# freewym/espresso

Hardware: AMD Instinct MI355X
Metric: audio-hours/sec training (LibriSpeech Conformer-12 + CTC) (higher is better)
Workload: dtype bf16; 1 GPU; LibriSpeech 960h Conformer-12 + CTC update step, <=26000 frames & <=24 utts per GPU, V=5004, on-GPU fbank+CMVN+SpecAugment, dropout 0.1, clip 2.0, Adam; parallelism=dp1

## Files before the change

espresso_amd/csrc/conv_igemm.hip:

```cpp
#include <hip/hip_runtime.h>

#include "gemm_common.h"

namespace {

typedef const __attribute__((address_space(1))) void* gptr_t;
typedef __attribute__((address_space(3))) void* lptr_t;

struct ConvGatherArgs {
  const bf16_t* src;
  const bf16_t* W;
  bf16_t* out;
  const float* bias;
  double* stats;
  const bf16_t* zero;
  int RB, RT, RF;
  int ST, SF, SC;
  int at, af;
  int ntaps;
  int bt[9], bf[9], koff[9];
  int N;
  long ldw;
  int OT, OF, ot_mul, ot_add, of_mul, of_add;
};

template <int BN_>
__global__ __launch_bounds__(256, 2) void conv_gather_kernel(const ConvGatherArgs a) {
  constexpr int BM_ = 128, NST = 2;
  constexpr int NJ = BN_ / 32;
  constexpr int A_BYTES = BM_ * ROW_BYTES, STAGE = A_BYTES + BN_ * ROW_BYTES;
  constexpr int NA = BM_ / 32, NB = BN_ / 32;
  extern __shared__ __attribute__((aligned(16))) char dsm[];
  const int tid = threadIdx.x, lane = tid & 63, wave = tid >> 6;
  const int wm = wave >> 1, wcol = (wave & 1) * (BN_ / 2);
  const uint32_t M = (uint32_t)a.RB * a.RT * a.RF;
  const uint32_t m0 = blockIdx.x * BM_;
  const int cpt = a.SC / BK;
  const int nk = a.ntaps * cpt;

  int rowb[NA], rowt[NA], rowf[NA];
  int cs[NA];
#pragma unroll
  for (int i = 0; i < NA; ++i) {
    const int r = (wave + 4 * i) * 8 + (lane >> 3);
    cs[i] = (lane & 7) ^ (r & 7) ^ ((r >> 4) & 7);
    const uint32_t p = m0 + r;
    if (p < M) {
      const uint32_t q = p / (uint32_t)a.RF, b = q / (uint32_t)a.RT;
      const int rf = (int)(p - q * a.RF), rt = (int)(q - b * a.RT);
      rowb[i] = (int)b * a.ST;
      rowt[i] = rt * a.at;
      rowf[i] = rf * a.af;
    } else {
      rowb[i] = -1;
      rowt[i] = rowf[i] = 0;
    }
  }
  const bf16_t* bp[NB];
#pragma unroll
  for (int i = 0; i < NB; ++i) {
    const int r = (wave + 4 * i) * 8 + (lane >> 3);
    const int c = (lane & 7) ^ (r & 7) ^ ((r >> 4) & 7);
    bp[i] = a.W + (long)min(r, a.N - 1) * a.ldw + c * 8;
  }
  auto issue = [&](int stage, int kt) {
    const int tap = kt / cpt, chunk = kt - tap * cpt;
    const int dt = a.bt[tap], df = a.bf[tap];
    const long ko = a.koff[tap] + chunk * BK;
    char* base = dsm + stage * STAGE + wave * 1024;
#pragma unroll
    for (int i = 0; i < NA; ++i) {
      const int st = rowt[i] + dt, sf = rowf[i] + df;
      const bool ok = rowb[i] >= 0 && (unsigned)st < (unsigned)a.ST && (unsigned)sf < (unsigned)a.SF;
      const bf16_t* s = ok ? a.src + (((long)(rowb[i] + st)) * a.SF + sf) * a.SC + chunk * BK + cs[i] * 8 : a.zero + cs[i] * 8;
      __builtin_amdgcn_global_load_lds((gptr_t)s, (lptr_t)(base + i * 4096), 16, 0, 0);
    }
#pragma unroll
    for (int i = 0; i < NB; ++i)
      __builtin_amdgcn_global_load_lds((gptr_t)(bp[i] + ko), (lptr_t)(base + A_BYTES + i * 4096), 16, 0, 0);
  };

  f32x4_t acc[4][NJ];
#pragma unroll
  for (int i = 0; i < 4; ++i)
#pragma unroll
    for (int j = 0; j < NJ; ++j) acc[i][j] = (f32x4_t){0.f, 0.f, 0.f, 0.f};
  uint32_t a_off[2][4], b_off[2][NJ];
#pragma unroll
  for (int ks = 0; ks < 2; ++ks) {
#pragma unroll
    for (int i = 0; i < 4; ++i) a_off[ks][i] = lds_off(wm * 64 + i * 16 + (lane & 15), ks * 4 + (lane >> 4));
#pragma unroll
    for (int j = 0; j < NJ; ++j) b_off[ks][j] = A_BYTES + lds_off(wcol + j * 16 + (lane & 15), ks * 4 + (lane >> 4));
  }

  if (nk > 0) issue(0, 0);
  int stage = 0;
  for (int kt = 0; kt < nk; ++kt) {
    asm volatile("s_waitcnt vmcnt(0)" ::: "memory");
    __builtin_amdgcn_s_barrier();
    if (kt + 1 < nk) issue(stage ^ 1, kt + 1);
    const char* st = dsm + stage * STAGE;
#pragma unroll
    for (int ks = 0; ks < 2; ++ks) {
      bf16x8_t af[4], bfr[NJ];
#pragma unroll
      for (int i = 0; i < 4; ++i) af[i] = *reinterpret_cast<const bf16x8_t*>(st + a_off[ks][i]);
#pragma unroll
      for (int j = 0; j < NJ; ++j) bfr[j] = *reinterpret_cast<const bf16x8_t*>(st + b_off[ks][j]);
#pragma unroll
      for (int i = 0; i < 4; ++i)
#pragma unroll
        for (int j = 0; j < NJ; ++j)
          acc[i][j] = __builtin_amdgcn_mfma_f32_16x16x32_bf16(
              __builtin_bit_cast(__attribute__((ext_vector_type(8))) __bf16, af[i]),
              __builtin_bit_cast(__attribute__((ext_vector_type(8))) __bf16, bfr[j]), acc[i][j], 0, 0, 0);
    }
    stage ^= 1;
  }

  constexpr int CG = BN_ / 8;
  constexpr int RL = 256 / CG;
  float* sC = reinterpret_cast<float*>(dsm);
  const int cg = tid % CG, rlane = tid / CG;
  float bias8[8], s8[8], q8[8];
#pragma unroll
  for (int e = 0; e < 8; ++e) {
    bias8[e] = a.bias ? a.bias[cg * 8 + e] : 0.f;
    s8[e] = q8[e] = 0.f;
  }
#pragma unroll 1
  for (int half = 0; half < 2; ++half) {
    __syncthreads();
    if (wm == half) {
#pragma unroll
      for (int i = 0; i < 4; ++i)
#pragma unroll
        for (int j = 0; j < NJ; ++j)
#pragma unroll
          for (int r = 0; r < 4; ++r) sC[(i * 16 + (lane >> 4) * 4 + r) * BN_ + wcol + j * 16 + (lane & 15)] = acc[i][j][r];
    }
    __syncthreads();
#pragma unroll 1
    for (int pass = 0; pass < 64 / RL; ++pass) {
      const int rl = pass * RL + rlane;
      const uint32_t p = m0 + half * 64 + rl;
      if (p < M) {
        const uint32_t q = p / (uint32_t)a.RF, b = q / (uint32_t)a.RT;
        const int rf = (int)(p - q * a.RF), rt = (int)(q - b * a.RT);
        const long orow = ((long)b * a.OT + (long)rt * a.ot_mul + a.ot_add) * a.OF + (long)rf * a.of_mul + a.of_add;
        const float4 x0 = *reinterpret_cast<const float4*>(sC + rl * BN_ + cg * 8);
        const float4 x1 = *reinterpret_cast<const float4*>(sC + rl * BN_ + cg * 8 + 4);
        float v[8] = {x0.x, x0.y, x0.z, x0.w, x1.x, x1.y, x1.z, x1.w};
#pragma unroll
        for (int e = 0; e < 8; ++e) v[e] += bias8[e];
        uint4 u;
        u.x = pack_bf2(v[0], v[1]); u.y = pack_bf2(v[2], v[3]); u.z = pack_bf2(v[4], v[5]); u.w = pack_bf2(v[6], v[7]);
        *reinterpret_cast<uint4*>(a.out + orow * a.N + cg * 8) = u;
        if (a.stats) {
          const uint32_t w[4] = {u.x, u.y, u.z, u.w};
#pragma unroll
          for (int e = 0; e < 4; ++e) {
            const float lo = __uint_as_float(w[e] << 16), hi = __uint_as_float(w[e] & 0xffff0000u);
            s8[2 * e] += lo; q8[2 * e] += lo * lo;
            s8[2 * e + 1] += hi; q8[2 * e + 1] += hi * hi;
          }
        }
      }
    }
  }
  if (a.stats) {
    __syncthreads();
    float* red = reinterpret_cast<float*>(dsm);
#pragma unroll
    for (int e = 0; e < 8; ++e) {
      red[(rlane * 2 + 0) * BN_ + cg * 8 + e] = s8[e];
      red[(rlane * 2 + 1) * BN_ + cg * 8 + e] = q8[e];
    }
    __syncthreads();
    if (tid < 2 * BN_) {
      const int which = tid / BN_, c = tid - which * BN_;
      float t = 0.f;
      for (int r = 0; r < RL; ++r) t += red[(r * 2 + which) * BN_ + c];
      atomicAdd(a.stats + which * a.N + c, (double)t);
    }
  }
}

const bf16_t* zero_line(hipStream_t stream) {
  static bf16_t* z = nullptr;
  if (!z) {
    if (hipMalloc(&z, 256) != hipSuccess) return nullptr;
    if (hipMemsetAsync(z, 0, 256, stream) != hipSuccess) return nullptr;
    hipStreamSynchronize(stream);
  }
  return z;
}

template <int BN_>
int launch_gather(const ConvGatherArgs& a, hipStream_t stream) {
  constexpr int bytes = 2 * (128 + BN_) * ROW_BYTES;
  static bool attr_ok = hipFuncSetAttribute(reinterpret_cast<const void*>(&conv_gather_kernel<BN_>),
                                            hipFuncAttributeMaxDynamicSharedMemorySize, bytes) == hipSuccess;
  if (!attr_ok) return -1;
  const long M = (long)a.RB * a.RT * a.RF;
  if (M <= 0) return 0;
  if (M >= (1L << 31) - 128) return -1;
  hipLaunchKernelGGL((conv_gather_kernel<BN_>), dim3((unsigned)((M + 127) / 128)), dim3(256), bytes, stream, a);
  return EA_CHECK_LAUNCH();
}


struct ConvWgradArgs {
  const bf16_t* X;
  const bf16_t* dZ;
  float* slab;
  const bf16_t* zero;
  int RB, RT, RF, ST, SF, Cin, Cout;
  int at, af, ntaps;
  int bt[9], bf[9];
  int chunks_per_wg;
};

__device__ __forceinline__ int tr_sw(int r) { return (r & 3) ^ ((r >> 3) & 1); }
__device__ __forceinline__ void ds_read_tr16_x8(const uint32_t (&ad)[8], uint2 (&o)[8]) {
  asm volatile(
      "ds_read_b64_tr_b16 %0, %8\n\tds_read_b64_tr_b16 %1, %9\n\tds_read_b64_tr_b16 %2, %10\n\tds_read_b64_tr_b16 %3, %11\n\t"
      "ds_read_b64_tr_b16 %4, %12\n\tds_read_b64_tr_b16 %5, %13\n\tds_read_b64_tr_b16 %6, %14\n\tds_read_b64_tr_b16 %7, %15\n\t"
      "s_waitcnt lgkmcnt(0)"
      : "=&v"(o[0]), "=&v"(o[1]), "=&v"(o[2]), "=&v"(o[3]), "=&v"(o[4]), "=&v"(o[5]), "=&v"(o[6]), "=&v"(o[7])
      : "v"(ad[0]), "v"(ad[1]), "v"(ad[2]), "v"(ad[3]), "v"(ad[4]), "v"(ad[5]), "v"(ad[6]), "v"(ad[7])
      : "memory");
}

__global__ __launch_bounds__(256, 4) void conv_wgrad_kernel(const ConvWgradArgs a) {
  constexpr int TILE = 64 * ROW_BYTES;
  constexpr int NT = 3, NBUF = 2;
  const int tap0 = (int)(blockIdx.z % 3) * 3;
  const int zsplit = (int)(blockIdx.z / 3);
  __shared__ __attribute__((aligned(16))) char lds[(2 + NBUF) * TILE];
  const int tid = threadIdx.x, lane = tid & 63, wave = tid >> 6;
  const int wr = wave >> 1, wc = wave & 1;
  const int co0 = blockIdx.x * 64, ci0 = blockIdx.y * 64;
  const long M = (long)a.RB * a.RT * a.RF;
  const long chunk0 = (long)zsplit * a.chunks_per_wg;
  long nch = (M + 63) / 64 - chunk0;
  if (nch > a.chunks_per_wg) nch = a.chunks_per_wg;
  if (nch < 0) nch = 0;

  f32x4_t acc[NT][2][2];
#pragma unroll
  for (int t = 0; t < NT; ++t)
#pragma unroll
    for (int i = 0; i < 2; ++i)
#pragma unroll
      for (int j = 0; j < 2; ++j) acc[t][i][j] = (f32x4_t){0.f, 0.f, 0.f, 0.f};

  int rr[2], cs[2];
#pragma unroll
  for (int i = 0; i < 2; ++i) {
    rr[i] = (wave + 4 * i) * 8 + (lane >> 3);
    cs[i] = (lane & 7) ^ (tr_sw(rr[i]) << 1);
  }
  int rowb[2], rowt[2], rowf[2];
  long rowp[2];
  auto decode = [&](long ch) {
#pragma unroll
    for (int i = 0; i < 2; ++i) {
      const long p = (chunk0 + ch) * 64 + rr[i];
      rowp[i] = p;
      if (p < M) {
        const uint32_t q = (uint32_t)p / (uint32_t)a.RF, b = q / (uint32_t)a.RT;
        rowb[i] = (int)b * a.ST;
        rowt[i] = (int)(q - b * a.RT) * a.at;
        rowf[i] = (int)((uint32_t)p - q * a.RF) * a.af;
      } else {
        rowb[i] = -1;
        rowt[i] = rowf[i] = 0;
      }
    }
  };
  auto issue_A = [&](int abuf) {
#pragma unroll
    for (int i = 0; i < 2; ++i) {
      const bf16_t* s = rowb[i] >= 0 ? a.dZ + rowp[i] * a.Cout + co0 + cs[i] * 8 : a.zero + cs[i] * 8;
      __builtin_amdgcn_global_load_lds((gptr_t)s, (lptr_t)(lds + abuf * TILE + (wave + 4 * i) * 1024), 16, 0, 0);
    }
  };
  auto issue_B = [&](int buf, int tap) {
#pragma unroll
    for (int i = 0; i < 2; ++i) {
      const int st = rowt[i] + a.bt[tap0 + tap], sf = rowf[i] + a.bf[tap0 + tap];
      const bool ok = rowb[i] >= 0 && (unsigned)st < (unsigned)a.ST && (unsigned)sf < (unsigned)a.SF;
      const bf16_t* s = ok ? a.X + (((long)(rowb[i] + st)) * a.SF + sf) * a.Cin + ci0 + cs[i] * 8 : a.zero + cs[i] * 8;
      __builtin_amdgcn_global_load_lds((gptr_t)s, (lptr_t)(lds + (2 + buf) * TILE + (wave + 4 * i) * 1024), 16, 0, 0);
    }
  };
  const uint32_t lds0 = (uint32_t)(uintptr_t)lds;
  auto read_frags = [&](int tile_off, int c0, uint4 (&fr)[2][2]) {
    const int g = lane >> 4, i = lane & 15;
    uint32_t ad[8];
    uint2 o[8];
#pragma unroll
    for (int ks = 0; ks < 2; ++ks)
#pragma unroll
      for (int t = 0; t < 2; ++t)
#pragma unroll
        for (int h = 0; h < 2; ++h) {
          const int r = ks * 32 + 8 * g + (i >> 2) + 4 * h;
          const int chunk = (c0 >> 4) + t;
          ad[(ks * 2 + t) * 2 + h] = lds0 + tile_off + r * ROW_BYTES + ((chunk ^ tr_sw(r)) << 5) + (i & 3) * 8;
        }
    ds_read_tr16_x8(ad, o);
#pragma unroll
    for (int ks = 0; ks < 2; ++ks)
#pragma unroll
      for (int t = 0; t < 2; ++t) fr[ks][t] = make_uint4(o[(ks * 2 + t) * 2].x, o[(ks * 2 + t) * 2].y, o[(ks * 2 + t) * 2 + 1].x, o[(ks * 2 + t) * 2 + 1].y);
  };

  const int nsteps = (int)nch * NT;
  int is = 0, itap = 0;
  long ich = 0;
  auto issue_next = [&]() {
    if (is >= nsteps) return;
    if (itap == 0) {
      decode(ich);
      issue_A((int)(ich & 1));
    }
    issue_B(is & (NBUF - 1), itap);
    ++is;
    if (++itap == NT) { itap = 0; ++ich; }
  };
  issue_next();
  uint4 fa[2][2];
  long ch = 0;
  int tap = 0;
  for (int s = 0; s < nsteps; ++s) {
    const int tap1 = tap + 1 == NT ? 0 : tap + 1;
    asm volatile("s_waitcnt vmcnt(0)" ::: "memory");
    __builtin_amdgcn_s_barrier();
    uint4 fb[2][2];
    if (tap == 0) read_frags((int)(ch & 1) * TILE, wr * 32, fa);
    read_frags((2 + (s & (NBUF - 1))) * TILE, wc * 32, fb);
    __builtin_amdgcn_sched_barrier(0);
    issue_next();
#pragma unroll
    for (int t = 0; t < NT; ++t) {
      if (t == tap) {
#pragma unroll
        for (int ks = 0; ks < 2; ++ks)
#pragma unroll
          for (int i = 0; i < 2; ++i)
#pragma unroll
            for (int j = 0; j < 2; ++j)
              acc[t][i][j] = __builtin_amdgcn_mfma_f32_16x16x32_bf16(
                  __builtin_bit_cast(__attribute__((ext_vector_type(8))) __bf16, fa[ks][i]),
                  __builtin_bit_cast(__attribute__((ext_vector_type(8))) __bf16, fb[ks][j]), acc[t][i][j], 0, 0, 0);
      }
    }
    tap = tap1;
    if (tap1 == 0) ++ch;
  }

  float* out = a.slab + (long)zsplit * a.Cout * a.ntaps * a.Cin;
#pragma unroll
  for (int t = 0; t < NT; ++t) {
    {
#pragma unroll
      for (int i = 0; i < 2; ++i)
#pragma unroll
        for (int j = 0; j < 2; ++j)
#pragma unroll
          for (int r = 0; r < 4; ++r) {
            const int co = co0 + wr * 32 + i * 16 + (lane >> 4) * 4 + r, ci = ci0 + wc * 32 + j * 16 + (lane & 15);
            out[((long)co * a.ntaps + tap0 + t) * a.Cin + ci] = acc[t][i][j][r];
          }
    }
  }
}

__global__ __launch_bounds__(256) void conv_wgrad_reduce_kernel(const float* __restrict__ slab, float* __restrict__ dW, long n, int nsplit,
                                                                int cin = 0) {
  const int zper = (nsplit + gridDim.y - 1) / gridDim.y;
  const int z0 = blockIdx.y * zper, z1 = min(nsplit, z0 + zper);
  const long i = ((long)blockIdx.x * 256 + threadIdx.x) * 4;
  if (i >= n || z0 >= z1) return;
  float4 s = *reinterpret_cast<const float4*>(slab + (long)z0 * n + i);
  for (int z = z0 + 1; z < z1; ++z) {
    const float4 x = *reinterpret_cast<const float4*>(slab + (long)z * n + i);
    s.x += x.x; s.y += x.y; s.z += x.z; s.w += x.w;
  }
  if (cin > 0) {
    const long ct = i / cin;
    const int ci = (int)(i - ct * cin), tap = (int)(ct % 9);
    const long co = ct / 9;
    float* d = dW + (co * cin + ci) * 9 + tap;
    const float v[4] = {s.x, s.y, s.z, s.w};
#pragma unroll
    for (int e = 0; e < 4; ++e) {
      if (gridDim.y == 1) d[9 * e] += v[e];
      else atomicAdd(d + 9 * e, v[e]);
    }
    return;
  }
  if (gridDim.y == 1) {
    float4 d = *reinterpret_cast<const float4*>(dW + i);
    d.x += s.x; d.y += s.y; d.z += s.z; d.w += s.w;
    *reinterpret_cast<float4*>(dW + i) = d;
  } else {
    atomicAdd(dW + i, s.x); atomicAdd(dW + i + 1, s.y); atomicAdd(dW + i + 2, s.z); atomicAdd(dW + i + 3, s.w);
  }
}

static int wgrad_split(long M, int Cin, int Cout) {
  const long chunks = (M + 63) / 64;
  const int blocks = (Cin / 64) * (Cout / 64);
  constexpr long target = 256;
  long nsplit = (target + blocks - 1) / blocks;
  if (nsplit > chunks / 8) nsplit = chunks / 8;
  if (nsplit < 1) nsplit = 1;
  return (int)nsplit;
}

}

extern "C" int ea_conv3x3_fwd(const void* X, const void* W, const float* bias, void* Z, double* stats, int B, int T, int F,
                              int Cin, int Cout, int sy, int sx, hipStream_t stream) {
  if (B <= 0 || T <= 0 || F <= 0) return 0;
  if (Cin % 64 || (Cout != 64 && Cout != 128) || sy < 1 || sx < 1) return -2;
  ConvGatherArgs a;
  a.src = (const bf16_t*)X; a.W = (const bf16_t*)W; a.out = (bf16_t*)Z; a.bias = bias; a.stats = stats;
  a.zero = zero_line(stream);
  if (!a.zero) return -1;
  const int To = (T - 1) / sy + 1, Fo = (F - 1) / sx + 1;
  a.RB = B; a.RT = To; a.RF = Fo;
  a.ST = T; a.SF = F; a.SC = Cin;
  a.at = sy; a.af = sx;
  a.ntaps = 9;
  for (int ky = 0; ky < 3; ++ky)
    for (int kx = 0; kx < 3; ++kx) {
      const int t = ky * 3 + kx;
      a.bt[t] = ky - 1; a.bf[t] = kx - 1; a.koff[t] = t * Cin;
    }
  a.N = Cout; a.ldw = 9L * Cin;
  a.OT = To; a.OF = Fo; a.ot_mul = 1; a.ot_add = 0; a.of_mul = 1; a.of_add = 0;
  return Cout == 128 ? launch_gather<128>(a, stream) : launch_gather<64>(a, stream);
}

extern "C" int ea_conv3x3_dgrad(const void* dZ, const void* Wd, void* dX, int B, int T, int F, int Cin, int Cout, int sy, int sx,
                                hipStream_t stream) {
  if (B <= 0 || T <= 0 || F <= 0) return 0;
  if (Cout % 64 || (Cin != 64 && Cin != 128) || sy < 1 || sx < 1 || sy > 2 || sx > 2) return -2;
  const int To = (T - 1) / sy + 1, Fo = (F - 1) / sx + 1;
  const bf16_t* zero = zero_line(stream);
  if (!zero) return -1;
  for (int pt = 0; pt < sy; ++pt)
    for (int pf = 0; pf < sx; ++pf) {
      ConvGatherArgs a;
      a.src = (const bf16_t*)dZ; a.W = (const bf16_t*)Wd; a.out = (bf16_t*)dX; a.bias = nullptr; a.stats = nullptr; a.zero = zero;
      a.RB = B; a.RT = (T - pt + sy - 1) / sy; a.RF = (F - pf + sx - 1) / sx;
      a.ST = To; a.SF = Fo; a.SC = Cout;
      a.at = 1; a.af = 1;
      a.ntaps = 0;
      for (int ky = 0; ky < 3; ++ky) {
        if ((pt + 1 - ky) % sy) continue;
        for (int kx = 0; kx < 3; ++kx) {
          if ((pf + 1 - kx) % sx) continue;
          const int t = a.ntaps++;
          a.bt[t] = (pt + 1 - ky) / sy; a.bf[t] = (pf + 1 - kx) / sx; a.koff[t] = (ky * 3 + kx) * Cout;
        }
      }
      a.N = Cin; a.ldw = 9L * Cout;
      a.OT = T; a.OF = F; a.ot_mul = sy; a.ot_add = pt; a.of_mul = sx; a.of_add = pf;
      if (a.RT <= 0 || a.RF <= 0) continue;
      if (a.ntaps == 0) return -2;
      const int rc = Cin == 128 ? launch_gather<128>(a, stream) : launch_gather<64>(a, stream);
      if (rc) return rc;
    }
  return 0;
}

extern "C" long ea_conv3x3_wgrad_workspace_bytes(int B, int T, int F, int Cin, int Cout, int sy, int sx) {
  const int To = (T - 1) / sy + 1, Fo = (F - 1) / sx + 1;
  return (long)wgrad_split((long)B * To * Fo, Cin, Cout) * Cout * 9 * Cin * (long)sizeof(float);
}

static int conv3x3_wgrad_impl(const void* X, const void* dZ, float* dW, void* workspace, int B, int T, int F, int Cin, int Cout,
                              int sy, int sx, int param_layout, hipStream_t stream);
extern "C" int ea_conv3x3_wgrad(const void* X, const void* dZ, float* dW, void* workspace, int B, int T, int F, int Cin, int Cout,
                                int sy, int sx, hipStream_t stream) {
  return conv3x3_wgrad_impl(X, dZ, dW, workspace, B, T, F, Cin, Cout, sy, sx, 0, stream);
}
extern "C" int ea_conv3x3_wgrad_param_layout(const void* X, const void* dZ, float* dW, void* workspace, int B, int T, int F, int Cin,
                                             int Cout, int sy, int sx, hipStream_t stream) {
  return conv3x3_wgrad_impl(X, dZ, dW, workspace, B, T, F, Cin, Cout, sy, sx, 1, stream);
}
static int conv3x3_wgrad_impl(const void* X, const void* dZ, float* dW, void* workspace, int B, int T, int F, int Cin, int Cout,
                              int sy, int sx, int param_layout, hipStream_t stream) {
  if (B <= 0 || T <= 0 || F <= 0) return 0;
  if (Cin % 64 || Cout % 64 || sy < 1 || sx < 1 || !workspace) return -2;
  ConvWgradArgs a;
  a.X = (const bf16_t*)X; a.dZ = (const bf16_t*)dZ; a.slab = (float*)workspace;
  a.zero = zero_line(stream);
  if (!a.zero) return -1;
  const int To = (T - 1) / sy + 1, Fo = (F - 1) / sx + 1;
  a.RB = B; a.RT = To; a.RF = Fo; a.ST = T; a.SF = F; a.Cin = Cin; a.Cout = Cout;
  a.at = sy; a.af = sx; a.ntaps = 9;
  for (int ky = 0; ky < 3; ++ky)
    for (int kx = 0; kx < 3; ++kx) { a.bt[ky * 3 + kx] = ky - 1; a.bf[ky * 3 + kx] = kx - 1; }
  const long M = (long)B * To * Fo;
  if (M >= (1L << 31) - 128) return -2;
  const int nsplit = wgrad_split(M, Cin, Cout);
  const long chunks = (M + 63) / 64;
  a.chunks_per_wg = (int)((chunks + nsplit - 1) / nsplit);
  hipLaunchKernelGGL(conv_wgrad_kernel, dim3(Cout / 64, Cin / 64, nsplit * 3), dim3(256), 0, stream, a);
  const long n = (long)Cout * 9 * Cin;
  const long blocks = (n / 4 + 255) / 256;
  int zg = (int)(1024 / blocks);
  if (zg > nsplit / 4) zg = nsplit / 4;
  if (zg < 1) zg = 1;
  hipLaunchKernelGGL(conv_wgrad_reduce_kernel, dim3((unsigned)blocks, zg), dim3(256), 0, stream, (const float*)workspace, dW, n, nsplit,
                     param_layout ? Cin : 0);
  return EA_CHECK_LAUNCH();
}
```

espresso_amd/csrc/convmodule.hip:

```cpp
#include "common.h"
#include "convmodule_math.h"
#include "espresso_amd.h"

namespace {

constexpr int KMAX = 31;

constexpr int CT = 64, TTILE = 64, TPT = TTILE / 4;

template <int KW, int PADL>
__global__ __launch_bounds__(256) void glu_dwconv_fwd_kernel(const bf16_t* __restrict__ Y,
                                                             const float* __restrict__ w,
                                                             bf16_t* __restrict__ U, bf16_t* __restrict__ Z,
                                                             double* __restrict__ stats, int T, int C) {
  constexpr int PAD = PADL, ROWS = TTILE + KW - 1;
  __shared__ __attribute__((aligned(16))) float su[ROWS][CT];
  __shared__ float sred[2][4][CT];
  const int c0 = blockIdx.x * CT, t0 = blockIdx.y * TTILE, b = blockIdx.z;
  const long rowbase = (long)b * T;
  if ((C & 7) == 0 && c0 + CT <= C) {
    bf16_t (*sub)[CT] = reinterpret_cast<bf16_t (*)[CT]>(&su[0][0]);
    bf16_t (*sz)[CT] = reinterpret_cast<bf16_t (*)[CT]>(&su[0][0]) + ROWS;
    constexpr int NCH = (ROWS * (CT / 8) + 255) / 256;
    uint4 va[NCH], vg[NCH];
#pragma unroll
    for (int k = 0; k < NCH; ++k) {
      const int i = threadIdx.x + 256 * k;
      const int row = min(i / (CT / 8), ROWS - 1), c8 = (i % (CT / 8)) * 8;
      const int tin = min(max(t0 - PAD + row, 0), T - 1);
      const bf16_t* yr = Y + (rowbase + tin) * (2L * C) + c0 + c8;
      va[k] = *reinterpret_cast<const uint4*>(yr);
      vg[k] = *reinterpret_cast<const uint4*>(yr + C);
    }
    const int cl = threadIdx.x & (CT - 1), grp = threadIdx.x >> 6;
    float wk[KW];
#pragma unroll
    for (int k = 0; k < KW; ++k) wk[k] = w[(long)(c0 + cl) * KW + k];
#pragma unroll
    for (int k = 0; k < NCH; ++k) {
      const int i = threadIdx.x + 256 * k;
      if (i < ROWS * (CT / 8)) {
        const int row = i / (CT / 8), c8 = (i % (CT / 8)) * 8;
        const int tin = t0 - PAD + row;
        uint32_t pk[4];
        glu_gate8(va[k], vg[k], pk);
        const bool inside = tin >= 0 && tin < T;
        const uint4 u4 = inside ? make_uint4(pk[0], pk[1], pk[2], pk[3]) : make_uint4(0, 0, 0, 0);
        if (inside && row >= PAD && row < PAD + TTILE) *reinterpret_cast<uint4*>(U + (rowbase + tin) * C + c0 + c8) = u4;
        *reinterpret_cast<uint4*>(&sub[row][c8]) = u4;
      }
    }
    __syncthreads();
    float acc[TPT];
#pragma unroll
    for (int j = 0; j < TPT; ++j) acc[j] = 0.f;
#pragma unroll
    for (int r = 0; r < TPT + KW - 1; ++r) {
      const float x = bf2f(sub[grp * TPT + r][cl]);
#pragma unroll
      for (int j = 0; j < TPT; ++j)
        if (r - j >= 0 && r - j < KW) acc[j] += wk[r - j] * x;
    }
    float s = 0.f, q = 0.f;
#pragma unroll
    for (int j = 0; j < TPT; ++j) {
      const int tout = t0 + grp * TPT + j;
      const bf16_t zb = f2bf(acc[j]);
      sz[grp * TPT + j][cl] = zb;
      if (tout < T) {
        const float z = bf2f(zb);
        s += z;
        q += z * z;
      }
    }
    if (stats) {
      sred[0][grp][cl] = s;
      sred[1][grp][cl] = q;
    }
    __syncthreads();
#pragma unroll
    for (int k = 0; k < 2; ++k) {
      const int i = threadIdx.x + 256 * k;
      const int r = i >> 3, c8 = (i & 7) * 8;
      if (t0 + r < T) *reinterpret_cast<uint4*>(Z + (rowbase + t0 + r) * C + c0 + c8) = *reinterpret_cast<const uint4*>(&sz[r][c8]);
    }
    if (stats && threadIdx.x < CT) {
      const int x = threadIdx.x;
      atomicAdd(stats + c0 + x, (double)(sred[0][0][x] + sred[0][1][x] + sred[0][2][x] + sred[0][3][x]));
      atomicAdd(stats + C + c0 + x, (double)(sred[1][0][x] + sred[1][1][x] + sred[1][2][x] + sred[1][3][x]));
    }
    return;
  }
  const bool vec = (C & 7) == 0;
  for (int i = threadIdx.x; i < ROWS * (CT / 8); i += 256) {
    const int row = i / (CT / 8), c8 = (i % (CT / 8)) * 8;
    const int tin = t0 - PAD + row;
    float u[8];
#pragma unroll
    for (int e = 0; e < 8; ++e) u[e] = 0.f;
    if (tin >= 0 && tin < T && c0 + c8 < C) {
      const bf16_t* yr = Y + (rowbase + tin) * (2L * C) + c0 + c8;
      uint32_t pk[4] = {0, 0, 0, 0};
      if (vec && c0 + c8 + 8 <= C) {
        const uint4 av = *reinterpret_cast<const uint4*>(yr);
        const uint4 gv = *reinterpret_cast<const uint4*>(yr + C);
        glu_gate8(av, gv, pk);
        if (row >= PAD && row < PAD + TTILE)
          *reinterpret_cast<uint4*>(U + (rowbase + tin) * C + c0 + c8) = make_uint4(pk[0], pk[1], pk[2], pk[3]);
      } else {
        for (int e = 0; e < 8; ++e) {
          if (c0 + c8 + e >= C) break;
          const bf16_t ub = f2bf(bf2f(yr[e]) * sigmoid_f(bf2f(yr[C + e])));
          if (row >= PAD && row < PAD + TTILE) U[(rowbase + tin) * C + c0 + c8 + e] = ub;
          pk[e >> 1] |= (uint32_t)ub << (16 * (e & 1));
        }
      }
#pragma unroll
      for (int e = 0; e < 4; ++e) {
        u[2 * e] = __uint_as_float(pk[e] << 16);
        u[2 * e + 1] = __uint_as_float(pk[e] & 0xffff0000u);
      }
    }
    *reinterpret_cast<float4*>(&su[row][c8]) = make_float4(u[0], u[1], u[2], u[3]);
    *reinterpret_cast<float4*>(&su[row][c8 + 4]) = make_float4(u[4], u[5], u[6], u[7]);
  }
  const int cl = threadIdx.x & (CT - 1), grp = threadIdx.x >> 6;
  const int c = c0 + cl;
  float wk[KW];
#pragma unroll
  for (int k = 0; k < KW; ++k) wk[k] = c < C ? w[(long)c * KW + k] : 0.f;
  __syncthreads();
  float acc[TPT];
#pragma unroll
  for (int j = 0; j < TPT; ++j) acc[j] = 0.f;
#pragma unroll
  for (int r = 0; r < TPT + KW - 1; ++r) {
    const float x = su[grp * TPT + r][cl];
#pragma unroll
    for (int j = 0; j < TPT; ++j)
      if (r - j >= 0 && r - j < KW) acc[j] += wk[r - j] * x;
  }
  float s = 0.f, q = 0.f;
#pragma unroll
  for (int j = 0; j < TPT; ++j) {
    const int tout = t0 + grp * TPT + j;
    if (tout < T && c < C) {
      const bf16_t zb = f2bf(acc[j]);
      Z[(rowbase + tout) * C + c] = zb;
      const float z = bf2f(zb);
      s += z;
      q += z * z;
    }
  }
  if (stats) {
    sred[0][grp][cl] = s;
    sred[1][grp][cl] = q;
    __syncthreads();
    if (threadIdx.x < CT && c0 + threadIdx.x < C) {
      const int x = threadIdx.x;
      atomicAdd(stats + c0 + x, (double)(sred[0][0][x] + sred[0][1][x] + sred[0][2][x] + sred[0][3][x]));
      atomicAdd(stats + C + c0 + x, (double)(sred[1][0][x] + sred[1][1][x] + sred[1][2][x] + sred[1][3][x]));
    }
  }
}

__global__ void bn_finalize_kernel(const double* __restrict__ stats, float* __restrict__ mean_rstd,
                                   float* __restrict__ running_mean, float* __restrict__ running_var,
                                   int C, float n, float eps, float momentum) {
  const int c = blockIdx.x * blockDim.x + threadIdx.x;
  if (c >= C) return;
  const float mean = (float)(stats[c] / (double)n);
  float var = (float)(stats[C + c] / (double)n - (stats[c] / (double)n) * (stats[c] / (double)n));
  var = fmaxf(var, 0.f);
  mean_rstd[c] = mean;
  mean_rstd[C + c] = rsqrtf(var + eps);
  if (running_mean) {
    running_mean[c] = (1.f - momentum) * running_mean[c] + momentum * mean;
    const float unb = n > 1.f ? var * n / (n - 1.f) : var;
    running_var[c] = (1.f - momentum) * running_var[c] + momentum * unb;
  }
}
__global__ void bn_from_running_kernel(const float* __restrict__ running_mean, const float* __restrict__ running_var,
                                       float* __restrict__ mean_rstd, int C, float eps) {
  const int c = blockIdx.x * blockDim.x + threadIdx.x;
  if (c >= C) return;
  mean_rstd[c] = running_mean[c];
  mean_rstd[C + c] = rsqrtf(running_var[c] + eps);
}

__global__ __launch_bounds__(256) void bn_act_fwd_kernel(const bf16_t* __restrict__ Z, const float* __restrict__ mean_rstd,
                                                         const float* __restrict__ gamma, const float* __restrict__ beta,
                                                         bf16_t* __restrict__ Hout, long M, int C, int act) {
  const int nch = C >> 3;
  const long total = M * nch;
  const long stride = (long)gridDim.x * blockDim.x;
  const int ch = (int)(((long)blockIdx.x * blockDim.x + threadIdx.x) % nch);
  float sc[8], sh[8];
#pragma unroll
  for (int e = 0; e < 8; ++e) {
    const int c = ch * 8 + e;
    bn_scale_shift(mean_rstd[c], mean_rstd[C + c], gamma[c], beta[c], sc[e], sh[e]);
  }
  for (long i = (long)blockIdx.x * blockDim.x + threadIdx.x; i < total; i += stride) {
    const long m = i / nch;
    const uint4 u = *reinterpret_cast<const uint4*>(Z + m * C + ch * 8);
    float o[8];
    bn_act8(u, sc, sh, act, o);
    uint4 r;
    r.x = pack_bf2(o[0], o[1]); r.y = pack_bf2(o[2], o[3]); r.z = pack_bf2(o[4], o[5]); r.w = pack_bf2(o[6], o[7]);
    *reinterpret_cast<uint4*>(Hout + m * C + ch * 8) = r;
  }
}

__global__ __launch_bounds__(256) void bn_act_fwd_stats_kernel(const bf16_t* __restrict__ Z, const double* __restrict__ stats,
                                                               float* __restrict__ mean_rstd, float* __restrict__ running_mean,
                                                               float* __restrict__ running_var, const float* __restrict__ gamma,
                                                               const float* __restrict__ beta, bf16_t* __restrict__ Hout, long M,
                                                               int C, int act, float n, float eps, float momentum,
                                                               double* __restrict__ zero_next, int zero_n) {
  extern __shared__ float s_scsh[];
  const int nch = C >> 3;
  const long total = M * nch;
  const long stride = (long)gridDim.x * blockDim.x;
  const long gtid = (long)blockIdx.x * blockDim.x + threadIdx.x;
  const double inv_n = 1.0 / (double)n;
  for (int c = threadIdx.x; c < C; c += 256) {
    const double m1 = stats[c] * inv_n;
    const float mean = (float)m1;
    float var = (float)(stats[C + c] * inv_n - m1 * m1);
    var = fmaxf(var, 0.f);
    const float rstd = rsqrtf(var + eps);
    const float scv = rstd * gamma[c];
    s_scsh[c] = scv;
    s_scsh[C + c] = beta[c] - mean * scv;
    if (blockIdx.x == 0) {
      mean_rstd[c] = mean;
      mean_rstd[C + c] = rstd;
      if (running_mean) {
        running_mean[c] = (1.f - momentum) * running_mean[c] + momentum * mean;
        const float unb = n > 1.f ? var * n / (n - 1.f) : var;
        running_var[c] = (1.f - momentum) * running_var[c] + momentum * unb;
      }
    }
  }
  __syncthreads();
  const int ch = (int)(gtid % nch);
  float sc[8], sh[8];
#pragma unroll
  for (int e = 0; e < 8; ++e) {
    sc[e] = s_scsh[ch * 8 + e];
    sh[e] = s_scsh[C + ch * 8 + e];
  }
  for (long i = gtid; i < total; i += stride) {
    const long m = i / nch;
    const uint4 u = *reinterpret_cast<const uint4*>(Z + m * C + ch * 8);
    const uint32_t wv[4] = {u.x, u.y, u.z, u.w};
    float o[8];
#pragma unroll
    for (int e = 0; e < 8; ++e) {
      const float z = (e & 1) ? __uint_as_float(wv[e >> 1] & 0xffff0000u) : __uint_as_float(wv[e >> 1] << 16);
      const float y = z * sc[e] + sh[e];
      o[e] = act == 2 ? silu_f(y) : (act == 1 ? fmaxf(y, 0.f) : y);
    }
    uint4 r;
    r.x = pack_bf2(o[0], o[1]); r.y = pack_bf2(o[2], o[3]); r.z = pack_bf2(o[4], o[5]); r.w = pack_bf2(o[6], o[7]);
    *reinterpret_cast<uint4*>(Hout + m * C + ch * 8) = r;
  }
  if (zero_next)
    for (long i = gtid; i < zero_n; i += stride) zero_next[i] = 0.0;
}

__global__ __launch_bounds__(256) void bn_act_bwd_reduce_kernel(const bf16_t* __restrict__ Z, const bf16_t* __restrict__ dH,
                                                                const float* __restrict__ mean_rstd,
                                                                const float* __restrict__ gamma, const float* __restrict__ beta,
                                                                float* __restrict__ red, long M, int C, int act,
                                                                int rows_per_block, int TCH) {
  extern __shared__ float sm[];
  const int nch = C >> 3;
  const int cx = threadIdx.x % TCH, ry = threadIdx.x / TCH, lanes = 256 / TCH;
  const int ch = blockIdx.x * TCH + cx;
  const long r0 = (long)blockIdx.y * rows_per_block;
  const long r1 = min(M, r0 + rows_per_block);
  float sa[8], sb[8];
#pragma unroll
  for (int e = 0; e < 8; ++e) sa[e] = sb[e] = 0.f;
  if (ch < nch) {
    float mu[8], rs[8], ga[8], be[8];
#pragma unroll
    for (int e = 0; e < 8; ++e) {
      const int c = ch * 8 + e;
      mu[e] = mean_rstd[c]; rs[e] = mean_rstd[C + c]; ga[e] = gamma[c]; be[e] = beta[c];
    }
    auto accum = [&](const uint4& uz, const uint4& ud) {
      const uint32_t wz[4] = {uz.x, uz.y, uz.z, uz.w}, wd[4] = {ud.x, ud.y, ud.z, ud.w};
#pragma unroll
      for (int e = 0; e < 8; ++e) {
        const float z = (e & 1) ? __uint_as_float(wz[e >> 1] & 0xffff0000u) : __uint_as_float(wz[e >> 1] << 16);
        float d = (e & 1) ? __uint_as_float(wd[e >> 1] & 0xffff0000u) : __uint_as_float(wd[e >> 1] << 16);
        const float xh = (z - mu[e]) * rs[e];
        const float y = xh * ga[e] + be[e];
        d *= act == 2 ? dsilu_f(y) : (act == 1 ? (y > 0.f ? 1.f : 0.f) : 1.f);
        sa[e] += d;
        sb[e] += d * xh;
      }
    };
    constexpr int R = 4;
    long m = r0 + ry;
    for (; m + (long)(R - 1) * lanes < r1; m += (long)R * lanes) {
      uint4 uz[R], ud[R];
#pragma unroll
      for (int r = 0; r < R; ++r) {
        uz[r] = *reinterpret_cast<const uint4*>(Z + (m + (long)r * lanes) * C + ch * 8);
        ud[r] = *reinterpret_cast<const uint4*>(dH + (m + (long)r * lanes) * C + ch * 8);
      }
#pragma unroll
      for (int r = 0; r < R; ++r) accum(uz[r], ud[r]);
    }
    for (; m < r1; m += lanes) {
      const uint4 uz = *reinterpret_cast<const uint4*>(Z + m * C + ch * 8);
      const uint4 ud = *reinterpret_cast<const uint4*>(dH + m * C + ch * 8);
      accum(uz, ud);
    }
  }
  float* mine = sm + ((long)ry * TCH + cx) * 16;
#pragma unroll
  for (int e = 0; e < 8; ++e) { mine[e] = sa[e]; mine[8 + e] = sb[e]; }
  __syncthreads();
  for (int o = threadIdx.x; o < TCH * 16; o += 256) {
    const int cxo = o / 16, e = o % 16;
    const int cho = blockIdx.x * TCH + cxo;
    if (cho >= nch) continue;
    float a = 0.f;
    for (int r = 0; r < lanes; ++r) a += sm[((long)r * TCH + cxo) * 16 + e];
    atomicAdd(red + (e < 8 ? 0 : C) + cho * 8 + (e & 7), a);
  }
}

__global__ __launch_bounds__(256) void bn_act_bwd_apply_kernel(const bf16_t* __restrict__ Z, const bf16_t* __restrict__ dH,
                                                               const float* __restrict__ mean_rstd,
                                                               const float* __restrict__ gamma, const float* __restrict__ beta,
                                                               const float* __restrict__ red, bf16_t* __restrict__ dZ,
                                                               long M, int C, int act, float n,
                                                               float* __restrict__ dgamma = nullptr, float* __restrict__ dbeta = nullptr,
                                                               float* __restrict__ zero_next = nullptr, int zero_n = 0) {
  const int nch = C >> 3;
  const long total = M * nch;
  const float invn = n > 0.f ? 1.f / n : 0.f;
  const long stride = (long)gridDim.x * blockDim.x;
  const long gtid = (long)blockIdx.x * blockDim.x + threadIdx.x;
  const int ch = (int)(gtid % nch);
  float mu[8], rs[8], ga[8], be[8], r0[8], r1[8];
#pragma unroll
  for (int e = 0; e < 8; ++e) {
    const int c = ch * 8 + e;
    mu[e] = mean_rstd[c]; rs[e] = mean_rstd[C + c]; ga[e] = gamma[c]; be[e] = beta[c];
    r0[e] = red[c] * invn; r1[e] = red[C + c] * invn;
  }
  if (blockIdx.x == 0 && (dgamma || dbeta)) {
    for (int c = threadIdx.x; c < C; c += 256) {
      if (dbeta) dbeta[c] += red[c];
      if (dgamma) dgamma[c] += red[C + c];
    }
  }
  if (zero_next && blockIdx.x == gridDim.x - 1)
    for (int i = threadIdx.x; i < zero_n; i += 256) zero_next[i] = 0.f;
  for (long i = (long)blockIdx.x * blockDim.x + threadIdx.x; i < total; i += stride) {
    const long m = i / nch;
    const uint4 uz = *reinterpret_cast<const uint4*>(Z + m * C + ch * 8);
    const uint4 ud = *reinterpret_cast<const uint4*>(dH + m * C + ch * 8);
    const uint32_t wz[4] = {uz.x, uz.y, uz.z, uz.w}, wd[4] = {ud.x, ud.y, ud.z, ud.w};
    float o[8];
#pragma unroll
    for (int e = 0; e < 8; ++e) {
      const float z = (e & 1) ? __uint_as_float(wz[e >> 1] & 0xffff0000u) : __uint_as_float(wz[e >> 1] << 16);
      float d = (e & 1) ? __uint_as_float(wd[e >> 1] & 0xffff0000u) : __uint_as_float(wd[e >> 1] << 16);
      const float xh = (z - mu[e]) * rs[e];
      const float y = xh * ga[e] + be[e];
      d *= act == 2 ? dsilu_f(y) : (act == 1 ? (y > 0.f ? 1.f : 0.f) : 1.f);
      o[e] = rs[e] * ga[e] * (d - r0[e] - xh * r1[e]);
    }
    uint4 r;
    r.x = pack_bf2(o[0], o[1]); r.y = pack_bf2(o[2], o[3]); r.z = pack_bf2(o[4], o[5]); r.w = pack_bf2(o[6], o[7]);
    *reinterpret_cast<uint4*>(dZ + m * C + ch * 8) = r;
  }
}

template <int KW, int PADL>
__global__ __launch_bounds__(256) void glu_dwconv_bwd_data_kernel(const bf16_t* __restrict__ dZ, const bf16_t* __restrict__ Y,
                                                                  const float* __restrict__ w, bf16_t* __restrict__ dY,
                                                                  int T, int C) {
  constexpr int PAD = KW - 1 - PADL, ROWS = TTILE + KW - 1;
  constexpr int SDZ_BYTES = ROWS * CT * 2, SY_BYTES = 2 * TTILE * CT * 2;
  static_assert(SDZ_BYTES % 16 == 0 && SDZ_BYTES + SY_BYTES >= ROWS * CT * 4, "views of the shared buffer");
  __shared__ __attribute__((aligned(16))) char smem[SDZ_BYTES + SY_BYTES];
  bf16_t (*sdz)[CT] = reinterpret_cast<bf16_t (*)[CT]>(smem);
  bf16_t (*sy)[TTILE][CT] = reinterpret_cast<bf16_t (*)[TTILE][CT]>(smem + SDZ_BYTES);
  const int c0 = blockIdx.x * CT, t0 = blockIdx.y * TTILE, b = blockIdx.z;
  const long rowbase = (long)b * T;
  const int cl = threadIdx.x & (CT - 1), grp = threadIdx.x >> 6;
  const int c = c0 + cl;
  if ((C & 7) == 0 && c0 + CT <= C) {
    constexpr int NDZ = (ROWS * (CT / 8) + 255) / 256;
    uint4 vdz[NDZ], vy[4];
#pragma unroll
    for (int k = 0; k < NDZ; ++k) {
      const int i = threadIdx.x + 256 * k;
      const int row = min(i / (CT / 8), ROWS - 1), c8 = (i % (CT / 8)) * 8;
      const int tin = min(max(t0 - PAD + row, 0), T - 1);
      vdz[k] = *reinterpret_cast<const uint4*>(dZ + (rowbase + tin) * C + c0 + c8);
    }
#pragma unroll
    for (int k = 0; k < 4; ++k) {
      const int i = threadIdx.x + 256 * k;
      const int half = i >> 9, r = (i >> 3) & 63, c8 = (i & 7) * 8;
      const int tout = min(t0 + r, T - 1);
      vy[k] = *reinterpret_cast<const uint4*>(Y + (rowbase + tout) * (2L * C) + (long)half * C + c0 + c8);
    }
    float wk[KW];
#pragma unroll
    for (int k = 0; k < KW; ++k) wk[k] = w[(long)c * KW + k];
#pragma unroll
    for (int k = 0; k < NDZ; ++k) {
      const int i = threadIdx.x + 256 * k;
      if (i < ROWS * (CT / 8)) {
        const int row = i / (CT / 8), c8 = (i % (CT / 8)) * 8;
        const int tin = t0 - PAD + row;
        *reinterpret_cast<uint4*>(&sdz[row][c8]) = (tin >= 0 && tin < T) ? vdz[k] : make_uint4(0, 0, 0, 0);
      }
    }
#pragma unroll
    for (int k = 0; k < 4; ++k) {
      const int i = threadIdx.x + 256 * k;
      *reinterpret_cast<uint4*>(&sy[i >> 9][(i >> 3) & 63][(i & 7) * 8]) = vy[k];
    }
    __syncthreads();
    float acc[TPT];
#pragma unroll
    for (int j = 0; j < TPT; ++j) acc[j] = 0.f;
#pragma unroll
    for (int r = 0; r < TPT + KW - 1; ++r) {
      const float x = bf2f(sdz[grp * TPT + r][cl]);
#pragma unroll
      for (int j = 0; j < TPT; ++j) {
        const int k = j + (KW - 1) - r;
        if (k >= 0 && k < KW) acc[j] += wk[k] * x;
      }
    }
#pragma unroll
    for (int j = 0; j < TPT; ++j) {
      const int r = grp * TPT + j;
      const float av = bf2f(sy[0][r][cl]);
      const float sg = sigmoid_f(bf2f(sy[1][r][cl]));
      sy[0][r][cl] = f2bf(acc[j] * sg);
      sy[1][r][cl] = f2bf(acc[j] * av * sg * (1.f - sg));
    }
    __syncthreads();
#pragma unroll
    for (int k = 0; k < 4; ++k) {
      const int i = threadIdx.x + 256 * k;
      const int half = i >> 9, r = (i >> 3) & 63, c8 = (i & 7) * 8;
      if (t0 + r < T)
        *reinterpret_cast<uint4*>(dY + (rowbase + t0 + r) * (2L * C) + (long)half * C + c0 + c8) = *reinterpret_cast<const uint4*>(&sy[half][r][c8]);
    }
    return;
  }
  float (*sdf)[CT] = reinterpret_cast<float (*)[CT]>(smem);
  for (int i = threadIdx.x; i < ROWS * (CT / 8); i += 256) {
    const int row = i / (CT / 8), c8 = (i % (CT / 8)) * 8;
    const int tin = t0 - PAD + row;
    float d[8];
#pragma unroll
    for (int e = 0; e < 8; ++e) d[e] = 0.f;
    if (tin >= 0 && tin < T && c0 + c8 < C) {
      const bf16_t* src = dZ + (rowbase + tin) * C + c0 + c8;
      for (int e = 0; e < 8; ++e)
        if (c0 + c8 + e < C) d[e] = bf2f(src[e]);
    }
    *reinterpret_cast<float4*>(&sdf[row][c8]) = make_float4(d[0], d[1], d[2], d[3]);
    *reinterpret_cast<float4*>(&sdf[row][c8 + 4]) = make_float4(d[4], d[5], d[6], d[7]);
  }
  float wk[KW];
#pragma unroll
  for (int k = 0; k < KW; ++k) wk[k] = c < C ? w[(long)c * KW + k] : 0.f;
  __syncthreads();
  float acc[TPT];
#pragma unroll
  for (int j = 0; j < TPT; ++j) acc[j] = 0.f;
#pragma unroll
  for (int r = 0; r < TPT + KW - 1; ++r) {
    const float x = sdf[grp * TPT + r][cl];
#pragma unroll
    for (int j = 0; j < TPT; ++j) {
      const int k = j + (KW - 1) - r;
      if (k >= 0 && k < KW) acc[j] += wk[k] * x;
    }
  }
#pragma unroll
  for (int j = 0; j < TPT; ++j) {
    const int tout = t0 + grp * TPT + j;
    if (tout < T && c < C) {
      const bf16_t* yr = Y + (rowbase + tout) * (2L * C);
      const float av = bf2f(yr[c]);
      const float sg = sigmoid_f(bf2f(yr[C + c]));
      bf16_t* dyr = dY + (rowbase + tout) * (2L * C);
      dyr[c] = f2bf(acc[j] * sg);
      dyr[C + c] = f2bf(acc[j] * av * sg * (1.f - sg));
    }
  }
}

template <int KW, int PADL>
__global__ __launch_bounds__(256) void dwconv_bwd_weight_kernel(const bf16_t* __restrict__ dZ, const bf16_t* __restrict__ U,
                                                                float* __restrict__ part, int T, int C, int tiles_per_block) {
  constexpr int PAD = PADL, ROWS = TTILE + KW - 1, KG = 8;
  __shared__ __attribute__((aligned(16))) float sU[ROWS + KG][CT];
  __shared__ __attribute__((aligned(16))) float sD[TTILE][CT];
  const int c0 = blockIdx.x * CT, b = blockIdx.z;
  const long rowbase = (long)b * T;
  const int cl = threadIdx.x & (CT - 1), grp = threadIdx.x >> 6;
  float acc[KG];
#pragma unroll
  for (int k = 0; k < KG; ++k) acc[k] = 0.f;
  const int tbeg = blockIdx.y * tiles_per_block * TTILE, tend = min(T, tbeg + tiles_per_block * TTILE);
  for (int t0 = tbeg; t0 < tend; t0 += TTILE) {
    __syncthreads();
    const bool c_ok = (C & 7) == 0;
    for (int i = threadIdx.x; i < (ROWS + KG) * (CT / 8); i += 256) {
      const int row = i / (CT / 8), c8 = (i % (CT / 8)) * 8;
      const int tin = t0 - PAD + row;
      float u[8];
#pragma unroll
      for (int e = 0; e < 8; ++e) u[e] = 0.f;
      if (row < ROWS && tin >= 0 && tin < T) {
        const bf16_t* src = U + (rowbase + tin) * C + c0 + c8;
        if (c_ok && c0 + c8 + 8 <= C) {
          const uint4 v = *reinterpret_cast<const uint4*>(src);
          const uint32_t w[4] = {v.x, v.y, v.z, v.w};
#pragma unroll
          for (int e = 0; e < 4; ++e) {
            u[2 * e] = __uint_as_float(w[e] << 16);
            u[2 * e + 1] = __uint_as_float(w[e] & 0xffff0000u);
          }
        } else {
          for (int e = 0; e < 8; ++e)
            if (c0 + c8 + e < C) u[e] = bf2f(src[e]);
        }
      }
      *reinterpret_cast<float4*>(&sU[row][c8]) = make_float4(u[0], u[1], u[2], u[3]);
      *reinterpret_cast<float4*>(&sU[row][c8 + 4]) = make_float4(u[4], u[5], u[6], u[7]);
    }
    for (int i = threadIdx.x; i < TTILE * (CT / 8); i += 256) {
      const int row = i / (CT / 8), c8 = (i % (CT / 8)) * 8;
      const int t = t0 + row;
      float d[8];
#pragma unroll
      for (int e = 0; e < 8; ++e) d[e] = 0.f;
      if (t < T) {
        const bf16_t* src = dZ + (rowbase + t) * C + c0 + c8;
        if (c_ok && c0 + c8 + 8 <= C) {
          const uint4 v = *reinterpret_cast<const uint4*>(src);
          const uint32_t w[4] = {v.x, v.y, v.z, v.w};
#pragma unroll
          for (int e = 0; e < 4; ++e) {
            d[2 * e] = __uint_as_float(w[e] << 16);
            d[2 * e + 1] = __uint_as_float(w[e] & 0xffff0000u);
          }
        } else {
          for (int e = 0; e < 8; ++e)
            if (c0 + c8 + e < C) d[e] = bf2f(src[e]);
        }
      }
      *reinterpret_cast<float4*>(&sD[row][c8]) = make_float4(d[0], d[1], d[2], d[3]);
      *reinterpret_cast<float4*>(&sD[row][c8 + 4]) = make_float4(d[4], d[5], d[6], d[7]);
    }
    __syncthreads();
    if (grp * KG < KW) {
      float x[KG];
#pragma unroll
      for (int kk = 0; kk < KG - 1; ++kk) x[kk + 1] = sU[grp * KG + kk][cl];
#pragma unroll
      for (int tt = 0; tt < TTILE; ++tt) {
#pragma unroll
        for (int kk = 0; kk < KG - 1; ++kk) x[kk] = x[kk + 1];
        x[KG - 1] = sU[tt + grp * KG + KG - 1][cl];
        const float d = sD[tt][cl];
#pragma unroll
        for (int kk = 0; kk < KG; ++kk) acc[kk] += d * x[kk];
      }
    }
  }
  const int c = c0 + cl;
  if (c < C) {
    float* out = part + (((long)b * gridDim.y + blockIdx.y) * C + c) * KW;
#pragma unroll
    for (int kk = 0; kk < KG; ++kk)
      if (grp * KG + kk < KW) out[grp * KG + kk] = acc[kk];
  }
}
__global__ __launch_bounds__(256) void dwconv_weight_reduce_kernel(const float* __restrict__ part, float* __restrict__ dw, int nslab,
                                                                   int n) {
  const int i = blockIdx.x * 256 + threadIdx.x;
  if (i >= n) return;
  float a = 0.f;
  for (int s = blockIdx.y; s < nslab; s += gridDim.y) a += part[(long)s * n + i];
  if (gridDim.y == 1) dw[i] += a;
  else atomicAdd(dw + i, a);
}

static inline int egrid(long n) {
  long b = (n + 255) / 256;
  if (b > 8192) b = 8192;
  if (b < 1) b = 1;
  return (int)b;
}
static inline int egrid_ch(long n, int nch) {
  long b = egrid(n);
  while ((b * 256) % nch) ++b;
  return (int)b;
}

}

#define EA_KW_DISPATCH(KW, CAUSAL, FN, ...)                                          \
  switch (KW) {                                                                      \
    case 3: if (CAUSAL) FN<3, 2>(__VA_ARGS__); else FN<3, 1>(__VA_ARGS__); break;       \
    case 7: if (CAUSAL) FN<7, 6>(__VA_ARGS__); else FN<7, 3>(__VA_ARGS__); break;       \
    case 15: if (CAUSAL) FN<15, 14>(__VA_ARGS__); else FN<15, 7>(__VA_ARGS__); break;   \
    case 31: if (CAUSAL) FN<31, 30>(__VA_ARGS__); else FN<31, 15>(__VA_ARGS__); break;  \
    default: return -2;                                                              \
  }

template <int KW, int PADL>
static void launch_glu_dwconv_fwd(dim3 grid, hipStream_t stream, const bf16_t* Y, const float* w, bf16_t* U, bf16_t* Z,
                                  double* stats, int T, int C) {
  hipLaunchKernelGGL((glu_dwconv_fwd_kernel<KW, PADL>), grid, dim3(256), 0, stream, Y, w, U, Z, stats, T, C);
}
template <int KW, int PADL>
static void launch_glu_dwconv_bwd_data(dim3 grid, hipStream_t stream, const bf16_t* dZ, const bf16_t* Y, const float* w,
                                       bf16_t* dY, int T, int C) {
  hipLaunchKernelGGL((glu_dwconv_bwd_data_kernel<KW, PADL>), grid, dim3(256), 0, stream, dZ, Y, w, dY, T, C);
}
template <int KW, int PADL>
static void launch_dwconv_bwd_weight(dim3 grid, hipStream_t stream, const bf16_t* dZ, const bf16_t* U, float* dw, int T,
                                     int C, int tiles_per_block) {
  hipLaunchKernelGGL((dwconv_bwd_weight_kernel<KW, PADL>), grid, dim3(256), 0, stream, dZ, U, dw, T, C, tiles_per_block);
}

static int glu_dwconv_fwd(const void* Y, const float* w, void* U, void* Z, double* stats, int B, int T, int C, int KW, bool causal,
                          hipStream_t stream) {
  if (B <= 0 || T <= 0) return 0;
  if (C % 2) return -2;
  dim3 grid((C + CT - 1) / CT, (T + TTILE - 1) / TTILE, B);
  EA_KW_DISPATCH(KW, causal, launch_glu_dwconv_fwd, grid, stream, (const bf16_t*)Y, w, (bf16_t*)U, (bf16_t*)Z, stats, T, C);
  return EA_CHECK_LAUNCH();
}
extern "C" int ea_glu_dwconv_fwd(const void* Y, const float* w, void* U, void* Z, double* stats, int B, int T,
                                 int C, int KW, hipStream_t stream) {
  return glu_dwconv_fwd(Y, w, U, Z, stats, B, T, C, KW, false, stream);
}
extern "C" int ea_glu_dwconv_causal_fwd(const void* Y, const float* w, void* U, void* Z, double* stats, int B, int T,
                                        int C, int KW, hipStream_t stream) {
  return glu_dwconv_fwd(Y, w, U, Z, stats, B, T, C, KW, true, stream);
}

extern "C" int ea_bn_finalize(const double* stats, float* mean_rstd, float* running_mean, float* running_var, int C,
                              float n, float eps, float momentum, hipStream_t stream) {
  hipLaunchKernelGGL(bn_finalize_kernel, dim3((C + 255) / 256), dim3(256), 0, stream, stats, mean_rstd, running_mean,
                     running_var, C, n, eps, momentum);
  return EA_CHECK_LAUNCH();
}
extern "C" int ea_bn_from_running(const float* running_mean, const float* running_var, float* mean_rstd, int C,
                                  float eps, hipStream_t stream) {
  hipLaunchKernelGGL(bn_from_running_kernel, dim3((C + 255) / 256), dim3(256), 0, stream, running_mean, running_var,
                     mean_rstd, C, eps);
  return EA_CHECK_LAUNCH();
}
extern "C" int ea_bn_act_fwd(const void* Z, const float* mean_rstd, const float* gamma, const float* beta, void* H,
                             long M, int C, int act, hipStream_t stream) {
  if (M <= 0) return 0;
  if (C % 8) return -2;
  hipLaunchKernelGGL(bn_act_fwd_kernel, dim3(egrid_ch(M * (C / 8), C / 8)), dim3(256), 0, stream, (const bf16_t*)Z, mean_rstd,
                     gamma, beta, (bf16_t*)H, M, C, act);
  return EA_CHECK_LAUNCH();
}
extern "C" int ea_bn_act_bwd(const void* Z, const void* dH, const float* mean_rstd, const float* gamma,
                             const float* beta, float* red , void* dZ, float* dgamma, float* dbeta,
                             long M, int C, int act, int training, hipStream_t stream);
extern "C" int ea_bn_act_fwd_train(const void* Z, const double* stats, float* mean_rstd, float* running_mean, float* running_var,
                                   const float* gamma, const float* beta, void* H, long M, int C, int act, float n, float eps,
                                   float momentum, double* zero_next, int zero_n, hipStream_t stream) {
  if (M <= 0) return 0;
  if (C % 8) return -2;
  hipLaunchKernelGGL(bn_act_fwd_stats_kernel, dim3(egrid_ch(M * (C / 8), C / 8)), dim3(256), (size_t)2 * C * sizeof(float), stream, (const bf16_t*)Z, stats,
                     mean_rstd, running_mean, running_var, gamma, beta, (bf16_t*)H, M, C, act, n, eps, momentum, zero_next, zero_n);
  return EA_CHECK_LAUNCH();
}

namespace {
__device__ __forceinline__ int c1_sw(int r) { return (r & 3) ^ ((r >> 3) & 1); }
__device__ __forceinline__ void c1_tr_read8(const uint32_t (&ad)[8], uint2 (&o)[8]) {
  asm volatile(
      "ds_read_b64_tr_b16 %0, %8\n\tds_read_b64_tr_b16 %1, %9\n\tds_read_b64_tr_b16 %2, %10\n\tds_read_b64_tr_b16 %3, %11\n\t"
      "ds_read_b64_tr_b16 %4, %12\n\tds_read_b64_tr_b16 %5, %13\n\tds_read_b64_tr_b16 %6, %14\n\tds_read_b64_tr_b16 %7, %15\n\t"
      "s_waitcnt lgkmcnt(0)"
      : "=&v"(o[0]), "=&v"(o[1]), "=&v"(o[2]), "=&v"(o[3]), "=&v"(o[4]), "=&v"(o[5]), "=&v"(o[6]), "=&v"(o[7])
      : "v"(ad[0]), "v"(ad[1]), "v"(ad[2]), "v"(ad[3]), "v"(ad[4]), "v"(ad[5]), "v"(ad[6]), "v"(ad[7])
      : "memory");
}
__global__ __launch_bounds__(256) void conv1_bn_bwd_wgrad_kernel(const float* __restrict__ X, const bf16_t* __restrict__ Z,
                                                                 const bf16_t* __restrict__ dH, const float* __restrict__ mean_rstd,
                                                                 const float* __restrict__ gamma, const float* __restrict__ beta,
                                                                 const float* __restrict__ red, float* __restrict__ dW,
                                                                 float* __restrict__ dbias, int T, int F, int To, int Fo, int CO,
                                                                 int sy, int sx, long npos, int act, float n) {
  __shared__ __attribute__((aligned(16))) char tile[4][32 * 128];
  __shared__ float sred[4][64][16];
  const int lane = threadIdx.x & 63, wave = threadIdx.x >> 6;
  const int li = lane & 15, g4 = lane >> 4;
  const float invn = n > 0.f ? 1.f / n : 0.f;
  const long nblk = (npos + 31) / 32;
  const long bmax = (npos - 1) / ((long)Fo * To);
  const uint32_t lds0 = (uint32_t)(uintptr_t)(&tile[wave][0]);
  for (int cs = 0; cs < CO; cs += 64) {
    const int c8 = lane & 7, prow = lane >> 3;
    float mu[8], rs[8], ga[8], be[8], r0[8], r1[8];
#pragma unroll
    for (int e = 0; e < 8; ++e) {
      const int c = cs + c8 * 8 + e;
      mu[e] = mean_rstd[c]; rs[e] = mean_rstd[CO + c]; ga[e] = gamma[c]; be[e] = beta[c];
      r0[e] = red[c] * invn; r1[e] = red[CO + c] * invn;
    }
    f32x4_t acc[4];
#pragma unroll
    for (int mt = 0; mt < 4; ++mt) acc[mt] = (f32x4_t){0.f, 0.f, 0.f, 0.f};
    for (long blk = (long)blockIdx.x * 4 + wave; blk < nblk; blk += (long)gridDim.x * 4) {
      const long pb = blk * 32;
      uint4 uz4[4], ud4[4];
#pragma unroll
      for (int it = 0; it < 4; ++it) {
        const long p = min(pb + prow + 8 * it, npos - 1);
        uz4[it] = *reinterpret_cast<const uint4*>(Z + p * CO + cs + c8 * 8);
        ud4[it] = *reinterpret_cast<const uint4*>(dH + p * CO + cs + c8 * 8);
      }
      int fo = (int)(pb % Fo), to = (int)((pb / Fo) % To);
      long b = pb / ((long)Fo * To);
      float xs[8];
      bool xv[8];
#pragma unroll
      for (int j = 0; j < 8; ++j) {
        const int k = 8 * g4 + j;
        int f = fo + k, t = to;
        long bb = b;
        while (f >= Fo) { f -= Fo; ++t; }
        while (t >= To) { t -= To; ++bb; }
        const int tap = li < 9 ? li : 0;
        const int ti = t * sy + tap / 3 - 1, fi = f * sx + tap % 3 - 1;
        xv[j] = pb + k < npos && li < 9 && ti >= 0 && ti < T && fi >= 0 && fi < F;
        const int tc = min(max(ti, 0), T - 1), fc = min(max(fi, 0), F - 1);
        const long bc = bb < bmax ? bb : bmax;
        xs[j] = X[(bc * T + tc) * F + fc];
      }
#pragma unroll
      for (int it = 0; it < 4; ++it) {
        const int r = prow + 8 * it;
        const long p = pb + r;
        uint4 o = make_uint4(0, 0, 0, 0);
        {
          const uint4 uz = uz4[it], ud = ud4[it];
          const uint32_t wz[4] = {uz.x, uz.y, uz.z, uz.w}, wd[4] = {ud.x, ud.y, ud.z, ud.w};
          float d[8];
#pragma unroll
          for (int e = 0; e < 8; ++e) {
            const float z = (e & 1) ? __uint_as_float(wz[e >> 1] & 0xffff0000u) : __uint_as_float(wz[e >> 1] << 16);
            float g = (e & 1) ? __uint_as_float(wd[e >> 1] & 0xffff0000u) : __uint_as_float(wd[e >> 1] << 16);
            const float xh = (z - mu[e]) * rs[e];
            const float y = xh * ga[e] + be[e];
            g *= act == 2 ? dsilu_f(y) : (act == 1 ? (y > 0.f ? 1.f : 0.f) : 1.f);
            d[e] = rs[e] * ga[e] * (g - r0[e] - xh * r1[e]);
          }
          o.x = pack_bf2(d[0], d[1]); o.y = pack_bf2(d[2], d[3]); o.z = pack_bf2(d[4], d[5]); o.w = pack_bf2(d[6], d[7]);
        }
        if (p >= npos) o = make_uint4(0, 0, 0, 0);
        *reinterpret_cast<uint4*>(&tile[wave][r * 128 + (((c8 >> 1) ^ c1_sw(r)) << 5) + (c8 & 1) * 16]) = o;
      }
      uint32_t bh[4], bl[4];
#pragma unroll
      for (int j = 0; j < 8; ++j) {
        const int k = 8 * g4 + j;
        float x = xv[j] ? xs[j] : 0.f;
        if (li == 9 && pb + k < npos) x = 1.f;
        const uint32_t hi = (uint32_t)f2bf(x);
        const uint32_t lo = (uint32_t)f2bf(x - __uint_as_float(hi << 16));
        if (j & 1) { bh[j >> 1] |= hi << 16; bl[j >> 1] |= lo << 16; }
        else { bh[j >> 1] = hi; bl[j >> 1] = lo; }
      }
      __builtin_amdgcn_fence(__ATOMIC_RELEASE, "wavefront");
      __builtin_amdgcn_wave_barrier();
      __builtin_amdgcn_fence(__ATOMIC_ACQUIRE, "wavefront");
      uint32_t ad[8];
      uint2 o8[8];
#pragma unroll
      for (int mt = 0; mt < 4; ++mt)
#pragma unroll
        for (int h = 0; h < 2; ++h) {
          const int r = 8 * g4 + 4 * h + (li >> 2);
          ad[mt * 2 + h] = lds0 + r * 128 + ((mt ^ c1_sw(r)) << 5) + (li & 3) * 8;
        }
      c1_tr_read8(ad, o8);
      const bf16x8_t vbh = __builtin_bit_cast(bf16x8_t, make_uint4(bh[0], bh[1], bh[2], bh[3]));
      const bf16x8_t vbl = __builtin_bit_cast(bf16x8_t, make_uint4(bl[0], bl[1], bl[2], bl[3]));
#pragma unroll
      for (int mt = 0; mt < 4; ++mt) {
        const bf16x8_t a8 = __builtin_bit_cast(bf16x8_t, make_uint4(o8[mt * 2].x, o8[mt * 2].y, o8[mt * 2 + 1].x, o8[mt * 2 + 1].y));
        acc[mt] = __builtin_amdgcn_mfma_f32_16x16x32_bf16(__builtin_bit_cast(__attribute__((ext_vector_type(8))) __bf16, a8),
                                                          __builtin_bit_cast(__attribute__((ext_vector_type(8))) __bf16, vbh), acc[mt], 0, 0, 0);
        acc[mt] = __builtin_amdgcn_mfma_f32_16x16x32_bf16(__builtin_bit_cast(__attribute__((ext_vector_type(8))) __bf16, a8),
                                                          __builtin_bit_cast(__attribute__((ext_vector_type(8))) __bf16, vbl), acc[mt], 0, 0, 0);
      }
      __builtin_amdgcn_wave_barrier();
    }
#pragma unroll
    for (int mt = 0; mt < 4; ++mt)
#pragma unroll
      for (int r = 0; r < 4; ++r) sred[wave][mt * 16 + g4 * 4 + r][li] = acc[mt][r];
    __syncthreads();
    for (int i = threadIdx.x; i < 64 * 10; i += 256) {
      const int c = i / 10, k = i % 10;
      const float a = sred[0][c][k] + sred[1][c][k] + sred[2][c][k] + sred[3][c][k];
      if (k < 9) atomicAdd(dW + (cs + c) * 9 + k, a);
      else if (dbias) atomicAdd(dbias + cs + c, a);
    }
    __syncthreads();
  }
}

__global__ void bn_param_grad_kernel(const float* __restrict__ red, float* __restrict__ dgamma, float* __restrict__ dbeta, int C) {
  const int c = blockIdx.x * blockDim.x + threadIdx.x;
  if (c >= C) return;
  if (dbeta) dbeta[c] += red[c];
  if (dgamma) dgamma[c] += red[C + c];
}
}

static void launch_bn_bwd_reduce(const void* Z, const void* dH, const float* mean_rstd, const float* gamma, const float* beta,
                                 float* red, long M, int C, int act, hipStream_t stream);

extern "C" int ea_bn_act_bwd(const void* Z, const void* dH, const float* mean_rstd, const float* gamma,
                             const float* beta, float* red, void* dZ, float* dgamma, float* dbeta, long M, int C,
                             int act, int training, hipStream_t stream) {
  if (M <= 0) return 0;
  if (C % 8) return -2;
  launch_bn_bwd_reduce(Z, dH, mean_rstd, gamma, beta, red, M, C, act, stream);
  hipLaunchKernelGGL(bn_act_bwd_apply_kernel, dim3(egrid_ch(M * (C / 8), C / 8)), dim3(256), 0, stream, (const bf16_t*)Z,
                     (const bf16_t*)dH, mean_rstd, gamma, beta, red, (bf16_t*)dZ, M, C, act,
                     training ? (float)M : 0.f);
  if (dgamma || dbeta) hipLaunchKernelGGL(bn_param_grad_kernel, dim3((C + 255) / 256), dim3(256), 0, stream, red, dgamma, dbeta, C);
  return EA_CHECK_LAUNCH();
}

extern "C" int ea_bn_act_bwd_fused(const void* Z, const void* dH, const float* mean_rstd, const float* gamma, const float* beta,
                                   float* red, void* dZ, float* dgamma, float* dbeta, long M, int C, int act, int training,
                                   float* zero_next, int zero_n, hipStream_t stream) {
  if (M <= 0) return 0;
  if (C % 8) return -2;
  launch_bn_bwd_reduce(Z, dH, mean_rstd, gamma, beta, red, M, C, act, stream);
  hipLaunchKernelGGL(bn_act_bwd_apply_kernel, dim3(egrid_ch(M * (C / 8), C / 8)), dim3(256), 0, stream, (const bf16_t*)Z,
                     (const bf16_t*)dH, mean_rstd, gamma, beta, red, (bf16_t*)dZ, M, C, act, training ? (float)M : 0.f, dgamma, dbeta,
                     zero_next, zero_n);
  return EA_CHECK_LAUNCH();
}

extern "C" int ea_conv1_bn_bwd(const float* X, const void* Z, const void* dH, const float* mean_rstd, const float* gamma,
                               const float* beta, float* red, float* dgamma, float* dbeta, float* dW, float* dbias, int B, int T,
                               int F, int CO, int sy, int sx, int act, int training, hipStream_t stream) {
  if (B <= 0 || T <= 0 || F <= 0) return 0;
  if (CO % 64) return -2;
  const int To = (T - 1) / sy + 1, Fo = (F - 1) / sx + 1;
  const long npos = (long)B * To * Fo;
  launch_bn_bwd_reduce(Z, dH, mean_rstd, gamma, beta, red, npos, CO, act, stream);
  long nb = (npos + 127) / 128;
  if (nb > 1024) nb = 1024;
  hipLaunchKernelGGL(conv1_bn_bwd_wgrad_kernel, dim3((unsigned)nb), dim3(256), 0, stream, X, (const bf16_t*)Z,
                     (const bf16_t*)dH, mean_rstd, gamma, beta, red, dW, dbias, T, F, To, Fo, CO, sy, sx, npos, act,
                     training ? (float)npos : 0.f);
  if (dgamma || dbeta) hipLaunchKernelGGL(bn_param_grad_kernel, dim3((CO + 255) / 256), dim3(256), 0, stream, red, dgamma, dbeta, CO);
  return EA_CHECK_LAUNCH();
}

static void launch_bn_bwd_reduce(const void* Z, const void* dH, const float* mean_rstd, const float* gamma, const float* beta,
                                 float* red, long M, int C, int act, hipStream_t stream) {
  const int nch = C / 8;
  int TCH = 1;
  while (TCH < 256 && TCH < nch) TCH <<= 1;
  const int lanes = 256 / TCH;
  int rpb = 8 * lanes;
  if (rpb < 32) rpb = 32;
  const long gx = (nch + TCH - 1) / TCH;
  const long want = (M + (2048 / gx) - 1) / (2048 / gx > 0 ? 2048 / gx : 1);
  if (want > rpb) rpb = (int)((want + lanes - 1) / lanes * lanes);
  dim3 g1((unsigned)gx, (unsigned)((M + rpb - 1) / rpb));
  hipLaunchKernelGGL(bn_act_bwd_reduce_kernel, g1, dim3(256), (size_t)256 * 16 * sizeof(float), stream, (const bf16_t*)Z,
                     (const bf16_t*)dH, mean_rstd, gamma, beta, red, M, C, act, rpb, TCH);
}
extern "C" int ea_bn_param_grad(const float* red, float* dgamma, float* dbeta, int C, hipStream_t stream) {
  hipLaunchKernelGGL(bn_param_grad_kernel, dim3((C + 255) / 256), dim3(256), 0, stream, red, dgamma, dbeta, C);
  return EA_CHECK_LAUNCH();
}

constexpr int DW_TILES_PER_BLOCK = 2;
static inline int dw_time_blocks(int T) {
  const int nt = (T + TTILE - 1) / TTILE;
  return (nt + DW_TILES_PER_BLOCK - 1) / DW_TILES_PER_BLOCK;
}
extern "C" long ea_dwconv_wgrad_workspace_bytes(int B, int T, int C, int KW) {
  return (long)B * dw_time_blocks(T) * C * KW * (long)sizeof(float);
}

static int dwconv_bwd_weight(const void* dZ, const void* U, float* dw, void* wgrad_ws, int B, int T, int C, int KW, bool causal,
                            hipStream_t stream) {
  if (B <= 0 || T <= 0) return 0;
  dim3 gridw((C + CT - 1) / CT, dw_time_blocks(T), B);
  float* part = (float*)wgrad_ws;
  EA_KW_DISPATCH(KW, causal, launch_dwconv_bwd_weight, gridw, stream, (const bf16_t*)dZ, (const bf16_t*)U, part, T, C, DW_TILES_PER_BLOCK);
  const int nslab = (int)(gridw.y * gridw.z);
  hipLaunchKernelGGL(dwconv_weight_reduce_kernel, dim3((C * KW + 255) / 256, nslab >= 16 ? 8 : 1), dim3(256), 0, stream, part, dw,
                     nslab, C * KW);
  return EA_CHECK_LAUNCH();
}
static int glu_dwconv_bwd(const void* dZ, const void* Y, const void* U, const float* w, void* dY, float* dw, void* wgrad_ws, int B,
                          int T, int C, int KW, bool causal, hipStream_t stream) {
  if (B <= 0 || T <= 0) return 0;
  if (C % 2) return -2;
  dim3 grid((C + CT - 1) / CT, (T + TTILE - 1) / TTILE, B);
  EA_KW_DISPATCH(KW, causal, launch_glu_dwconv_bwd_data, grid, stream, (const bf16_t*)dZ, (const bf16_t*)Y, w, (bf16_t*)dY, T, C);
  if (!dw) return EA_CHECK_LAUNCH();
  return dwconv_bwd_weight(dZ, U, dw, wgrad_ws, B, T, C, KW, causal, stream);
}

extern "C" int ea_glu_dwconv_bwd(const void* dZ, const void* Y, const void* U, const float* w, void* dY, float* dw,
                                 void* wgrad_ws, int B, int T, int C, int KW, hipStream_t stream) {
  return glu_dwconv_bwd(dZ, Y, U, w, dY, dw, wgrad_ws, B, T, C, KW, false, stream);
}
extern "C" int ea_dwconv_bwd_weight(const void* dZ, const void* U, float* dw, void* wgrad_ws, int B, int T, int C, int KW,
                                    hipStream_t stream) {
  return dwconv_bwd_weight(dZ, U, dw, wgrad_ws, B, T, C, KW, false, stream);
}
extern "C" int ea_glu_dwconv_causal_bwd(const void* dZ, const void* Y, const void* U, const float* w, void* dY, float* dw,
                                        void* wgrad_ws, int B, int T, int C, int KW, hipStream_t stream) {
  return glu_dwconv_bwd(dZ, Y, U, w, dY, dw, wgrad_ws, B, T, C, KW, true, stream);
}
extern "C" int ea_dwconv_causal_bwd_weight(const void* dZ, const void* U, float* dw, void* wgrad_ws, int B, int T, int C, int KW,
                                           hipStream_t stream) {
  return dwconv_bwd_weight(dZ, U, dw, wgrad_ws, B, T, C, KW, true, stream);
}
```

espresso_amd/functional.py:

```python
import collections

import ctypes
import os

import torch

from . import kernels as K

_seed_state = {"base": 0x5EED, "counter": 0}


def set_dropout_seed(seed: int):
    _seed_state["base"] = int(seed) & 0xFFFFFFFF
    _seed_state["counter"] = 0


_seed_trace = None


class trace_dropout_seeds:

    def __enter__(self):
        global _seed_trace
        self.prev, self.entries = _seed_trace, []
# ... 371 lines not shown
               drop_seed=s1)
        dW1 = _wgrad(dz, xn, M, Fd, C)
        db1 = K.colsum(dz, _zeros_f32(Fd, x), M, Fd, Fd)
        dxn = _new((M, C), torch.bfloat16, x)
        K.gemm(dz, w1_16, dxn, M, C, Fd, lda=Fd, ldb=C, ldc=C, b_kstrided=True)
        if ln_g is None:
            return dxn + dy, None, None, dW1, db1, dW2, db2, None, None, None, None, None, None, None
        dg, db = _zeros_f32(C, x), _zeros_f32(C, x)
        dx = K.layernorm_bwd(x, dxn, ln_g, mean, rstd, dg, db, dx_add=dy)
        return dx, dg, db, dW1, db1, dW2, db2, None, None, None, None, None, None, None


def ffn_module(x, ln_g, ln_b, w1, b1, w2, b2, act="silu", p_act=0.0, p_out=0.0, out_scale=0.5, eps=1e-5):
    return _FFN.apply(x, ln_g, ln_b, w1, b1, w2, b2, bf16_weight(w1), bf16_weight(w2), act, p_act, p_out, out_scale, eps)


def _pad8(n):
    return (n + 7) // 8 * 8


class _RelPosMHSA(torch.autograd.Function):

    @staticmethod
    def forward(ctx, x, ln_g, ln_b, wqkv, bqkv, wo, bo, u, v, wpos, wqkv16, wo16, wpos16, pe, key_len, attn_mask, B, T,
                H, p_attn, p_out, eps, pre_ln, causal=False):
        M, C = x.shape
        dh = C // H
        scaling = dh ** -0.5
        if pre_ln:
            xn, mean, rstd = K.layernorm_fwd(x, ln_g, ln_b, eps)
        else:
            xn, mean, rstd = x, None, None
        qkv = _new((M, 3 * C), torch.bfloat16, x)
        K.gemm(xn, wqkv16, qkv, M, 3 * C, C, lda=C, ldb=C, ldc=3 * C, bias=bqkv)
        relpos = pe is not None
        learned = relpos and wpos is None
        if learned:
            qu, _ = K.relpos_q_prep(qkv, 3 * C, None, None, M, C, scaling, want_qv=False)
            qv = qu
        else:
            qu, qv = K.relpos_q_prep(qkv, 3 * C, u if relpos else None, v if relpos else None, M, C, scaling, want_qv=relpos)
        Z = H * B
        Sp = _pad8(T)
        R = 2 * T - 1
        Rp = _pad8(R)
        pp = None
        if relpos:
            if learned:
                pp = K.cast_f32_to_bf16(pe.detach().contiguous())
            else:
                pp = _new((R, C), torch.bfloat16, x)
                K.gemm(pe, wpos16, pp, R, C, C, lda=C, ldb=C, ldc=C)
        sa = _next_seed("attn.probs", p_attn) if p_attn > 0 else 0
        fused = attn_mask is None and K.flash_attention_supported(dh, T, T, relpos)
        P = Pd = lse = bits = None
        if fused:
            o, lse, bits = K.flash_attention_fwd(qu, qv if relpos else None, qkv[:, C:], qkv[:, 2 * C:], pp, key_len, H, B, T, T, C,
                                                 3 * C, C, causal=causal, drop_p=p_attn, drop_seed=sa, want_bits=True)
        else:
            ac = _new((Z * T, Sp), torch.float32, x)
            K.gemm(qu, qkv, ac, T, T, dh, lda=C, ldb=3 * C, ldc=Sp, batch=Z, zdiv=B, sA=(dh, T * C), sB=(dh, T * 3 * C),
                   b_off=C, sC=(B * T * Sp, T * Sp))
            bd = None
            if relpos:
                bd = _new((Z * T, Rp), torch.float32, x)
                K.gemm(qv, pp, bd, T, R, dh, lda=C, ldb=C, ldc=Rp, batch=Z, zdiv=B, sA=(dh, T * C), sB=(dh, 0),
                       sC=(B * T * Rp, T * Rp))
            P, Pd = K.relpos_softmax_fwd(ac, bd, key_len, attn_mask, H, B, T, T, Sp, Rp, Sp, causal, p_attn, sa)
            del ac, bd
            o = _new((M, C), torch.bfloat16, x)
            K.gemm(Pd, qkv, o, T, dh, T, lda=Sp, ldb=3 * C, ldc=C, b_kstrided=True, batch=Z, zdiv=B, sA=(B * T * Sp, T * Sp),
                   sB=(dh, T * 3 * C), b_off=2 * C, sC=(dh, T * C))
        so = _next_seed("attn.out", p_out) if p_out > 0 else 0
        y = _new((M, C), torch.bfloat16, x)
        K.gemm(o, wo16, y, M, C, C, lda=C, ldb=C, ldc=C, bias=bo, drop_p=p_out, drop_seed=so, resid=x, ldr=C)
        ctx.save_for_backward(x, ln_g, mean, rstd, xn, qkv, qu, qv, pp, P, Pd, o, wqkv16, wo16, wpos16, pe, lse, key_len, bits)
        ctx.cfg = (B, T, H, p_attn, p_out, sa, so, pre_ln, relpos, learned, fused, causal)
        return y

    @staticmethod
    def backward(ctx, dy):
        (x, ln_g, mean, rstd, xn, qkv, qu, qv, pp, P, Pd, o, wqkv16, wo16, wpos16, pe, lse, key_len, bits) = ctx.saved_tensors
        B, T, H, p_attn, p_out, sa, so, pre_ln, relpos, learned, fused, causal = ctx.cfg
        M, C = x.shape
        dh = C // H
        scaling = dh ** -0.5
        Z = H * B
        Sp, R = _pad8(T), 2 * T - 1
        Rp = _pad8(R)
        dy = dy.contiguous()
        g = K.scale_dropout(dy, a=1.0, drop_p=p_out, drop_seed=so) if p_out > 0 else dy
        dWo = _wgrad(g, o, M, C, C)
        dbo = K.colsum(g, _zeros_f32(C, x), M, C, C)
        do = _new((M, C), torch.bfloat16, x)
        K.gemm(g, wo16, do, M, C, C, lda=C, ldb=C, ldc=C, b_kstrided=True)
        dqkv = _new((M, 3 * C), torch.bfloat16, x)
        t2 = dBD = None
        if fused:
            t1, t2, dBD = K.flash_attention_bwd(qu, qv if relpos else None, qkv[:, C:], qkv[:, 2 * C:], pp, key_len, o, do, lse,
                                                dqkv[:, C:], dqkv[:, 2 * C:], H, B, T, T, C, 3 * C, 3 * C, ldpp=C, causal=causal,
                                                scaling=scaling, drop_p=p_attn, drop_seed=sa, keep_bits=bits,
                                                dq=dqkv if relpos else None, lddq=3 * C)
        else:
            dPd = _new((Z * T, Sp), torch.float32, x)
            K.gemm(do, qkv, dPd, T, T, dh, lda=C, ldb=3 * C, ldc=Sp, batch=Z, zdiv=B, sA=(dh, T * C), sB=(dh, T * 3 * C),
                   b_off=2 * C, sC=(B * T * Sp, T * Sp))
            K.gemm(Pd, do, dqkv, T, dh, T, lda=Sp, ldb=C, ldc=3 * C, a_kstrided=True, b_kstrided=True, batch=Z, zdiv=B,
                   sA=(B * T * Sp, T * Sp), sB=(dh, T * C), sC=(dh, T * 3 * C), c_off=2 * C)
            dAC, dBD = K.relpos_softmax_bwd(P, dPd, H, B, T, T, Sp, Sp, Rp, want_bd=relpos, drop_p=p_attn, drop_seed=sa)
            del dPd
            K.gemm(dAC, qu, dqkv, T, dh, T, lda=Sp, ldb=C, ldc=3 * C, a_kstrided=True, b_kstrided=True, batch=Z, zdiv=B,
                   sA=(B * T * Sp, T * Sp), sB=(dh, T * C), sC=(dh, T * 3 * C), c_off=C)
            t1 = _new((M, C), torch.bfloat16, x)
            K.gemm(dAC, qkv, t1, T, dh, T, lda=Sp, ldb=3 * C, ldc=C, b_kstrided=True, batch=Z, zdiv=B, sA=(B * T * Sp, T * Sp),
                   sB=(dh, T * 3 * C), b_off=C, sC=(dh, T * C), alpha=scaling)
            if relpos:
                t2 = _new((M, C), torch.bfloat16, x)
                K.gemm(dBD, pp, t2, T, dh, R, lda=Rp, ldb=C, ldc=C, b_kstrided=True, batch=Z, zdiv=B, sA=(B * T * Rp, T * Rp),
                       sB=(dh, 0), sC=(dh, T * C), alpha=scaling)
        du = dv = dWpos = dpe = None
        if relpos:
            dpp32 = _new((R, C), torch.float32, x)
            K.gemm(dBD, qv, dpp32, R, dh, B * T, lda=Rp, ldb=C, ldc=C, a_kstrided=True, b_kstrided=True, batch=H, zdiv=1,
                   sA=(B * T * Rp, 0), sB=(dh, 0), sC=(dh, 0), splitk=_auto_splitk(((R + 127) // 128) * H, B * T))
            if learned:
                dpe = dpp32
            else:
                dWpos = _wgrad(K.cast_f32_to_bf16(dpp32), pe, R, C, C)
                du = K.colsum(t1, _zeros_f32(C, x), M, C, C)
                dv = K.colsum(t2, _zeros_f32(C, x), M, C, C)
            if not fused:
                K.add2_strided(t1, C, t2, C, dqkv, 3 * C, M, C)
        else:
            K.add2_strided(t1, C, torch.zeros_like(t1), C, dqkv, 3 * C, M, C)
        dWqkv = _wgrad(dqkv, xn, M, 3 * C, C)
        dbqkv = K.colsum(dqkv, _zeros_f32(3 * C, x), M, 3 * C, 3 * C)
        dxn = _new((M, C), torch.bfloat16, x)
        K.gemm(dqkv, wqkv16, dxn, M, C, 3 * C, lda=3 * C, ldb=C, ldc=C, b_kstrided=True)
        if pre_ln:
            dg, db = _zeros_f32(C, x), _zeros_f32(C, x)
            dx = K.layernorm_bwd(x, dxn, ln_g, mean, rstd, dg, db, dx_add=dy)
        else:
            dg = db = None
            dx = K.scale_dropout(dxn, a=1.0, y=dy, b=1.0)
        return (dx, dg, db, dWqkv, dbqkv, dWo, dbo, du, dv, dWpos, None, None, None, dpe) + (None,) * 10


def relpos_mhsa(x, ln_g, ln_b, wqkv, bqkv, wo, bo, u, v, wpos, pe, key_len, attn_mask, B, T, H, p_attn=0.0, p_out=0.0,
                eps=1e-5, pre_ln=True, wqkv16=None, causal=False):
    return _RelPosMHSA.apply(
        x, ln_g, ln_b, wqkv, bqkv, wo, bo, u, v, wpos, wqkv16 if wqkv16 is not None else bf16_weight(wqkv),
        bf16_weight(wo), bf16_weight(wpos) if wpos is not None else None, pe, key_len, attn_mask, B, T, H, p_attn, p_out,
        eps, pre_ln, causal)


class _ConvModule(torch.autograd.Function):

    @staticmethod
    def forward(ctx, x, ln_g, ln_b, wpw1, wdw, bn_g, bn_b, wpw2, wpw1_16, wpw2_16, running_mean, running_var, B, T, KW,
                p_out, eps, bn_eps, bn_momentum, training, causal=False):
        M, C = x.shape
        xn, mean, rstd = K.layernorm_fwd(x, ln_g, ln_b, eps)
        Y = _new((M, 2 * C), torch.bfloat16, x)
        K.gemm(xn, wpw1_16, Y, M, 2 * C, C, lda=C, ldb=C, ldc=2 * C)
        wdw2 = wdw.detach().reshape(C, KW).contiguous()
        stats = torch.zeros(2 * C, dtype=torch.float64, device=x.device) if training else None
        U, Zt = K.glu_dwconv_fwd(Y, wdw2, B, T, C, KW, stats, causal=causal)
        if training:
            mr = K.bn_finalize(stats, C, M, bn_eps, bn_momentum, running_mean, running_var)
        else:
            mr = K.bn_from_running(running_mean, running_var, bn_eps)
        Hh = K.bn_act_fwd(Zt, mr, bn_g, bn_b, "silu")
        so = _next_seed("conv.out", p_out) if p_out > 0 else 0
        y = _new((M, C), torch.bfloat16, x)
        K.gemm(Hh, wpw2_16, y, M, C, C, lda=C, ldb=C, ldc=C, drop_p=p_out, drop_seed=so, resid=x, ldr=C)
        ctx.save_for_backward(x, ln_g, mean, rstd, xn, Y, U, Zt, mr, Hh, bn_g, bn_b, wdw2, wpw1_16, wpw2_16)
        ctx.cfg = (B, T, KW, p_out, so, training, causal)
        ctx.wdw_shape = wdw.shape
        return y

    @staticmethod
    def backward(ctx, dy):
        (x, ln_g, mean, rstd, xn, Y, U, Zt, mr, Hh, bn_g, bn_b, wdw2, wpw1_16, wpw2_16) = ctx.saved_tensors
        B, T, KW, p_out, so, training, causal = ctx.cfg
        M, C = x.shape
        dy = dy.contiguous()
        g = K.scale_dropout(dy, a=1.0, drop_p=p_out, drop_seed=so) if p_out > 0 else dy
        dWpw2 = _wgrad(g, Hh, M, C, C)
        dH = _new((M, C), torch.bfloat16, x)
        K.gemm(g, wpw2_16, dH, M, C, C, lda=C, ldb=C, ldc=C, b_kstrided=True)
        dbn_g, dbn_b = _zeros_f32(C, x), _zeros_f32(C, x)
        dZ = K.bn_act_bwd(Zt, dH, mr, bn_g, bn_b, dbn_g, dbn_b, "silu", training)
        dwdw = _zeros_f32(C * KW, x)
        dY = K.glu_dwconv_bwd(dZ, Y, U, wdw2, dwdw, B, T, C, KW, causal=causal)
        dWpw1 = _wgrad(dY, xn, M, 2 * C, C)
        dxn = _new((M, C), torch.bfloat16, x)
        K.gemm(dY, wpw1_16, dxn, M, C, 2 * C, lda=2 * C, ldb=C, ldc=C, b_kstrided=True)
        dg, db = _zeros_f32(C, x), _zeros_f32(C, x)
        dx = K.layernorm_bwd(x, dxn, ln_g, mean, rstd, dg, db, dx_add=dy)
        return (dx, dg, db, dWpw1.view(2 * C, C, 1), dwdw.view(ctx.wdw_shape), dbn_g, dbn_b, dWpw2.view(C, C, 1)) + (None,) * 13


def conv_module(x, ln_g, ln_b, wpw1, wdw, bn_g, bn_b, wpw2, running_mean, running_var, B, T, p_out=0.0, eps=1e-5,
                bn_eps=1e-5, bn_momentum=0.1, training=True, causal=False):
    C = x.shape[1]
    KW = wdw.shape[-1]
    return _ConvModule.apply(x, ln_g, ln_b, wpw1, wdw, bn_g, bn_b, wpw2, bf16_weight(wpw1).view(2 * C, C),
                             bf16_weight(wpw2).view(C, C), running_mean, running_var, B, T, KW, p_out, eps, bn_eps,
                             bn_momentum, training, bool(causal))


class _CTCLoss(torch.autograd.Function):

    @staticmethod
    def forward(ctx, logits, targets, in_len, tgt_len, B, T, blank, zero_infinity):
        M, V = logits.shape
        assert M == B * T
        if logits.stride(1) != 1:
            logits = logits.contiguous()
        Lmax = targets.shape[1]
        lprobs = K.log_softmax(logits, M, V, logits.stride(0))
        nll, ws = K.ctc_loss_fwd(lprobs, targets, in_len, tgt_len, B, T, V, Lmax, blank)
        ctx.save_for_backward(lprobs, ws, nll, targets, in_len, tgt_len)
        ctx.cfg = (B, T, V, Lmax, blank, zero_infinity, logits.dtype)
        ctx.mark_non_differentiable(lprobs)
        return nll, lprobs

    @staticmethod
    def backward(ctx, dnll, _dlp):
        lprobs, ws, nll, targets, in_len, tgt_len = ctx.saved_tensors
        B, T, V, Lmax, blank, zero_infinity, dt = ctx.cfg
        scale_dev = dnll.float().contiguous()
        bf = dt == torch.bfloat16
        ld = _pad8(V) if bf else V
        dl = K.ctc_loss_grad(lprobs, ws, nll, targets, in_len, tgt_len, B, T, V, Lmax, blank, ld_out=ld, grad_bf16=bf,
                             grad_scale=1.0, grad_scale_dev=scale_dev, zero_infinity=zero_infinity)
        return (dl if ld == V else dl[:, :V]), None, None, None, None, None, None, None


def ctc_loss(logits, targets, in_len, tgt_len, B, T, blank=0, zero_infinity=True):
    return _CTCLoss.apply(logits, targets, in_len, tgt_len, B, T, blank, zero_infinity)


class _LabelSmoothedCE(torch.autograd.Function):

    @staticmethod
    def forward(ctx, logits, target, pad_idx, eps, smoothing="uniform", prior=None, tgt_len=0):
        M, V = logits.shape
        if logits.stride(1) != 1:
            logits = logits.contiguous()
        out, _ = K.label_smoothed_ce(logits, logits.stride(0), target, M, V, pad_idx, eps, want_grad=False, smoothing=smoothing,
                                     prior=prior, tgt_len=tgt_len)
        ctx.save_for_backward(logits, target, prior)
        ctx.cfg = (pad_idx, eps, smoothing, tgt_len)
        return out[0], out[1]

    @staticmethod
    def backward(ctx, dloss, _dnll):
        logits, target, prior = ctx.saved_tensors
        pad_idx, eps, smoothing, tgt_len = ctx.cfg
        M, V = logits.shape
        bf = logits.dtype == torch.bfloat16
        _, dl = K.label_smoothed_ce(logits, logits.stride(0), target, M, V, pad_idx, eps, want_grad=True, grad_bf16=bf,
                                    grad_ld=_pad8(V) if bf else V, smoothing=smoothing, prior=prior, tgt_len=tgt_len)
        g = dl if dl.shape[1] == V else dl[:, :V]
        return g * dloss.to(g.dtype), None, None, None, None, None, None


def label_smoothed_ce(logits, target, pad_idx, eps, smoothing="uniform", prior=None, tgt_len=0):
    return _LabelSmoothedCE.apply(logits, target, pad_idx, eps, smoothing, prior, tgt_len)


_CONV_IGEMM = True


_CONV1_FUSED_BWD = True


def set_conv1_fused_backward(on: bool) -> bool:
    global _CONV1_FUSED_BWD
    old, _CONV1_FUSED_BWD = _CONV1_FUSED_BWD, bool(on)
    return old


def set_conv_implicit_gemm(on: bool):
    global _CONV_IGEMM
    _CONV_IGEMM = bool(on)


def _conv_igemm_ok(cin, cout, sy, sx):
    return _CONV_IGEMM and cin in (64, 128) and cout in (64, 128) and sy in (1, 2) and sx in (1, 2)


class _ConvSubsample(torch.autograd.Function):

    @staticmethod
    def forward(ctx, X, row_zero, strides, bufs, p_drop, training, bn_eps, bn_momentum, *params):
        B, T, F = X.shape
        L = len(params) // 4
        saved = []
        cfgs = []
        A = None
        Tc, Fc, Cc = T, F, 1
        for i in range(L):
            w, b, g, beta = params[4 * i: 4 * i + 4]
            rm, rv = bufs[2 * i], bufs[2 * i + 1]
            sy, sx = strides[i]
            Co = w.shape[0]
            To, Fo = (Tc - 1) // sy + 1, (Fc - 1) // sx + 1
            stats = _pool_zeros((2 * Co,), torch.float64, X.device) if training else None
            if i == 0:
                assert w.shape[1] == 1 and tuple(w.shape[2:]) == (3, 3)
                Zi = K.conv1_fwd(X, w.detach().reshape(Co, 9).contiguous(), b, B, Tc, Fc, Co, sy, sx, stats)
                col, w16 = None, None
            elif _conv_igemm_ok(Cc, Co, sy, sx):
                w16 = K.cast_f32_to_bf16(w.detach().permute(0, 2, 3, 1).reshape(Co, 9 * Cc).contiguous())
                Zi = K.conv3x3_fwd(A, w16, b, B, Tc, Fc, Cc, Co, sy, sx, stats=stats)
                col = A
            else:
                col = K.im2col3x3(A, B, Tc, Fc, Cc, sy, sx)
                w16 = K.cast_f32_to_bf16(w.detach().permute(0, 2, 3, 1).reshape(Co, 9 * Cc).contiguous())
                Zi = _new((B * To * Fo, Co), torch.bfloat16, X)
                K.gemm(col, w16, Zi, B * To * Fo, Co, 9 * Cc, lda=9 * Cc, ldb=9 * Cc, ldc=Co, bias=b)
                if training:
                    K.colstats(Zi, stats)
            n = B * To * Fo
            mr = K.bn_finalize(stats, Co, n, bn_eps, bn_momentum, rm, rv) if training else K.bn_from_running(rm, rv, bn_eps)
            A = K.bn_act_fwd(Zi, mr, g, beta, "relu")
            saved += [Zi, mr, col, w16, g, beta]
            cfgs.append((Tc, Fc, Cc, To, Fo, Co, sy, sx))
            Tc, Fc, Cc = To, Fo, Co
        out = A.view(B * Tc, Fc * Cc)
        seed = _next_seed("subsample.out", p_drop) if (training and p_drop > 0) else 0
        if seed:
            out = K.scale_dropout(out, a=1.0, drop_p=p_drop, drop_seed=seed)
        if row_zero is not None:
            K.zero_rows(out, row_zero)
        ctx.save_for_backward(X, row_zero, *[t for t in saved if t is not None])
        ctx.layout = [[t is not None for t in saved[6 * i: 6 * i + 6]] for i in range(L)]
        ctx.cfg = (B, cfgs, p_drop, seed, training, [tuple(p.shape) for p in params[0::4]])
        ctx.igemm = [i > 0 and _conv_igemm_ok(cfgs[i][2], cfgs[i][5], cfgs[i][6], cfgs[i][7]) for i in range(L)]
        ctx.weights = [params[4 * i] for i in range(L)]
        ctx.params = list(params)
        return out

    @staticmethod
    def backward(ctx, dout):
        X, row_zero, *flat = ctx.saved_tensors
        B, cfgs, p_drop, seed, training, wshapes = ctx.cfg
        L = len(cfgs)
        it = iter(flat)
        per = []
        for i in range(L):
            per.append([next(it) if has else None for has in ctx.layout[i]])
        dout = dout.contiguous()
        if seed:
            dout = K.scale_dropout(dout, a=1.0, drop_p=p_drop, drop_seed=seed)
        elif row_zero is not None:
            dout = dout.clone()
        if row_zero is not None:
            K.zero_rows(dout, row_zero)
        grads = [None] * (4 * L)
        Tc, Fc, Cc, To, Fo, Co, sy, sx = cfgs[-1]
        dA = dout.view(B * To * Fo, Co)
        cur = torch.cuda.current_stream(X.device)
        side = _side_stream(X.device)
        keep = []
        for i in range(L - 1, -1, -1):
            Zi, mr, col, w16, g, beta = per[i]
            Tc, Fc, Cc, To, Fo, Co, sy, sx = cfgs[i]
            pw, pb, pg, pbe = ctx.params[4 * i: 4 * i + 4]
            sg, sbe = (_grad_sink(pg, Co), _grad_sink(pbe, Co)) if training else (None, None)
            if sg is not None and sbe is not None:
                dg, dbeta = sg, sbe
            else:
                sg = sbe = None
                dg, dbeta = _zeros_f32(Co, X), _zeros_f32(Co, X)
            if i == 0 and Co % 64 == 0 and _CONV1_FUSED_BWD:
                sW, sb = _grad_sink(pw, Co * 9), _grad_sink(pb, Co)
                if sW is not None and sb is not None:
                    db, dW = sb, sW
                else:
                    sW = None
                    db, dW = _zeros_f32(Co, X), _zeros_f32(Co * 9, X)
                K.conv1_bn_bwd(X, Zi, dA, mr, g, beta, dg, dbeta, dW, db, B, Tc, Fc, Co, sy, sx, "relu", training)
                if sW is None:
                    grads[0], grads[1] = dW.view(wshapes[0]), db
                if sg is None:
                    grads[2], grads[3] = dg, dbeta
                continue
            dZ = K.bn_act_bwd(Zi, dA, mr, g, beta, dg, dbeta, "relu", training)
            keep.append(dZ)
            n = B * To * Fo
            db = _zeros_f32(Co, X)
            if i == 0:
                dW = _zeros_f32(Co * 9, X)
                side.wait_stream(cur)
                with torch.cuda.stream(side):
                    K.conv1_wgrad(X, dZ, dW, db, B, Tc, Fc, Co, sy, sx)
                grads[0] = dW.view(wshapes[0])
            elif ctx.igemm[i]:
                sW = _grad_sink(pw, Co * 9 * Cc)
                side.wait_stream(cur)
                if sW is not None:
                    with torch.cuda.stream(side):
                        K.conv3x3_wgrad(col, dZ, sW, B, Tc, Fc, Cc, Co, sy, sx, param_layout=True)
                else:
                    dWp = _zeros_f32(Co * 9 * Cc, X).view(Co, 9 * Cc)
                    with torch.cuda.stream(side):
                        K.conv3x3_wgrad(col, dZ, dWp, B, Tc, Fc, Cc, Co, sy, sx)
                    grads[4 * i] = dWp.view(Co, 3, 3, Cc).permute(0, 3, 1, 2)
                if not training:
                    db = g.detach() * mr[1] * dbeta
                elif _grad_sink(pb, Co) is not None:
                    db = None
                wd16 = K.cast_f32_to_bf16(ctx.weights[i].detach().permute(1, 2, 3, 0).reshape(Cc, 9 * Co).contiguous())
                dA = K.conv3x3_dgrad(dZ, wd16, B, Tc, Fc, Cc, Co, sy, sx)
            else:
                dWp = torch.empty((Co, 9 * Cc), dtype=torch.float32, device=X.device)
                side.wait_stream(cur)
                with torch.cuda.stream(side):
                    _wgrad(dZ, col, n, Co, 9 * Cc, out=dWp)
                    K.colsum(dZ, db, n, Co, Co)
                grads[4 * i] = dWp.view(Co, 3, 3, Cc).permute(0, 3, 1, 2)
                dcol = _new((n, 9 * Cc), torch.bfloat16, X)
                K.gemm(dZ, w16, dcol, n, 9 * Cc, Co, lda=Co, ldb=9 * Cc, ldc=9 * Cc, b_kstrided=True)
                dA = K.col2im3x3(dcol, B, Tc, Fc, Cc, sy, sx)
            grads[4 * i + 1] = db
            if sg is None:
                grads[4 * i + 2] = dg
                grads[4 * i + 3] = dbeta
        cur.wait_stream(side)
        del keep
        return (None,) * 8 + tuple(grads)


def conv_subsample(X, row_zero, strides, params, bufs, p_drop=0.0, training=True, bn_eps=1e-5, bn_momentum=0.1):
    return _ConvSubsample.apply(X, row_zero, tuple(strides), list(bufs), p_drop, training, bn_eps, bn_momentum, *params)


_grad_ready_callback = None


def set_grad_ready_callback(fn):
    global _grad_ready_callback
    _grad_ready_callback = fn


def _ptr(t):
    return None if t is None else t.data_ptr()


class _LayerBinding:

    def __init__(self, m, kind="conformer"):
        import ctypes

        from ._lib import EaConformerLayer

        self.keep = []
        self.kind = kind
        L = EaConformerLayer()

        def w16(p, shape=None):
            t = bf16_weight(p)
            t = t.reshape(shape) if shape is not None else t
            self.keep.append(t)
            return t.data_ptr()

        def grad(p):
            if p.grad is None:
                p.grad = torch.zeros_like(p)
            return p.grad.data_ptr()

        def ffn(dst, gdst, f):
            dst.ln_g, dst.ln_b = _ptr(f.layer_norm.weight), _ptr(f.layer_norm.bias)
            dst.w1, dst.b1, dst.w2, dst.b2 = w16(f.w_1.weight), _ptr(f.w_1.bias), w16(f.w_2.weight), _ptr(f.w_2.bias)
            gdst.ln_g, gdst.ln_b = grad(f.layer_norm.weight), grad(f.layer_norm.bias)
            gdst.w1, gdst.b1, gdst.w2, gdst.b2 = grad(f.w_1.weight), grad(f.w_1.bias), grad(f.w_2.weight), grad(f.w_2.bias)

        if kind == "conformer":
            ffn(L.ffn1, L.grads.ffn1, m.ffn1)
            ffn(L.ffn2, L.grads.ffn2, m.ffn2)
            Cm, Fm = m.embed_dim, m.ffn1.w_1.weight.shape[0]
            self.wt = torch.empty(4 * Cm * Fm + 7 * Cm * Cm, dtype=torch.bfloat16, device=m.ffn1.w_1.weight.device)
        else:
            f1, gf = L.ffn1, L.grads.ffn1
            f1.ln_g, f1.ln_b = _ptr(m.final_layer_norm.weight), _ptr(m.final_layer_norm.bias)
            f1.w1, f1.b1, f1.w2, f1.b2 = w16(m.fc1.weight), _ptr(m.fc1.bias), w16(m.fc2.weight), _ptr(m.fc2.bias)
            gf.ln_g, gf.ln_b = grad(m.final_layer_norm.weight), grad(m.final_layer_norm.bias)
            gf.w1, gf.b1, gf.w2, gf.b2 = grad(m.fc1.weight), grad(m.fc1.bias), grad(m.fc2.weight), grad(m.fc2.bias)
            Cm, Fm = m.embed_dim, m.fc1.weight.shape[0]
            self.wt = torch.empty(2 * Cm * Fm + 4 * Cm * Cm, dtype=torch.bfloat16, device=m.fc1.weight.device)
        L.wt = self.wt.data_ptr()
        a = m.self_attn
        qw, kw, vw = a.q_proj.weight, a.k_proj.weight, a.v_proj.weight
        qb, kb, vb = a.q_proj.bias, a.k_proj.bias, a.v_proj.bias
        for p in (qw, kw, vw, qb, kb, vb):
            grad(p)
        fused16 = getattr(qw, "_ea_fused_qkv", None)
        n = qw.numel()
        grads_contig = (qw.grad is not None and kw.grad is not None and vw.grad is not None
                        and kw.grad.data_ptr() == qw.grad.data_ptr() + 4 * n and vw.grad.data_ptr() == kw.grad.data_ptr() + 4 * n)
        if fused16 is not None and grads_contig:
            wqkv16, self.split_w = fused16, None
            gw = qw.grad.data_ptr()
        else:
            wqkv16 = torch.cat([bf16_weight(qw), bf16_weight(kw), bf16_weight(vw)], 0)
            gbuf = torch.zeros(3 * qw.shape[0], qw.shape[1], dtype=torch.float32, device=qw.device)
            self.split_w = (gbuf, (qw, kw, vw))
            gw = gbuf.data_ptr()
        self.keep.append(wqkv16)
        nb = qb.numel()
        bias_contig = (kb.data_ptr() == qb.data_ptr() + 4 * nb and vb.data_ptr() == kb.data_ptr() + 4 * nb
                       and qb.grad is not None and kb.grad is not None and vb.grad is not None
                       and kb.grad.data_ptr() == qb.grad.data_ptr() + 4 * nb and vb.grad.data_ptr() == kb.grad.data_ptr() + 4 * nb)
        if bias_contig:
            self.split_b = None
            bq_ptr, gb_ptr = qb.data_ptr(), qb.grad.data_ptr()
        else:
            bq = torch.cat([qb.detach(), kb.detach(), vb.detach()], 0)
            gb = torch.zeros_like(bq)
            self.split_b = (gb, (qb, kb, vb))
            self.keep += [bq, gb]
            bq_ptr, gb_ptr = bq.data_ptr(), gb.data_ptr()
        self.cacheable = self.split_w is None and self.split_b is None
        self.key = (qw.data_ptr(), qw.grad.data_ptr() if qw.grad is not None else 0)
        A, GA = L.attn, L.grads.attn
        A.ln_g, A.ln_b = _ptr(m.self_attn_layer_norm.weight), _ptr(m.self_attn_layer_norm.bias)
        A.wqkv, A.bqkv, A.wo, A.bo = wqkv16.data_ptr(), bq_ptr, w16(a.out_proj.weight), _ptr(a.out_proj.bias)
        GA.ln_g, GA.ln_b = grad(m.self_attn_layer_norm.weight), grad(m.self_attn_layer_norm.bias)
        GA.wqkv, GA.bqkv, GA.wo, GA.bo = gw, gb_ptr, grad(a.out_proj.weight), grad(a.out_proj.bias)
        if a.pos_proj is not None:
            A.pos_u, A.pos_v, A.wpos = _ptr(a.pos_bias_u), _ptr(a.pos_bias_v), w16(a.pos_proj.weight)
            GA.pos_u, GA.pos_v, GA.wpos = grad(a.pos_bias_u), grad(a.pos_bias_v), grad(a.pos_proj.weight)
        for p in (qw, kw, vw, qb, kb, vb):
            grad(p)
        self.saved_buf, self.saved_busy = None, False
        self.L = L
        if kind != "conformer":
            mods = [a.q_proj, a.k_proj, a.v_proj, a.out_proj, m.self_attn_layer_norm, m.fc1, m.fc2, m.final_layer_norm]
            self.params = [p for mod in mods for p in mod.parameters()]
            if a.pos_proj is not None:
                self.params += [a.pos_bias_u, a.pos_bias_v, a.pos_proj.weight]
            return
        cm = m.conv_module
        Cc, GC = L.conv, L.grads.conv
        Cdim = m.embed_dim
        Cc.ln_g, Cc.ln_b = _ptr(cm.layer_norm.weight), _ptr(cm.layer_norm.bias)
        Cc.pw1 = w16(cm.pointwise_conv1.weight, (2 * Cdim, Cdim))
        Cc.dw = _ptr(cm.depthwise_conv.weight)
        Cc.bn_g, Cc.bn_b = _ptr(cm.batch_norm.weight), _ptr(cm.batch_norm.bias)
        Cc.bn_rm, Cc.bn_rv = _ptr(cm.batch_norm.running_mean), _ptr(cm.batch_norm.running_var)
        Cc.pw2 = w16(cm.pointwise_conv2.weight, (Cdim, Cdim))
        GC.ln_g, GC.ln_b = grad(cm.layer_norm.weight), grad(cm.layer_norm.bias)
        GC.pw1, GC.dw = grad(cm.pointwise_conv1.weight), grad(cm.depthwise_conv.weight)
        GC.bn_g, GC.bn_b, GC.pw2 = grad(cm.batch_norm.weight), grad(cm.batch_norm.bias), grad(cm.pointwise_conv2.weight)
        L.final_ln_g, L.final_ln_b = _ptr(m.final_layer_norm.weight), _ptr(m.final_layer_norm.bias)
        L.grads.final_ln_g, L.grads.final_ln_b = grad(m.final_layer_norm.weight), grad(m.final_layer_norm.bias)
        self.L = L
        self.params = [p for p in m.parameters()]
        self.saved_buf, self.saved_busy = None, False

    def finish_backward(self):
        if self.split_w is not None:
            gbuf, ps = self.split_w
            n = ps[0].shape[0]
            for i, p in enumerate(ps):
                p.grad += gbuf[i * n:(i + 1) * n]
        if self.split_b is not None:
            gb, ps = self.split_b
            n = ps[0].shape[0]
            for i, p in enumerate(ps):
                p.grad += gb[i * n:(i + 1) * n]
        if _grad_ready_callback is not None:
            _grad_ready_callback(self.params)


def _conformer_binding(module):
    bind = getattr(module, "_ea_binding", None)
    qw = module.self_attn.q_proj.weight
    if bind is None or bind.key != (qw.data_ptr(), qw.grad.data_ptr() if qw.grad is not None else 0):
        bind = _LayerBinding(module)
        module._ea_binding = bind if bind.cacheable else None
    return bind


def refresh_layer_transposes(layers, B, T):
    import ctypes

    from . import _lib
    from ._lib import EaLayerShape

    layers = list(layers)
    if not layers:
        return None
    dev = layers[0].ffn1.w_1.weight.device
    if dev.type != "cuda":
        return None
    binds = [_conformer_binding(m) for m in layers]
    if not all(b.cacheable for b in binds):
        return None
    cur, side = torch.cuda.current_stream(dev), _side_stream(dev)
    side.wait_stream(cur)
    lib = _lib.lib()
    for m, bind in zip(layers, binds):
        sh = EaLayerShape()
        sh.B, sh.T, sh.C, sh.H = B, T, m.embed_dim, m.num_heads
        sh.F = m.ffn1.w_1.weight.shape[0]
        sh.KW = m.conv_module.depthwise_conv.weight.shape[-1]
        sh.conv_causal = int(m.conv_module.causal)
        sh.training = 1
        _lib.check(lib.ea_conformer_layer_refresh_wt(ctypes.byref(bind.L), ctypes.byref(sh), ctypes.c_void_p(side.cuda_stream)),
                   "ea_conformer_layer_refresh_wt")
        m.__dict__["_ea_wt_fresh"] = bind
    return side.record_event()


_LAYER_CHAIN = True


def set_layer_chain(on: bool):
    global _LAYER_CHAIN
    _LAYER_CHAIN = bool(on)


_chain_pre = {}


def _chain_pre_buffer(like):
    key = (str(like.device), like.numel(), like.dtype)
    ring = _chain_pre.get(key)
    if ring is None:
        ring = _chain_pre[key] = [[torch.empty_like(like) for _ in range(3)], 0]
    ring[1] = (ring[1] + 1) % 3
    return ring[0][ring[1]]


def _chain_key(sh):
    return (sh.B, sh.T, sh.C, sh.H, sh.F, sh.KW, sh.conv_causal, sh.training, sh.has_attn_mask, sh.p_drop, sh.p_act,
            sh.p_attn)


class _ConformerLayerNative(torch.autograd.Function):
    @staticmethod
    def forward(ctx, x, module, key_len, attn_mask, pe, B, T, p_drop, p_act, p_attn, training, next_module=None):
        import ctypes

        from . import _lib
        from ._lib import EaLayerChain, EaLayerShape

        bind = _conformer_binding(module)
        sh = EaLayerShape()
        sh.B, sh.T, sh.C, sh.H = B, T, module.embed_dim, module.num_heads
        sh.F = module.ffn1.w_1.weight.shape[0]
        sh.KW = module.conv_module.depthwise_conv.weight.shape[-1]
        sh.conv_causal = int(module.conv_module.causal)
        sh.training = int(training)
        sh.wt_fresh = int(bool(training) and module.__dict__.pop("_ea_wt_fresh", None) is bind)
        sh.p_drop, sh.p_act, sh.p_attn = p_drop, p_act, p_attn
        sh.seed = _layer_seed("conformer", p_drop, p_act, p_attn)
        sh.has_attn_mask = int(attn_mask is not None)
        nb_saved, nb_scratch = ctypes.c_long(0), ctypes.c_long(0)
        lib = _lib.lib()
        _lib.check(lib.ea_conformer_layer_workspace(ctypes.byref(sh), ctypes.byref(nb_saved), ctypes.byref(nb_scratch)), "workspace")
        needs_bwd = ctx.needs_input_grad[0]
        if bind.saved_busy or not bind.cacheable:
            saved = torch.empty(nb_saved.value, dtype=torch.uint8, device=x.device)
            ctx.owns_arena = False
        else:
            if bind.saved_buf is None or bind.saved_buf.numel() < nb_saved.value or bind.saved_buf.device != x.device:
                bind.saved_buf = torch.empty(int(nb_saved.value * 1.1) + 4096, dtype=torch.uint8, device=x.device)
            saved = bind.saved_buf
            bind.saved_busy = bool(needs_bwd)
            ctx.owns_arena = bool(needs_bwd)
        scratch = _scratch_buffer(nb_scratch.value, x.device)
        _scratch_forward_touch(str(x.device))
        y = torch.empty_like(x)
        stream = K._stream()
        ch = EaLayerChain()
        token = module.__dict__.pop("_ea_chain_in", None)
        ctx.chain_prev = None
        if (token is not None and token[0] is bind and saved is bind.saved_buf and token[1].data_ptr() == x.data_ptr()
                and token[2] == _chain_key(sh)):
            ch.ln1_done = 1
            if needs_bwd:
                ctx.chain_prev = token[3]
        if next_module is not None and _LAYER_CHAIN and sh.C <= 512 and next_module is not module:
            nbind = _conformer_binding(next_module)
            if nbind.cacheable and not nbind.saved_busy:
                if nbind.saved_buf is None or nbind.saved_buf.numel() < nb_saved.value or nbind.saved_buf.device != x.device:
                    nbind.saved_buf = torch.empty(int(nb_saved.value * 1.1) + 4096, dtype=torch.uint8, device=x.device)
                ch.next = ctypes.addressof(nbind.L)
                ch.next_saved, ch.next_saved_bytes = nbind.saved_buf.data_ptr(), nbind.saved_buf.numel()
# ... 1044 lines not shown
```

espresso_amd/kernels.py:

```python
import ctypes
from typing import Optional

import torch

from . import _lib
from ._lib import EaGemmParams, check

ACT_NONE, ACT_RELU, ACT_SILU = 0, 1, 2
_ACT = {None: 0, "none": 0, "relu": 1, "silu": 2, "swish": 2}


def _stream():
    return ctypes.c_void_p(torch._C._cuda_getCurrentRawStream(torch._C._cuda_getDevice()))


def _p(t: Optional[torch.Tensor]):
    if t is None:
        return None
    if not t.is_cuda:
        raise RuntimeError("espresso_amd kernels need device tensors (no CPU path)")
    return ctypes.c_void_p(t.data_ptr())


def drop_params(p: float):
    if p <= 0.0:
        return 0, 1.0
    thr = min(int(p * 4294967296.0), 4294967295)
    return thr, 1.0 / (1.0 - p)


def gemm(
    A: torch.Tensor,
    B: torch.Tensor,
    C: torch.Tensor,
    M: int,
    N: int,
    K: int,
    *,
    lda: int,
    ldb: int,
    ldc: int,
    a_kstrided: bool = False,
    b_kstrided: bool = False,
    batch: int = 1,
    zdiv: int = 1,
    sA=(0, 0),
    sB=(0, 0),
    sC=(0, 0),
    a_off: int = 0,
    b_off: int = 0,
    c_off: int = 0,
    bias: Optional[torch.Tensor] = None,
    act=None,
    alpha: float = 1.0,
    out_scale: float = 1.0,
    resid: Optional[torch.Tensor] = None,
    ldr: int = 0,
    sR=(0, 0),
    r_off: int = 0,
    C2: Optional[torch.Tensor] = None,
    ldc2: int = 0,
    aux: Optional[torch.Tensor] = None,
    ldaux: int = 0,
    sX=(0, 0),
    accumulate: bool = False,
    drop_p: float = 0.0,
    drop_seed: int = 0,
    splitk: int = 1,
    qsplit=None,
):
    assert A.dtype == torch.bfloat16 and B.dtype == torch.bfloat16
    assert C.dtype in (torch.bfloat16, torch.float32)
    p = EaGemmParams()
    p.A = A.data_ptr() + 2 * a_off
    p.B = B.data_ptr() + 2 * b_off
    p.C = C.data_ptr() + C.element_size() * c_off
    p.C2 = (C2.data_ptr() + 2 * c_off) if C2 is not None else None
    if bias is not None:
        assert bias.dtype == torch.float32
        p.bias = bias.data_ptr()
    if resid is not None:
        assert resid.dtype in (torch.bfloat16, torch.float32)
        p.resid = resid.data_ptr() + resid.element_size() * r_off
        p.resid_f32 = 1 if resid.dtype == torch.float32 else 0
    if aux is not None:
        assert aux.dtype == torch.bfloat16
        p.aux = aux.data_ptr()
    p.M, p.N, p.K, p.batch, p.zdiv = M, N, K, batch, zdiv
    p.a_kstrided, p.b_kstrided = int(a_kstrided), int(b_kstrided)
    p.c_f32 = 1 if C.dtype == torch.float32 else 0
    p.accumulate = int(accumulate)
    p.act = _ACT[act] if not isinstance(act, int) else act
    p.lda, p.ldb, p.ldc, p.ldc2, p.ldr, p.ldaux = lda, ldb, ldc, ldc2, ldr, ldaux
    p.sA_hi, p.sA_lo = sA
    p.sB_hi, p.sB_lo = sB
    p.sC_hi, p.sC_lo = sC
    p.sR_hi, p.sR_lo = sR
    p.sX_hi, p.sX_lo = sX
    p.alpha, p.out_scale = alpha, out_scale
    thr, scale = drop_params(drop_p)
    p.drop_seed, p.drop_thr, p.drop_scale = drop_seed, thr, scale
    p.splitk = max(1, int(splitk))
    ws = None
    if p.splitk > 1:
        ws = torch.empty(p.splitk * batch * M * N, dtype=torch.float32, device=C.device)
        p.workspace = ws.data_ptr()
    if qsplit is not None:
        q_u, q_v, pos_u, pos_v, qn, ld_q, qscale = qsplit
        assert q_u.dtype == torch.bfloat16 and (q_v is None or q_v.dtype == torch.bfloat16)
        assert (pos_u is None or pos_u.dtype == torch.float32) and (pos_v is None or pos_v.dtype == torch.float32)
        p.q_u, p.q_v, p.pos_u, p.pos_v = _p(q_u), _p(q_v), _p(pos_u), _p(pos_v)
        p.qsplit_n, p.ld_q, p.qscale = int(qn), int(ld_q), float(qscale)
    check(_lib.lib().ea_gemm_bf16(ctypes.byref(p), _stream()), "ea_gemm_bf16")
    return C


def layernorm_fwd(x, gamma, beta, eps=1e-5, row_zero=None, drop_p=0.0, drop_seed=0, save_stats=True, out_f32=False):
    M, C = x.shape
    assert x.dtype == torch.bfloat16 and x.is_contiguous()
    y = torch.empty(M, C, dtype=torch.float32, device=x.device) if out_f32 else torch.empty_like(x)
    mean = torch.empty(M, dtype=torch.float32, device=x.device) if save_stats else None
    rstd = torch.empty(M, dtype=torch.float32, device=x.device) if save_stats else None
    thr, scale = drop_params(drop_p)
    fn = _lib.lib().ea_layernorm_fwd_f32out if out_f32 else _lib.lib().ea_layernorm_fwd
    check(fn(_p(x), _p(gamma), _p(beta), _p(y), _p(mean), _p(rstd), M, C, eps, _p(row_zero), drop_seed, thr, scale, _stream()),
          "ea_layernorm_fwd")
    return y, mean, rstd


def layernorm_bwd(x, dy, gamma, mean, rstd, dgamma, dbeta, row_zero=None, drop_p=0.0, drop_seed=0, dx_add=None):
    M, C = x.shape
    assert dy.is_contiguous() and dy.dtype in (torch.bfloat16, torch.float32)
    dx = torch.empty_like(x)
    thr, scale = drop_params(drop_p)
    ws = torch.empty(_lib.lib().ea_layernorm_bwd_workspace_bytes(M, C) // 4, dtype=torch.float32, device=x.device)
    fn = _lib.lib().ea_layernorm_bwd_f32dy if dy.dtype == torch.float32 else _lib.lib().ea_layernorm_bwd
    check(fn(_p(x), _p(dy), _p(gamma), _p(mean), _p(rstd), _p(dx), _p(dgamma), _p(dbeta), M, C, _p(row_zero), drop_seed, thr, scale,
             _p(dx_add), _p(ws), _stream()), "ea_layernorm_bwd")
    return dx


def cast_f32_to_bf16(src, dst=None):
    if dst is None:
        dst = torch.empty(src.shape, dtype=torch.bfloat16, device=src.device)
    check(_lib.lib().ea_cast_f32_to_bf16(_p(src), _p(dst), src.numel(), _stream()), "ea_cast_f32_to_bf16")
    return dst


def cast_f32_to_bf16_rows(src, ld_dst):
    M, N = src.shape
    assert src.dtype == torch.float32 and src.stride(1) == 1 and ld_dst >= N
    dst = torch.empty(M, ld_dst, dtype=torch.bfloat16, device=src.device)
    check(_lib.lib().ea_cast_f32_to_bf16_rows(_p(src), src.stride(0), _p(dst), ld_dst, M, N, _stream()), "ea_cast_f32_to_bf16_rows")
    return dst if ld_dst == N else dst[:, :N]


def cast_bf16_to_f32(src, dst=None):
    if dst is None:
        dst = torch.empty(src.shape, dtype=torch.float32, device=src.device)
    check(_lib.lib().ea_cast_bf16_to_f32(_p(src), _p(dst), src.numel(), _stream()), "ea_cast_bf16_to_f32")
    return dst


def scale_dropout(x, a=1.0, y=None, b=0.0, drop_p=0.0, drop_seed=0, out=None):
    assert x.dtype == torch.bfloat16 and x.is_contiguous()
    if out is None:
        out = torch.empty_like(x)
    thr, scale = drop_params(drop_p)
    check(_lib.lib().ea_scale_dropout_bf16(_p(x), _p(y), _p(out), x.numel(), a, b, drop_seed, thr, scale, _stream()),
          "ea_scale_dropout_bf16")
    return out


def colsum(X, out, M, N, ld):
    assert X.dtype == torch.bfloat16 and out.dtype == torch.float32
    check(_lib.lib().ea_colsum_bf16(_p(X), _p(out), M, N, ld, _stream()), "ea_colsum_bf16")
    return out


def colsum_ptr(X_ptr: int, out, M, N, ld):
    check(_lib.lib().ea_colsum_bf16(ctypes.c_void_p(X_ptr), _p(out), M, N, ld, _stream()), "ea_colsum_bf16")
    return out


def zero_rows(x, row_zero):
    M, C = x.shape
    check(_lib.lib().ea_zero_rows_bf16(_p(x), _p(row_zero), M, C, _stream()), "ea_zero_rows_bf16")
    return x


def relpos_q_prep(qkv, ldq, u, v, M, C, scaling, want_qv=True):
    qu = torch.empty(M, C, dtype=torch.bfloat16, device=qkv.device)
    qv = torch.empty(M, C, dtype=torch.bfloat16, device=qkv.device) if want_qv else None
    check(_lib.lib().ea_relpos_q_prep(_p(qkv), ldq, _p(u), _p(v), _p(qu), _p(qv), M, C, scaling, _stream()),
          "ea_relpos_q_prep")
    return qu, qv


def relpos_softmax_fwd(ac, bd, key_len, attn_mask, H, B, T, S, ld_ac, ld_bd, ld_p, causal=False, drop_p=0.0,
                       drop_seed=0):
    P = torch.empty(H * B * T, ld_p, dtype=torch.bfloat16, device=ac.device)
    Pd = torch.empty_like(P) if drop_p > 0 else None
    thr, scale = drop_params(drop_p)
    check(
        _lib.lib().ea_relpos_softmax_fwd(_p(ac), _p(bd), _p(key_len), _p(attn_mask), _p(P), _p(Pd), H, B, T, S, ld_ac,
                                         ld_bd, ld_p, int(causal), drop_seed, thr, scale, _stream()),
        "ea_relpos_softmax_fwd",
    )
    return P, (Pd if Pd is not None else P)


def flash_attention_supported(dh, T, S, relpos):
    return bool(_lib.lib().ea_flash_attention_supported(dh, T, S, int(relpos)))


def flash_keep_bits_buffer(H, B, T, device):
    return torch.empty(int(_lib.lib().ea_flash_keep_bits_bytes(H, B, T)) // 2, dtype=torch.int16, device=device)


def flash_attention_fwd(qu, qv, k, v, pp, key_len, H, B, T, S, ldq, ldkv, ldpp=0, causal=False, drop_p=0.0, drop_seed=0,
                        want_lse=True, want_bits=False):
    dh = 64
    out = torch.empty(B * T, H * dh, dtype=torch.bfloat16, device=qu.device)
    lse = torch.empty(H * B, T, dtype=torch.float32, device=qu.device) if want_lse else None
    thr, scale = drop_params(drop_p)
    bits = None
    if want_bits and thr and qv is not None and T == S and not causal:
        bits = flash_keep_bits_buffer(H, B, T, qu.device)
    check(
        _lib.lib().ea_flash_attention_fwd(_p(qu), _p(qv), ldq, _p(k), _p(v), ldkv, _p(pp), ldpp, _p(key_len), _p(out),
                                          H * dh, _p(lse), H, B, T, S, dh, int(causal), drop_seed, thr, scale, _p(bits), _stream()),
        "ea_flash_attention_fwd",
    )
    return (out, lse, bits) if want_bits else (out, lse)


def flash_attention_bwd(qu, qv, k, v, pp, key_len, out, dout, lse, dk, dv, H, B, T, S, ldq, ldkv, lddkv, ldpp=0, causal=False,
                        scaling=1.0, drop_p=0.0, drop_seed=0, keep_bits=None, dq=None, lddq=0):
    dh = 64
    C = H * dh
    relpos = qv is not None
    t1 = torch.empty(B * T, C, dtype=torch.bfloat16, device=qu.device)
    t2 = torch.empty_like(t1) if relpos else None
    Rp = (2 * T - 1 + 7) // 8 * 8
    dBD = torch.empty(H * B * T, Rp, dtype=torch.bfloat16, device=qu.device) if relpos else None
    D = torch.empty(H * B, T, dtype=torch.float32, device=qu.device)
    thr, scale = drop_params(drop_p)
    check(
        _lib.lib().ea_flash_attention_bwd(_p(qu), _p(qv), ldq, _p(k), _p(v), ldkv, _p(pp), ldpp, _p(key_len), _p(out), _p(dout),
                                          C, _p(lse), _p(D), _p(t1), _p(t2), C, _p(dBD), Rp, _p(dk), _p(dv), lddkv, H, B, T, S,
                                          dh, int(causal), scaling, drop_seed, thr, scale, _p(keep_bits), _p(dq), lddq,
                                          _stream()),
        "ea_flash_attention_bwd",
    )
    return t1, t2, dBD


def relpos_softmax_bwd(P, dPd, H, B, T, S, ld_p, ld_dp, ld_bd, want_bd=True, drop_p=0.0, drop_seed=0):
    dAC = torch.empty(H * B * T, ld_p, dtype=torch.bfloat16, device=P.device)
    dBD = torch.empty(H * B * T, ld_bd, dtype=torch.bfloat16, device=P.device) if want_bd else None
    thr, scale = drop_params(drop_p)
    check(
        _lib.lib().ea_relpos_softmax_bwd(_p(P), _p(dPd), _p(dAC), _p(dBD), H, B, T, S, ld_p, ld_dp, ld_bd, drop_seed,
                                         thr, scale, _stream()),
        "ea_relpos_softmax_bwd",
    )
    return dAC, dBD


def add2_strided(a, lda, b, ldb, out, ldo, M, C, out_off=0):
    check(
        _lib.lib().ea_add2_strided_bf16(_p(a), lda, _p(b), ldb, ctypes.c_void_p(out.data_ptr() + 2 * out_off), ldo, M,
                                        C, _stream()),
        "ea_add2_strided_bf16",
    )
    return out


def glu_dwconv_fwd(Y, w, B, T, C, KW, stats, causal=False):
    U = torch.empty(B * T, C, dtype=torch.bfloat16, device=Y.device)
    Z = torch.empty(B * T, C, dtype=torch.bfloat16, device=Y.device)
    name = "ea_glu_dwconv_causal_fwd" if causal else "ea_glu_dwconv_fwd"
    check(getattr(_lib.lib(), name)(_p(Y), _p(w), _p(U), _p(Z), _p(stats), B, T, C, KW, _stream()), name)
    return U, Z


def bn_finalize(stats, C, n, eps, momentum, running_mean=None, running_var=None):
    mean_rstd = torch.empty(2, C, dtype=torch.float32, device=stats.device)
    check(_lib.lib().ea_bn_finalize(_p(stats), _p(mean_rstd), _p(running_mean), _p(running_var), C, float(n), eps,
                                    momentum, _stream()), "ea_bn_finalize")
    return mean_rstd


def bn_from_running(running_mean, running_var, eps):
    C = running_mean.numel()
    mean_rstd = torch.empty(2, C, dtype=torch.float32, device=running_mean.device)
    check(_lib.lib().ea_bn_from_running(_p(running_mean), _p(running_var), _p(mean_rstd), C, eps, _stream()),
          "ea_bn_from_running")
    return mean_rstd


def bn_act_fwd(Z, mean_rstd, gamma, beta, act):
    M, C = Z.shape
    H = torch.empty_like(Z)
    check(_lib.lib().ea_bn_act_fwd(_p(Z), _p(mean_rstd), _p(gamma), _p(beta), _p(H), M, C, _ACT[act], _stream()),
          "ea_bn_act_fwd")
    return H


def conv1_bn_bwd(X, Z, dH, mean_rstd, gamma, beta, dgamma, dbeta, dW, dbias, B, T, F, CO, sy, sx, act, training=True):
    from . import functional as _F

    red = _F._pool_zeros((2, CO), torch.float32, Z.device)
    check(_lib.lib().ea_conv1_bn_bwd(_p(X), _p(Z), _p(dH), _p(mean_rstd), _p(gamma), _p(beta), _p(red), _p(dgamma), _p(dbeta), _p(dW),
                                     _p(dbias), B, T, F, CO, sy, sx, _ACT[act], int(training), _stream()), "ea_conv1_bn_bwd")


def bn_act_bwd(Z, dH, mean_rstd, gamma, beta, dgamma, dbeta, act, training=True):
    M, C = Z.shape
    from . import functional as _F

    red = _F._pool_zeros((2, C), torch.float32, Z.device)
    dZ = torch.empty_like(Z)
    check(
        _lib.lib().ea_bn_act_bwd(_p(Z), _p(dH), _p(mean_rstd), _p(gamma), _p(beta), _p(red), _p(dZ), _p(dgamma),
                                 _p(dbeta), M, C, _ACT[act], int(training), _stream()),
        "ea_bn_act_bwd",
    )
    return dZ


def glu_dwconv_bwd(dZ, Y, U, w, dw, B, T, C, KW, causal=False):
    dY = torch.empty(B * T, 2 * C, dtype=torch.bfloat16, device=Y.device)
    ws = torch.empty(int(_lib.lib().ea_dwconv_wgrad_workspace_bytes(B, T, C, KW)), dtype=torch.uint8, device=Y.device)
    name = "ea_glu_dwconv_causal_bwd" if causal else "ea_glu_dwconv_bwd"
    check(getattr(_lib.lib(), name)(_p(dZ), _p(Y), _p(U), _p(w), _p(dY), _p(dw), _p(ws), B, T, C, KW, _stream()), name)
    return dY


def conv1_fwd(X, W, bias, B, T, F, CO, sy, sx, stats):
    To, Fo = (T - 1) // sy + 1, (F - 1) // sx + 1
    Z = torch.empty(B * To * Fo, CO, dtype=torch.bfloat16, device=X.device)
    check(_lib.lib().ea_conv1_fwd(_p(X), _p(W), _p(bias), _p(Z), _p(stats), B, T, F, CO, sy, sx, _stream()),
          "ea_conv1_fwd")
    return Z


def conv1_wgrad(X, dZ, dW, dbias, B, T, F, CO, sy, sx):
    check(_lib.lib().ea_conv1_wgrad(_p(X), _p(dZ), _p(dW), _p(dbias), B, T, F, CO, sy, sx, _stream()), "ea_conv1_wgrad")


def conv3x3_fwd(X, W16, bias, B, T, F, Cin, Cout, sy, sx, stats=None):
    To, Fo = (T - 1) // sy + 1, (F - 1) // sx + 1
    Z = torch.empty((B * To * Fo, Cout), dtype=torch.bfloat16, device=X.device)
    check(_lib.lib().ea_conv3x3_fwd(_p(X), _p(W16), _p(bias), _p(Z), _p(stats), B, T, F, Cin, Cout, sy, sx, _stream()), "ea_conv3x3_fwd")
    return Z


def conv3x3_dgrad(dZ, Wd16, B, T, F, Cin, Cout, sy, sx):
    dX = torch.empty((B * T * F, Cin), dtype=torch.bfloat16, device=dZ.device)
    check(_lib.lib().ea_conv3x3_dgrad(_p(dZ), _p(Wd16), _p(dX), B, T, F, Cin, Cout, sy, sx, _stream()), "ea_conv3x3_dgrad")
    return dX


def conv3x3_wgrad(X, dZ, dW, B, T, F, Cin, Cout, sy, sx, param_layout=False):
    lib = _lib.lib()
    nb = lib.ea_conv3x3_wgrad_workspace_bytes(B, T, F, Cin, Cout, sy, sx)
    ws = torch.empty(nb, dtype=torch.uint8, device=X.device)
    fn = lib.ea_conv3x3_wgrad_param_layout if param_layout else lib.ea_conv3x3_wgrad
    check(fn(_p(X), _p(dZ), _p(dW), _p(ws), B, T, F, Cin, Cout, sy, sx, _stream()), "ea_conv3x3_wgrad")
    return dW


def im2col3x3(A, B, T, F, C, sy, sx):
    To, Fo = (T - 1) // sy + 1, (F - 1) // sx + 1
    col = torch.empty(B * To * Fo, 9 * C, dtype=torch.bfloat16, device=A.device)
    check(_lib.lib().ea_im2col3x3(_p(A), _p(col), B, T, F, C, sy, sx, _stream()), "ea_im2col3x3")
    return col


def col2im3x3(dcol, B, T, F, C, sy, sx):
    dA = torch.empty(B * T * F, C, dtype=torch.bfloat16, device=dcol.device)
    check(_lib.lib().ea_col2im3x3(_p(dcol), _p(dA), B, T, F, C, sy, sx, _stream()), "ea_col2im3x3")
    return dA


def colstats(X, stats):
    M, C = X.shape
    check(_lib.lib().ea_colstats_bf16(_p(X), _p(stats), M, C, _stream()), "ea_colstats_bf16")
    return stats


def log_softmax(x, M, V, ld):
    out = torch.empty(M, V, dtype=torch.float32, device=x.device)
    if x.dtype == torch.float32:
        check(_lib.lib().ea_log_softmax_f32(_p(x), ld, _p(out), M, V, _stream()), "ea_log_softmax_f32")
    else:
        assert x.dtype == torch.bfloat16
        check(_lib.lib().ea_log_softmax_bf16(_p(x), ld, _p(out), M, V, _stream()), "ea_log_softmax_bf16")
    return out


def ctc_loss_fwd(lprobs, targets, in_len, tgt_len, B, T, V, Lmax, blank):
    assert lprobs.dtype == torch.float32 and lprobs.is_contiguous()
    assert targets.dtype == torch.int32 and in_len.dtype == torch.int32 and tgt_len.dtype == torch.int32
    dev = lprobs.device
    nll = torch.empty(B, dtype=torch.float32, device=dev)
    ws = torch.empty(int(_lib.lib().ea_ctc_workspace_bytes(B, T, Lmax)), dtype=torch.uint8, device=dev)
    check(
        _lib.lib().ea_ctc_loss(_p(lprobs), _p(targets), _p(in_len), _p(tgt_len), _p(nll), _p(ws), B, T, V, Lmax, blank,
                               _stream()),
        "ea_ctc_loss",
    )
    return nll, ws


def ctc_loss_grad(lprobs, ws, nll, targets, in_len, tgt_len, B, T, V, Lmax, blank, ld_out=None, grad_bf16=True,
                  grad_scale=1.0, grad_scale_dev=None, zero_infinity=True):
    ld_out = V if ld_out is None else ld_out
    dl = torch.empty(B * T, ld_out, dtype=torch.bfloat16 if grad_bf16 else torch.float32, device=lprobs.device)
    check(
        _lib.lib().ea_ctc_grad(_p(lprobs), _p(ws), _p(nll), _p(targets), _p(in_len), _p(tgt_len), _p(dl), ld_out,
                               int(grad_bf16), B, T, V, Lmax, blank, grad_scale, _p(grad_scale_dev),
                               int(zero_infinity), _stream()),
        "ea_ctc_grad",
    )
    return dl


SMOOTHING = {"uniform": 0, "unigram": 1, "temporal": 2}


def label_smoothed_ce(logits, ld, target, M, V, pad_idx, eps, want_grad=True, grad_bf16=True, grad_scale=1.0,
                      grad_ld=None, smoothing="uniform", prior=None, tgt_len=0):
    assert target.dtype == torch.int32
    dev = logits.device
    out = torch.zeros(2, dtype=torch.float32, device=dev)
    dl = None
    grad_ld = V if grad_ld is None else grad_ld
    if want_grad:
        dl = torch.zeros(M, grad_ld, dtype=torch.bfloat16 if grad_bf16 else torch.float32, device=dev)
    check(
        _lib.lib().ea_label_smoothed_ce(_p(logits), ld, int(logits.dtype == torch.bfloat16), _p(target), _p(out),
                                        _p(dl), grad_ld, int(grad_bf16), M, V, pad_idx, eps, grad_scale, SMOOTHING[smoothing],
                                        _p(prior), tgt_len, _stream()),
        "ea_label_smoothed_ce",
    )
    return out, dl


def fbank_batch(wav, offsets, B, tables, cmvn_mean, cmvn_std, Tmax, nmel=80, frame_len=400, frame_shift=160,
                preemph=0.97, log_floor=1.1920928955078125e-07, want_sum=True):
    dev = wav.device
    feat = torch.empty(B, Tmax, nmel, dtype=torch.float32, device=dev)
    utt_sum = torch.zeros(B, dtype=torch.float32, device=dev) if want_sum else None
    out_len = torch.empty(B, dtype=torch.int32, device=dev)
    assert wav.dtype in (torch.float32, torch.int16)
    fn = _lib.lib().ea_fbank_batch if wav.dtype == torch.float32 else _lib.lib().ea_fbank_batch_i16
    check(
        fn(_p(wav), _p(offsets), B, _p(tables["window"]), _p(tables["twiddle"]), _p(tables["mel_start"]), _p(tables["mel_len"]),
           _p(tables["mel_woff"]), _p(tables["mel_w"]), _p(cmvn_mean), _p(cmvn_std), _p(feat), _p(utt_sum), _p(out_len), Tmax, nmel,
           frame_len, frame_shift, preemph, log_floor, _stream()),
        "ea_fbank_batch",
    )
    return feat, out_len, utt_sum


def feature_stats(feat, lengths, acc):
    B, Tmax, nmel = feat.shape
    assert acc.dtype == torch.float64 and acc.numel() == 2 * nmel + 1 and feat.dtype == torch.float32 and feat.is_contiguous()
    check(_lib.lib().ea_feature_stats(_p(feat), _p(lengths), _p(acc), B, Tmax, nmel, _stream()), "ea_feature_stats")
    return acc


def specaugment(feat, lengths, utt_sum, fmask, tmask, use_mean=True, mask_value=0.0):
    B, Tmax, nmel = feat.shape
    nf = fmask.shape[1] if fmask is not None else 0
    nt = tmask.shape[1] if tmask is not None else 0
    check(
        _lib.lib().ea_specaugment(_p(feat), _p(lengths), _p(utt_sum), _p(fmask), _p(tmask), nf, nt, B, Tmax, nmel,
                                  int(use_mean), mask_value, _stream()),
        "ea_specaugment",
    )
    return feat


def grad_sumsq(g, out):
    check(_lib.lib().ea_grad_sumsq(_p(g), g.numel(), _p(out), _stream()), "ea_grad_sumsq")
    return out


def clip_coef(sumsq, pre_scale, max_norm, coef, denom_dev=None):
    check(_lib.lib().ea_clip_coef(_p(sumsq), pre_scale, _p(denom_dev), max_norm, _p(coef), _stream()), "ea_clip_coef")
    return coef


def adam_step(p, g, m, v, p_bf16, coef, lr, beta1, beta2, eps, weight_decay, step, zero_grad=True):
    check(
        _lib.lib().ea_adam_step(_p(p), _p(g), _p(m), _p(v), _p(p_bf16), p.numel(), _p(coef), lr, beta1, beta2, eps,
                                weight_decay, step, int(zero_grad), _stream()),
        "ea_adam_step",
    )


def ctc_greedy_decode(x, in_len, B, T, V, blank, pad, ld=None, want_align=True):
    dev = x.device
    ld = x.stride(0) if ld is None else ld
    best = torch.empty(B * T, dtype=torch.int32, device=dev)
    bestv = torch.empty(B * T, dtype=torch.float32, device=dev)
    tokens = torch.empty(B, T, dtype=torch.int32, device=dev)
    align = torch.zeros(B, T, dtype=torch.int32, device=dev) if want_align else None
    out_len = torch.empty(B, dtype=torch.int32, device=dev)
    score = torch.empty(B, dtype=torch.float32, device=dev)
    check(
        _lib.lib().ea_ctc_greedy_decode(_p(x), ld, int(x.dtype == torch.bfloat16), _p(in_len), _p(best), _p(bestv), _p(tokens),
                                        _p(align), _p(out_len), _p(score), B, T, V, blank, pad, _stream()),
        "ea_ctc_greedy_decode",
    )
    return tokens, out_len, score, align


def _finish_outputs(n, nbest, max_u, device):
    return (torch.empty(n, nbest, max_u, dtype=torch.int32, device=device), torch.empty(n, nbest, dtype=torch.int32, device=device),
            torch.empty(n, nbest, dtype=torch.float32, device=device), torch.empty(n, dtype=torch.int32, device=device))


def _partial_outputs(n, max_u, device):
    return (torch.empty(n, max_u, dtype=torch.int32, device=device), torch.empty(n, dtype=torch.int32, device=device),
            torch.empty(n, dtype=torch.float32, device=device), torch.empty(n, dtype=torch.int32, device=device))


def _stream_state(bytes_fn, max_streams, max_frames, beam, device):
    nbytes = int(bytes_fn(max_frames, beam))
    assert nbytes > 0 and max_streams >= 1
    return torch.zeros(max_streams, nbytes, dtype=torch.uint8, device=device), nbytes


def _check_stream_state(state, bytes_fn, max_frames, beam):
    assert state.dtype == torch.uint8 and state.is_contiguous() and state.dim() == 2
    assert state.shape[1] == bytes_fn(max_frames, beam)


def _check_rnnt_step_args(logits, out, lm_rows, N, V, lm_no_blank):
    assert logits.dtype == torch.float32 and logits.dim() == 2 and logits.stride(1) == 1 and logits.shape[0] == N and logits.shape[1] >= V
    parent, token, keep = out
    assert parent.numel() == token.numel() == keep.numel() == N
    assert parent.dtype == token.dtype == torch.int32 and keep.dtype == torch.uint8
    if lm_rows is not None:
        assert lm_rows.dtype == torch.float32 and lm_rows.stride(1) == 1 and lm_rows.shape == (N, V - 1 if lm_no_blank else V)
    return parent, token, keep


def ctc_prefix_beam_workspace(B, T, beam, device):
    return torch.empty(int(_lib.lib().ea_ctc_prefix_beam_workspace_bytes(B, T, beam)), dtype=torch.uint8, device=device)


def ctc_prefix_beam_step(x, in_len, ws, B, T, V, beam, K, blank, t0, t1, lm_rows=None, lm_weight=0.0, ins_bonus=0.0, lm_out=None,
                         ld=None):
    ld = x.stride(0) if ld is None else ld
    assert x.dtype in (torch.float32, torch.bfloat16) and x.stride(-1) == 1 and x.shape[0] == B * T and x.shape[1] == V
    assert in_len.dtype == torch.int32 and in_len.numel() == B and ws.numel() >= _lib.lib().ea_ctc_prefix_beam_workspace_bytes(B, T, beam)
    parent, token, keep = lm_out if lm_out is not None else (None, None, None)
    if lm_rows is not None:
        assert lm_rows.dtype == torch.float32 and lm_rows.stride(1) == 1 and lm_rows.shape == (B * beam, V) and t1 == t0 + 1
        assert parent.numel() == token.numel() == keep.numel() == B * beam
        assert parent.dtype == token.dtype == torch.int32 and keep.dtype == torch.uint8
    check(_lib.lib().ea_ctc_prefix_beam_step(_p(x), ld, int(x.dtype == torch.bfloat16), _p(in_len), _p(ws), _p(lm_rows),
                                             lm_rows.stride(0) if lm_rows is not None else 0, _p(parent), _p(token), _p(keep), B, T,
                                             V, beam, K, blank, lm_weight, ins_bonus, t0, t1, _stream()), "ea_ctc_prefix_beam_step")


def ctc_prefix_beam_finish(ws, B, T, beam, nbest, pad, lm_rows=None, lm_weight=0.0, ins_bonus=0.0, eos=-1):
    dev = ws.device
    tokens, lengths, scores, nhyp = _finish_outputs(B, nbest, T, dev)
    check(_lib.lib().ea_ctc_prefix_beam_finish(_p(ws), _p(lm_rows), lm_rows.stride(0) if lm_rows is not None else 0, lm_weight,
                                               ins_bonus, eos, B, T, beam, nbest, pad, _p(tokens), _p(lengths), _p(scores),
                                               _p(nhyp), _stream()), "ea_ctc_prefix_beam_finish")
    return tokens, lengths, scores, nhyp


def _cg(graph, V=None):
    nodes, edges, root = graph
    assert nodes.dtype == edges.dtype == root.dtype == torch.int32 and nodes.is_contiguous() and edges.is_contiguous() and root.is_contiguous()
    assert nodes.dim() == 2 and nodes.shape[1] == 4 and nodes.shape[0] >= 1 and tuple(edges.shape) == (nodes.shape[0] - 1, 4)
    assert root.dim() == 2 and root.shape[1] == 2 and (V is None or root.shape[0] == V), "context graph built for another vocabulary"
    return _p(nodes), (_p(edges) if edges.numel() else None), _p(root), nodes.shape[0], edges.shape[0]


def ctc_prefix_beam_bias_workspace(B, T, beam, device):
    return torch.empty(int(_lib.lib().ea_ctc_prefix_beam_bias_workspace_bytes(B, T, beam)), dtype=torch.uint8, device=device)


def ctc_prefix_beam_bias_step(x, in_len, ws, graph, B, T, V, beam, K, blank, t0, t1, lm_rows=None, lm_weight=0.0, ins_bonus=0.0,
                              lm_out=None, ld=None):
    ld = x.stride(0) if ld is None else ld
    assert x.dtype in (torch.float32, torch.bfloat16) and x.stride(-1) == 1 and x.shape[0] == B * T and x.shape[1] == V
    assert in_len.dtype == torch.int32 and in_len.numel() == B
    assert ws.numel() >= _lib.lib().ea_ctc_prefix_beam_bias_workspace_bytes(B, T, beam)
    parent, token, keep = lm_out if lm_out is not None else (None, None, None)
    if lm_rows is not None:
        assert lm_rows.dtype == torch.float32 and lm_rows.stride(1) == 1 and lm_rows.shape == (B * beam, V) and t1 == t0 + 1
        assert parent.numel() == token.numel() == keep.numel() == B * beam
        assert parent.dtype == token.dtype == torch.int32 and keep.dtype == torch.uint8
    check(_lib.lib().ea_ctc_prefix_beam_bias_step(_p(x), ld, int(x.dtype == torch.bfloat16), _p(in_len), _p(ws), _p(lm_rows),
                                                  lm_rows.stride(0) if lm_rows is not None else 0, _p(parent), _p(token), _p(keep),
                                                  *_cg(graph, V), B, T, V, beam, K, blank, lm_weight, ins_bonus, t0, t1, _stream()),
          "ea_ctc_prefix_beam_bias_step")


def ctc_prefix_beam_bias_finish(ws, graph, B, T, beam, nbest, pad, lm_rows=None, lm_weight=0.0, ins_bonus=0.0, eos=-1):
    dev = ws.device
    tokens, lengths, scores, nhyp = _finish_outputs(B, nbest, T, dev)
# ... 939 lines not shown
```

include/espresso_amd.h:

```cpp
#ifndef ESPRESSO_AMD_H
#define ESPRESSO_AMD_H

#include <stdint.h>

#ifdef __cplusplus
extern "C" {
#endif

typedef struct ihipStream_t* ea_stream_t;

int ea_version(void);

enum { EA_ACT_NONE = 0, EA_ACT_RELU = 1, EA_ACT_SILU = 2 };

typedef struct EaGemmParams {
  const void* A;
  const void* B;
  void* C;
  void* C2;
  const float* bias;
  const void* resid;
  const void* aux;
  int M, N, K, batch, zdiv;
  int a_kstrided, b_kstrided, c_f32, accumulate, resid_f32, act;
  long lda, ldb, ldc, ldc2, ldr, ldaux;
  long sA_hi, sA_lo, sB_hi, sB_lo, sC_hi, sC_lo, sR_hi, sR_lo, sX_hi, sX_lo;
  float alpha, out_scale;
  uint64_t drop_seed;
  uint32_t drop_thr;
  float drop_scale;
  int splitk, kchunk;
  void* workspace;
  void* q_u;
  void* q_v;
  const float* pos_u;
  const float* pos_v;
  long ld_q;
  int qsplit_n;
  float qscale;
} EaGemmParams;

int ea_gemm_bf16(const EaGemmParams* p, ea_stream_t stream);
long ea_gemm_splitk_workspace_bytes(int M, int N, int batch, int splitk);
int ea_set_gemm_variant(int v);
int ea_set_gemm_xcd_swizzle(int mask);
int ea_set_gemm_glds(int stages);
long ea_set_gemm_nt_store_min_bytes(long bytes);
int ea_set_gemm_w8(int mode);
int ea_gemm_profile_enable(int on);
long ea_gemm_profile_read(double* total_ms, double* total_flops);
int ea_gemm_profile_bytes(double* total_bytes);
long ea_gemm_profile_dump(const char* path);

#define EA_WGRAD_MAX 16
typedef struct EaWgradProblem {
  const void* dy;
  const void* x;
  float* dW;
  float* dbias;
  int M, N, K;
  long ld_dy, ld_x, ldw;
} EaWgradProblem;
typedef struct EaWgradGroup {
  int count;
  EaWgradProblem p[EA_WGRAD_MAX];
} EaWgradGroup;
int ea_wgrad_group(const EaWgradGroup* group, ea_stream_t stream);
int ea_set_wgrad_transposing_reads(int on);
int ea_set_wgrad_w8(int mode);

int ea_layernorm_fwd(const void* x, const float* gamma, const float* beta, void* y, float* mean, float* rstd,
                     int M, int C, float eps, const uint8_t* row_zero, uint64_t drop_seed, uint32_t drop_thr,
                     float drop_scale, ea_stream_t stream);
int ea_layernorm_fwd_f32out(const void* x, const float* gamma, const float* beta, float* y, float* mean, float* rstd,
                            int M, int C, float eps, const uint8_t* row_zero, uint64_t drop_seed, uint32_t drop_thr,
                            float drop_scale, ea_stream_t stream);
int ea_layernorm_bwd_f32dy(const void* x, const float* dy, const float* gamma, const float* mean, const float* rstd,
                           void* dx, float* dgamma, float* dbeta, int M, int C, const uint8_t* row_zero,
                           uint64_t drop_seed, uint32_t drop_thr, float drop_scale, const void* dx_add,
                           void* workspace, ea_stream_t stream);
long ea_layernorm_bwd_workspace_bytes(int M, int C);
int ea_layernorm_bwd(const void* x, const void* dy, const float* gamma, const float* mean, const float* rstd,
                     void* dx, float* dgamma, float* dbeta, int M, int C, const uint8_t* row_zero,
                     uint64_t drop_seed, uint32_t drop_thr, float drop_scale, const void* dx_add,
                     void* workspace, ea_stream_t stream);
int ea_layernorm_bwd_dx(const void* x, const void* dy, const float* gamma, const float* mean, const float* rstd, void* dx,
                        float* dgamma, float* dbeta, int M, int C, const uint8_t* row_zero, uint64_t drop_seed,
                        uint32_t drop_thr, float drop_scale, const void* dx_add, void* workspace, ea_stream_t stream);
int ea_layernorm_param_reduce(const void* workspace, float* dgamma, float* dbeta, int M, int C, ea_stream_t stream);
#define EA_LNRED_MAX 8
typedef struct EaLnReduceItem { const void* workspace; float* dgamma; float* dbeta; int M, C; } EaLnReduceItem;
typedef struct EaLnReduceGroup { int count; EaLnReduceItem item[EA_LNRED_MAX]; } EaLnReduceGroup;
int ea_layernorm_param_reduce_group(const EaLnReduceGroup* group, ea_stream_t stream);
int ea_layernorm_bwd_dx2(const void* x, const void* dy, const float* gamma, const float* mean, const float* rstd, void* dx,
                         float* dgamma, float* dbeta, int M, int C, const void* dx_add, void* workspace, void* out2, float a2,
                         uint64_t seed2, uint32_t thr2, float scale2, ea_stream_t stream);
int ea_layernorm_fwd2(const void* x, const float* g1, const float* b1, void* y1, float* mean1, float* rstd1, const float* g2,
                      const float* b2, void* y2, float* mean2, float* rstd2, int M, int C, float eps, ea_stream_t stream);
int ea_layernorm_bwd2_dx(const void* x1, const void* dy1, const float* gamma1, const float* mean1, const float* rstd1,
                         const void* dx_add, void* ws1, const void* x2, const float* gamma2, const float* mean2, const float* rstd2,
                         void* ws2, void* dx, int M, int C, void* out2, float a2, uint64_t seed2, uint32_t thr2, float scale2,
                         ea_stream_t stream);

int ea_cast_f32_to_bf16(const float* src, void* dst, long n, ea_stream_t stream);
int ea_transpose_bf16_batch(const void* const* src, void* const* dst, const int* rows, const int* cols, int n, ea_stream_t stream);
int ea_audio_probe(const char* path, long* num_samples, int* sample_rate, int* channels, int* bits);
long ea_audio_read_i16(const char* path, int16_t* dst, long capacity, int* sample_rate);
int ea_audio_verify(const char* path);
int ea_audio_read_batch_i16(const char* const* paths, int n, int16_t* dst, const long* offsets, int num_threads, long* lengths,
                            int* sample_rates);

int ea_cast_f32_to_bf16_rows(const float* src, long ld_src, void* dst, long ld_dst, long M, int N, ea_stream_t stream);
int ea_cast_bf16_to_f32(const void* src, float* dst, long n, ea_stream_t stream);
int ea_scale_dropout_bf16(const void* x, const void* y, void* out, long n, float a, float b, uint64_t seed,
                          uint32_t thr, float inv_keep, ea_stream_t stream);
int ea_colsum_bf16(const void* X, float* out, int M, int N, long ld, ea_stream_t stream);
int ea_embedding_fwd(const int* tokens, const int* positions, const float* W, const float* pos_table, void* out, int M,
                     int C, float scale, ea_stream_t stream);
int ea_embedding_bwd(const int* tokens, const void* dy, float* dW, int M, int C, float scale, int pad_idx,
                     ea_stream_t stream);
int ea_zero_rows_bf16(void* x, const uint8_t* row_zero, int M, int C, ea_stream_t stream);

int ea_flash_attention_supported(int dh, int T, int S, int relpos);
int ea_flash_attention_fwd(const void* qu, const void* qv, long ldq, const void* k, const void* v, long ldkv,
                           const void* pp, long ldpp, const int* key_len, void* out, long ldo, float* lse, int H, int B,
                           int T, int S, int dh, int causal, uint64_t drop_seed, uint32_t drop_thr, float drop_scale,
                           void* keep_bits, ea_stream_t stream);
long ea_flash_keep_bits_bytes(int H, int B, int T);
int ea_set_flash_relpos(int on);
int ea_flash_keep_bits(void* keep_bits, int H, int B, int T, uint64_t drop_seed, uint32_t drop_thr, ea_stream_t stream);
int ea_flash_attention_bwd(const void* qu, const void* qv, long ldq, const void* k, const void* v, long ldkv,
                           const void* pp, long ldpp, const int* key_len, const void* out, const void* dout, long ldo,
                           const float* lse, float* D, void* t1, void* t2, long ldt, void* dBD, int ld_bd, void* dk,
                           void* dv, long lddkv, int H, int B, int T, int S, int dh, int causal, float scaling,
                           uint64_t drop_seed, uint32_t drop_thr, float drop_scale, const void* keep_bits,
                           void* dq, long lddq, ea_stream_t stream);

int ea_relpos_q_prep(const void* qkv, long ldq, const float* u, const float* v, void* qu, void* qv, int M,
                     int C, float scaling, ea_stream_t stream);
int ea_relpos_softmax_fwd(const float* ac, const float* bd, const int* key_len, const float* attn_mask, void* P,
                          void* Pd, int H, int B, int T, int S, int ld_ac, int ld_bd, int ld_p, int causal,
                          uint64_t drop_seed, uint32_t drop_thr, float drop_scale, ea_stream_t stream);
int ea_relpos_softmax_bwd(const void* P, const float* dPd, void* dAC, void* dBD, int H, int B, int T, int S,
                          int ld_p, int ld_dp, int ld_bd, uint64_t drop_seed, uint32_t drop_thr,
                          float drop_scale, ea_stream_t stream);
int ea_add2_strided_bf16(const void* a, long lda, const void* b, long ldb, void* out, long ldo, int M, int C,
                         ea_stream_t stream);

int ea_glu_dwconv_fwd(const void* Y, const float* w, void* U, void* Z, double* stats, int B, int T, int C, int KW,
                      ea_stream_t stream);
int ea_bn_finalize(const double* stats, float* mean_rstd, float* running_mean, float* running_var, int C, float n,
                   float eps, float momentum, ea_stream_t stream);
int ea_bn_from_running(const float* running_mean, const float* running_var, float* mean_rstd, int C, float eps,
                       ea_stream_t stream);
int ea_bn_act_fwd(const void* Z, const float* mean_rstd, const float* gamma, const float* beta, void* H, long M,
                  int C, int act, ea_stream_t stream);
int ea_bn_act_bwd(const void* Z, const void* dH, const float* mean_rstd, const float* gamma, const float* beta,
                  float* red, void* dZ, float* dgamma, float* dbeta, long M, int C, int act, int training,
                  ea_stream_t stream);
long ea_dwconv_wgrad_workspace_bytes(int B, int T, int C, int KW);
int ea_glu_dwconv_bwd(const void* dZ, const void* Y, const void* U, const float* w, void* dY, float* dw,
                      void* wgrad_ws, int B, int T, int C, int KW, ea_stream_t stream);
int ea_dwconv_bwd_weight(const void* dZ, const void* U, float* dw, void* wgrad_ws, int B, int T, int C, int KW, ea_stream_t stream);
int ea_glu_dwconv_causal_fwd(const void* Y, const float* w, void* U, void* Z, double* stats, int B, int T, int C, int KW,
                             ea_stream_t stream);
int ea_glu_dwconv_causal_bwd(const void* dZ, const void* Y, const void* U, const float* w, void* dY, float* dw,
                             void* wgrad_ws, int B, int T, int C, int KW, ea_stream_t stream);
int ea_dwconv_causal_bwd_weight(const void* dZ, const void* U, float* dw, void* wgrad_ws, int B, int T, int C, int KW,
                                ea_stream_t stream);
int ea_bn_act_fwd_train(const void* Z, const double* stats, float* mean_rstd, float* running_mean, float* running_var,
                        const float* gamma, const float* beta, void* H, long M, int C, int act, float n, float eps,
                        float momentum, double* zero_next, int zero_n, ea_stream_t stream);
int ea_bn_act_bwd_fused(const void* Z, const void* dH, const float* mean_rstd, const float* gamma, const float* beta,
                        float* red, void* dZ, float* dgamma, float* dbeta, long M, int C, int act, int training,
                        float* zero_next, int zero_n, ea_stream_t stream);
int ea_bn_param_grad(const float* red, float* dgamma, float* dbeta, int C, ea_stream_t stream);
int ea_conv1_bn_bwd(const float* X, const void* Z, const void* dH, const float* mean_rstd, const float* gamma, const float* beta,
                    float* red, float* dgamma, float* dbeta, float* dW, float* dbias, int B, int T, int F, int CO, int sy, int sx,
                    int act, int training, ea_stream_t stream);

int ea_conv1_fwd(const float* X, const float* W, const float* bias, void* Z, double* stats, int B, int T, int F,
                 int CO, int sy, int sx, ea_stream_t stream);
int ea_conv1_wgrad(const float* X, const void* dZ, float* dW, float* dbias, int B, int T, int F, int CO, int sy,
                   int sx, ea_stream_t stream);
int ea_conv3x3_fwd(const void* X, const void* W, const float* bias, void* Z, double* stats, int B, int T, int F, int Cin,
                   int Cout, int sy, int sx, ea_stream_t stream);
int ea_conv3x3_dgrad(const void* dZ, const void* Wd, void* dX, int B, int T, int F, int Cin, int Cout, int sy, int sx,
                     ea_stream_t stream);
long ea_conv3x3_wgrad_workspace_bytes(int B, int T, int F, int Cin, int Cout, int sy, int sx);
int ea_conv3x3_wgrad(const void* X, const void* dZ, float* dW, void* workspace, int B, int T, int F, int Cin, int Cout, int sy,
                     int sx, ea_stream_t stream);
int ea_conv3x3_wgrad_param_layout(const void* X, const void* dZ, float* dW, void* workspace, int B, int T, int F, int Cin, int Cout,
                                  int sy, int sx, ea_stream_t stream);
int ea_im2col3x3(const void* A, void* col, int B, int T, int F, int C, int sy, int sx, ea_stream_t stream);
int ea_col2im3x3(const void* dcol, void* dA, int B, int T, int F, int C, int sy, int sx, ea_stream_t stream);
int ea_colstats_bf16(const void* X, double* stats, long M, int C, ea_stream_t stream);

int ea_log_softmax_f32(const float* in, long ld_in, float* out, long M, int V, ea_stream_t stream);
int ea_log_softmax_bf16(const void* in, long ld_in, float* out, long M, int V, ea_stream_t stream);
long ea_ctc_workspace_bytes(int B, int T, int Lmax);
int ea_ctc_loss(const float* lprobs, const int* targets, const int* in_len, const int* tgt_len, float* nll,
                void* workspace, int B, int T, int V, int Lmax, int blank, ea_stream_t stream);
int ea_ctc_grad(const float* lprobs, const void* workspace, const float* nll, const int* targets,
                const int* in_len, const int* tgt_len, void* dlogits, long ld_out, int dlogits_bf16, int B, int T,
                int V, int Lmax, int blank, float grad_scale, const float* grad_scale_dev, int zero_infinity,
                ea_stream_t stream);
int ea_ctc_greedy_decode(const void* x, long ld, int x_bf16, const int* in_len, int* best, float* bestv, int* tokens,
                         int* align, int* out_len, float* score, int B, int T, int V, int blank, int pad,
                         ea_stream_t stream);
long ea_ctc_prefix_beam_workspace_bytes(int B, int T, int beam);
int ea_ctc_prefix_beam_step(const void* x, long ld, int x_bf16, const int* in_len, void* workspace, const float* lm_rows,
                            long ld_lm, int* lm_parent, int* lm_token, void* lm_keep, int B, int T, int V, int beam, int K,
                            int blank, float lm_weight, float ins_bonus, int t0, int t1, ea_stream_t stream);
int ea_ctc_prefix_beam_finish(void* workspace, const float* lm_rows, long ld_lm, float lm_weight, float ins_bonus, int eos,
                              int B, int T, int beam, int nbest, int pad, int* tokens, int* lengths, float* scores, int* nhyp,
                              ea_stream_t stream);
long ea_ctc_prefix_beam_bias_workspace_bytes(int B, int T, int beam);
int ea_ctc_prefix_beam_bias_step(const void* x, long ld, int x_bf16, const int* in_len, void* workspace, const float* lm_rows,
                                 long ld_lm, int* lm_parent, int* lm_token, void* lm_keep, const int* cg_nodes,
                                 const int* cg_edges, const int* cg_root, int cg_n_nodes, int cg_n_edges, int B, int T, int V,
                                 int beam, int K, int blank, float lm_weight, float ins_bonus, int t0, int t1, ea_stream_t stream);
int ea_ctc_prefix_beam_bias_finish(void* workspace, const float* lm_rows, long ld_lm, float lm_weight, float ins_bonus, int eos,
                                   const int* cg_nodes, int cg_n_nodes, int B, int T, int beam, int nbest, int pad, int* tokens,
                                   int* lengths, float* scores, int* nhyp, ea_stream_t stream);
int ea_context_graph_score_host(const int* nodes_host, const int* edges_host, const int* root_host, int n_nodes, int n_edges,
                                int V, const int* tokens_host, const int* lens_host, int N, int L, float* running_host,
                                float* final_host, int* q_host);
int ea_context_graph_score(const int* nodes, const int* edges, const int* root, int n_nodes, int n_edges, int V,
                           const int* tokens, const int* lens, int N, int L, float* running, float* final_bias, int* q_out,
                           ea_stream_t stream);
long ea_ctc_prefix_beam_stream_state_bytes(int max_frames, int beam);
int ea_ctc_prefix_beam_stream_reset(void* state, const int* slots, int n, int max_streams, int max_frames, int beam,
                                    ea_stream_t stream);
int ea_ctc_prefix_beam_stream_step(const void* x, long ld, int x_bf16, long total_rows, const int* slot_idx, const int* n_new,
                                   const int* row_off, int j0, int j1, int n, void* state, const float* lm_rows, long ld_lm,
                                   int* lm_parent, int* lm_token, void* lm_keep, const int* cg_nodes, const int* cg_edges,
                                   const int* cg_root, int cg_n_nodes, int cg_n_edges, int max_streams, int max_frames, int V,
                                   int beam, int K, int blank, float lm_weight, float ins_bonus, ea_stream_t stream);
int ea_ctc_prefix_beam_stream_finish(const void* state, const int* slots, int n, const float* lm_rows, long ld_lm, float lm_weight,
                                     float ins_bonus, int eos, const int* cg_nodes, int cg_n_nodes, int max_streams,
                                     int max_frames, int beam, int nbest, int pad, int max_u, int* tokens, int* lengths,
                                     float* scores, int* nhyp, ea_stream_t stream);
int ea_ctc_prefix_beam_stream_partial(const void* state, const int* slots, int n, float lm_weight, float ins_bonus, int biased,
                                      int max_streams, int max_frames, int beam, int pad, int max_u, int* tokens, int* lengths,
                                      float* scores, int* stable_len, ea_stream_t stream);
long ea_ctc_prefix_beam_times_workspace_bytes(int B, int T, int beam);
int ea_ctc_prefix_beam_times_step(const void* x, long ld, int x_bf16, const int* in_len, void* workspace, void* times_workspace,
                                  const float* lm_rows, long ld_lm, int* lm_parent, int* lm_token, void* lm_keep,
                                  const int* cg_nodes, const int* cg_edges, const int* cg_root, int cg_n_nodes, int cg_n_edges,
                                  int B, int T, int V, int beam, int K, int blank, float lm_weight, float ins_bonus, int t0, int t1,
                                  ea_stream_t stream);
int ea_ctc_prefix_beam_times_finish(void* workspace, const void* times_workspace, const float* lm_rows, long ld_lm, float lm_weight,
                                    float ins_bonus, int eos, const int* cg_nodes, int cg_n_nodes, int B, int T, int beam,
                                    int nbest, int pad, int* tokens, int* lengths, float* scores, int* nhyp, int* times,
                                    float* vscores, ea_stream_t stream);
long ea_ctc_prefix_beam_stream_times_state_bytes(int max_frames, int beam);
int ea_ctc_prefix_beam_stream_times_reset(void* state, void* times_state, const int* slots, int n, int max_streams, int max_frames,
                                          int beam, ea_stream_t stream);
int ea_ctc_prefix_beam_stream_times_step(const void* x, long ld, int x_bf16, long total_rows, const int* slot_idx, const int* n_new,
                                         const int* row_off, int j0, int j1, int n, void* state, void* times_state,
                                         const float* lm_rows, long ld_lm, int* lm_parent, int* lm_token, void* lm_keep,
                                         const int* cg_nodes, const int* cg_edges, const int* cg_root, int cg_n_nodes,
                                         int cg_n_edges, int max_streams, int max_frames, int V, int beam, int K, int blank,
                                         float lm_weight, float ins_bonus, ea_stream_t stream);
int ea_ctc_prefix_beam_stream_times_finish(const void* state, const void* times_state, const int* slots, int n, const float* lm_rows,
                                           long ld_lm, float lm_weight, float ins_bonus, int eos, const int* cg_nodes,
                                           int cg_n_nodes, int max_streams, int max_frames, int beam, int nbest, int pad, int max_u,
                                           int* tokens, int* lengths, float* scores, int* nhyp, int* times, float* vscores,
                                           ea_stream_t stream);
int ea_ctc_prefix_beam_stream_endpoint(const void* state, const void* times_state, const int* slots, int n, float lm_weight,
                                       float ins_bonus, int biased, int max_streams, int max_frames, int beam, int silence_frames,
                                       int empty_frames, int segment_frames, int* out, ea_stream_t stream);
long ea_rnnt_frame_beam_workspace_bytes(int B, int T, int beam);
int ea_rnnt_frame_beam_step(const float* logits, long ld, const float* lm_rows, long ld_lm, int lm_no_blank, const int* in_len,
                            void* workspace, int* parent, int* token, void* keep, int B, int T, int V, int beam, int K, int blank,
                            int eos, float temperature, float lm_weight, int t, ea_stream_t stream);
int ea_rnnt_frame_beam_finish(void* workspace, int B, int T, int beam, int nbest, int pad, int normalize, int* tokens,
                              int* lengths, float* scores, int* nhyp, ea_stream_t stream);
long ea_rnnt_frame_beam_stream_state_bytes(int max_frames, int beam);
int ea_rnnt_frame_beam_stream_reset(void* state, const int* slots, int n, int max_streams, int max_frames, int beam,
                                    ea_stream_t stream);
int ea_rnnt_frame_beam_stream_step(const float* logits, long ld, const float* lm_rows, long ld_lm, int lm_no_blank,
                                   const int* slot_idx, const int* n_new, int j, int n, void* state, int* parent, int* token,
                                   void* keep, int max_streams, int max_frames, int V, int beam, int K, int blank, int eos,
                                   float temperature, float lm_weight, ea_stream_t stream);
int ea_rnnt_frame_beam_stream_finish(const void* state, const int* slots, int n, int max_streams, int max_frames, int beam,
                                     int nbest, int pad, int normalize, int max_u, int* tokens, int* lengths, float* scores,
                                     int* nhyp, ea_stream_t stream);
int ea_rnnt_frame_beam_stream_partial(const void* state, const int* slots, int n, int max_streams, int max_frames, int beam,
                                      int pad, int max_u, int* tokens, int* lengths, float* scores, int* stable_len,
                                      ea_stream_t stream);
long ea_rnnt_frame_beam_bias_workspace_bytes(int B, int T, int beam);
int ea_rnnt_frame_beam_bias_step(const float* logits, long ld, const float* lm_rows, long ld_lm, int lm_no_blank, const int* in_len,
                                 void* workspace, int* parent, int* token, void* keep, const int* cg_nodes, const int* cg_edges,
                                 const int* cg_root, int cg_n_nodes, int cg_n_edges, int B, int T, int V, int beam, int K, int blank,
                                 int eos, float temperature, float lm_weight, int t, ea_stream_t stream);
int ea_rnnt_frame_beam_bias_finish(void* workspace, const int* cg_nodes, int cg_n_nodes, int B, int T, int beam, int nbest, int pad,
                                   int normalize, int* tokens, int* lengths, float* scores, int* nhyp, ea_stream_t stream);
long ea_rnnt_frame_beam_stream_bias_state_bytes(int max_frames, int beam);
int ea_rnnt_frame_beam_stream_bias_reset(void* state, const int* slots, int n, int max_streams, int max_frames, int beam,
                                         ea_stream_t stream);
int ea_rnnt_frame_beam_stream_bias_step(const float* logits, long ld, const float* lm_rows, long ld_lm, int lm_no_blank,
                                        const int* slot_idx, const int* n_new, int j, int n, void* state, int* parent, int* token,
                                        void* keep, const int* cg_nodes, const int* cg_edges, const int* cg_root, int cg_n_nodes,
                                        int cg_n_edges, int max_streams, int max_frames, int V, int beam, int K, int blank, int eos,
                                        float temperature, float lm_weight, ea_stream_t stream);
int ea_rnnt_frame_beam_stream_bias_finish(const void* state, const int* slots, int n, int max_streams, int max_frames, int beam,
                                          const int* cg_nodes, int cg_n_nodes, int nbest, int pad, int normalize, int max_u,
                                          int* tokens, int* lengths, float* scores, int* nhyp, ea_stream_t stream);
int ea_rnnt_frame_beam_stream_bias_partial(const void* state, const int* slots, int n, int max_streams, int max_frames, int beam,
                                           int pad, int max_u, int* tokens, int* lengths, float* scores, int* stable_len,
                                           ea_stream_t stream);
long ea_rnnt_frame_beam_times_workspace_bytes(int B, int T, int beam);
int ea_rnnt_frame_beam_times_step(const float* logits, long ld, const float* lm_rows, long ld_lm, int lm_no_blank, const int* in_len,
                                  void* workspace, void* times_workspace, int* parent, int* token, void* keep, const int* cg_nodes,
                                  const int* cg_edges, const int* cg_root, int cg_n_nodes, int cg_n_edges, int B, int T, int V,
                                  int beam, int K, int blank, int eos, float temperature, float lm_weight, int t, ea_stream_t stream);
int ea_rnnt_frame_beam_times_finish(void* workspace, const void* times_workspace, const int* cg_nodes, int cg_n_nodes, int B, int T,
                                    int beam, int nbest, int pad, int normalize, int* tokens, int* lengths, float* scores, int* nhyp,
                                    int* times, float* vscores, ea_stream_t stream);
long ea_rnnt_frame_beam_stream_times_state_bytes(int max_frames, int beam);
int ea_rnnt_frame_beam_stream_times_reset(void* state, void* times_state, const int* slots, int n, int biased, int max_streams,
                                          int max_frames, int beam, ea_stream_t stream);
int ea_rnnt_frame_beam_stream_times_step(const float* logits, long ld, const float* lm_rows, long ld_lm, int lm_no_blank,
                                         const int* slot_idx, const int* n_new, int j, int n, void* state, void* times_state,
                                         int* parent, int* token, void* keep, const int* cg_nodes, const int* cg_edges,
                                         const int* cg_root, int cg_n_nodes, int cg_n_edges, int max_streams, int max_frames, int V,
                                         int beam, int K, int blank, int eos, float temperature, float lm_weight, ea_stream_t stream);
int ea_rnnt_frame_beam_stream_times_finish(const void* state, const void* times_state, const int* slots, int n, int max_streams,
                                           int max_frames, int beam, const int* cg_nodes, int cg_n_nodes, int nbest, int pad,
                                           int normalize, int max_u, int* tokens, int* lengths, float* scores, int* nhyp, int* times,
                                           float* vscores, ea_stream_t stream);
int ea_rnnt_frame_beam_stream_endpoint(const void* state, const void* times_state, const int* slots, int n, int biased,
                                       int max_streams, int max_frames, int beam, int silence_frames, int empty_frames,
                                       int segment_frames, int* out, ea_stream_t stream);
int ea_ngram_create(const char* path, void* handle_host, char* err_host, long err_cap);
int ea_ngram_destroy(void* handle);
int ea_ngram_info(const void* handle, int* meta_host, long* counts_host);
long ea_ngram_vocab(const void* handle, char* buf_host, long cap);
long ea_ngram_records(const void* handle, int order, int* ngrams_host, float* logp_host, float* bow_host);
int ea_ngram_upload(void* handle);
int ea_ngram_score_host(const void* handle, const int* ctx_host, const int* words_host, int N, float* out_host);
int ea_ngram_score(const void* handle, const int* ctx, const int* words, int N, float* out, ea_stream_t stream);
long ea_ctc_lexicon_beam_workspace_bytes(int B, int T, int beam);
int ea_ctc_lexicon_beam_search(const void* x, long ld, int x_bf16, const int* in_len, void* workspace, const void* ngram,
                               const int* trie_off, const int* trie_tok, const int* trie_child, const int* trie_word,
                               const float* trie_smear, const void* word_start, int space, int B, int T, int V, int beam, int K,
                               int blank, float lm_weight, float word_score, float ins_bonus, int nbest, int pad, int* tokens,
                               int* lengths, float* scores, int* nhyp, ea_stream_t stream);
long ea_ctc_lexicon_stream_state_bytes(int max_frames, int beam);
int ea_ctc_lexicon_stream_reset(void* state, const int* slots, int n, const void* ngram, int max_streams, int max_frames,
                                int beam, ea_stream_t stream);
int ea_ctc_lexicon_stream_step(const void* x, long ld, int x_bf16, long total_rows, const int* slot_idx, const int* n_new,
                               const int* row_off, int n, void* state, const void* ngram, const int* trie_off,
                               const int* trie_tok, const int* trie_child, const int* trie_word, const float* trie_smear,
                               const void* word_start, int space, int max_streams, int max_frames, int V, int beam, int K,
                               int blank, float lm_weight, float word_score, float ins_bonus, ea_stream_t stream);
int ea_ctc_lexicon_stream_finish(const void* state, const int* slots, int n, const void* ngram, const int* trie_word,
                                 const float* trie_smear, int max_streams, int max_frames, int beam, float lm_weight,
                                 float word_score, float ins_bonus, int nbest, int pad, int max_u, int* tokens, int* lengths,
                                 float* scores, int* nhyp, ea_stream_t stream);
int ea_ctc_lexicon_stream_partial(const void* state, const int* slots, int n, int max_streams, int max_frames, int beam,
                                  float ins_bonus, int pad, int max_u, int* tokens, int* lengths, float* scores, int* stable_len,
                                  ea_stream_t stream);
int ea_ngram_token_map_create(const void* handle, const int* tok2word_host, int V, void* map_host);
int ea_ngram_token_map_destroy(void* map);
int ea_ngram_token_rows_step(const void* handle, const void* tok2word, int V, const int* ctx_in, const int* parent,
                             const int* token, const void* keep, int N, int* ctx_out, float* rows, long ld, ea_stream_t stream);
int ea_ngram_token_rows_start(const void* handle, const void* tok2word, int V, int N, int* ctx, float* rows, long ld,
                              ea_stream_t stream);
int ea_ngram_token_rows_host(const void* handle, const int* tok2word_host, int V, const int* ctx_in_host, const int* parent_host,
                             const int* token_host, const void* keep_host, int N, int* ctx_out_host, float* rows_host, long ld);
int ea_label_smoothed_ce(const void* logits, long ld, int logits_bf16, const int* target, float* out_loss,
                         void* dlogits, long ld_out, int dlogits_bf16, long M, int V, int pad_idx, float eps,
                         float grad_scale, int smoothing, const float* prior, int tgt_len, ea_stream_t stream);

int ea_fbank_batch(const float* wav, const long* offsets, int B, const float* window, const float* twiddle,
                   const int* mel_start, const int* mel_len, const int* mel_woff, const float* mel_w,
                   const float* cmvn_mean, const float* cmvn_std, float* feat, float* utt_sum, int* out_len,
                   int Tmax, int nmel, int frame_len, int frame_shift, float preemph, float log_floor,
                   ea_stream_t stream);
int ea_fbank_batch_i16(const int16_t* wav, const long* offsets, int B, const float* window, const float* twiddle,
                   const int* mel_start, const int* mel_len, const int* mel_woff, const float* mel_w,
                   const float* cmvn_mean, const float* cmvn_std, float* feat, float* utt_sum, int* out_len,
                   int Tmax, int nmel, int frame_len, int frame_shift, float preemph, float log_floor,
                   ea_stream_t stream);
int ea_specaugment(float* feat, const int* lengths, const float* utt_sum, const int* fmask, const int* tmask,
                   int nf, int nt, int B, int Tmax, int nmel, int use_mean, float mask_value, ea_stream_t stream);

int ea_feature_stats(const float* feat, const int* lengths, double* acc, int B, int Tmax, int nmel, ea_stream_t stream);

int ea_grad_sumsq(const float* g, long n, float* out, ea_stream_t stream);
int ea_clip_coef(const float* sumsq, float pre_scale, const float* denom_dev, float max_norm, float* coef,
                 ea_stream_t stream);
int ea_adam_step(float* p, float* g, float* m, float* v, void* p_bf16, long n, const float* coef, float lr,
                 float beta1, float beta2, float eps, float weight_decay, int step, int zero_grad,
                 ea_stream_t stream);

typedef struct EaFfnParams { const float *ln_g, *ln_b; const void* w1; const float* b1; const void* w2; const float* b2; } EaFfnParams;
typedef struct EaFfnGrads { float *ln_g, *ln_b, *w1, *b1, *w2, *b2; } EaFfnGrads;
typedef struct EaAttnParams {
  const float *ln_g, *ln_b; const void* wqkv; const float* bqkv; const void* wo; const float* bo;
  const float *pos_u, *pos_v; const void* wpos;
} EaAttnParams;
typedef struct EaAttnGrads { float *ln_g, *ln_b, *wqkv, *bqkv, *wo, *bo, *pos_u, *pos_v, *wpos; } EaAttnGrads;
typedef struct EaConvParams {
  const float *ln_g, *ln_b; const void* pw1; const float* dw; const float *bn_g, *bn_b; float *bn_rm, *bn_rv; const void* pw2;
} EaConvParams;
typedef struct EaConvGrads { float *ln_g, *ln_b, *pw1, *dw, *bn_g, *bn_b, *pw2; } EaConvGrads;
typedef struct EaLayerGrads { EaFfnGrads ffn1; EaAttnGrads attn; EaConvGrads conv; EaFfnGrads ffn2; float *final_ln_g, *final_ln_b; } EaLayerGrads;
typedef struct EaConformerLayer {
  EaFfnParams ffn1; EaAttnParams attn; EaConvParams conv; EaFfnParams ffn2; const float *final_ln_g, *final_ln_b;
  EaLayerGrads grads;
  void* wt;
} EaConformerLayer;
typedef struct EaLayerShape {
  int B, T, C, H, F, KW, training; float p_drop, p_act, p_attn; uint64_t seed; int has_attn_mask;
  int scratch_clean;
  int pos_mode, act;
  int S;
  int defer;
  int wt_fresh;
  int conv_causal;
} EaLayerShape;

enum {
  EA_SITE_FFN1_ACT = 0, EA_SITE_FFN1_OUT = 1, EA_SITE_ATTN_PROBS = 2, EA_SITE_ATTN_OUT = 3, EA_SITE_CONV_OUT = 4,
  EA_SITE_FFN2_ACT = 5, EA_SITE_FFN2_OUT = 6, EA_SITE_CROSS_PROBS = 7, EA_SITE_CROSS_OUT = 8
};
uint64_t ea_layer_dropout_seed(uint64_t layer_seed, int site);
int ea_dropout_hash_host(uint64_t seed, uint64_t idx0, long n, uint32_t* out);

int ea_set_backward_overlap(int on);
int ea_set_backward_deferred(int on);
int ea_set_backward_deferred_inline(int on);
int ea_backward_flush(ea_stream_t stream);
int ea_streams_share_queue(ea_stream_t a, ea_stream_t b);
int ea_side_stream_report(int* rejected, int* unprobed);
int ea_conformer_layer_workspace(const EaLayerShape* shape, long* saved_bytes, long* scratch_bytes);
int ea_conformer_layer_refresh_wt(const EaConformerLayer* layer, const EaLayerShape* shape, ea_stream_t stream);
int ea_conformer_layer_fwd(const EaConformerLayer* layer, const EaLayerShape* shape, const void* x_in, void* x_out,
                           const int* key_len, const float* attn_mask, const void* pe, void* saved, long saved_bytes,
                           void* scratch, long scratch_bytes, ea_stream_t stream);
int ea_conformer_layer_bwd(const EaConformerLayer* layer, const EaLayerShape* shape, const void* x_in, const void* dy,
                           void* dx, const int* key_len, const void* pe, void* saved, long saved_bytes, void* scratch,
                           long scratch_bytes, ea_stream_t stream);
typedef struct EaLayerChain {
  const EaConformerLayer* next; void* next_saved; long next_saved_bytes; int ln1_done;
  const EaConformerLayer* prev; void* prev_saved; long prev_saved_bytes; uint64_t prev_seed; void* prev_pre;
  int final_ln_done; const void* pre_in;
} EaLayerChain;
int ea_conformer_layer_fwd_chained(const EaConformerLayer* layer, const EaLayerShape* shape, const EaLayerChain* chain, const void* x_in,
                                   void* x_out, const int* key_len, const float* attn_mask, const void* pe, void* saved,
                                   long saved_bytes, void* scratch, long scratch_bytes, ea_stream_t stream);
int ea_conformer_layer_bwd_chained(const EaConformerLayer* layer, const EaLayerShape* shape, const EaLayerChain* chain, const void* x_in,
                                   const void* dy, void* dx, const int* key_len, const void* pe, void* saved, long saved_bytes,
                                   void* scratch, long scratch_bytes, ea_stream_t stream);
typedef struct EaStackLayer { const EaConformerLayer* layer; EaLayerShape shape; void* saved; long saved_bytes; void* x_in; } EaStackLayer;
int ea_conformer_stack_fwd(const EaStackLayer* L, int n, void* x_out, const int* key_len, const float* attn_mask, const void* pe,
                           void* scratch, long scratch_bytes, int chain, ea_stream_t stream);
int ea_conformer_stack_bwd(const EaStackLayer* L, int n, const void* dy, void* dx, void* const* dbuf, void* const* pre,
                           const int* key_len, const void* pe, void* scratch, long scratch_bytes, int chain, ea_stream_t stream);
int ea_transformer_layer_workspace(const EaLayerShape* shape, long* saved_bytes, long* scratch_bytes);
int ea_transformer_layer_fwd(const EaConformerLayer* layer, const EaLayerShape* shape, const void* x_in, void* x_out,
                             const int* key_len, const float* attn_mask, const void* pe, void* saved, long saved_bytes,
                             void* scratch, long scratch_bytes, ea_stream_t stream);
int ea_transformer_layer_bwd(const EaConformerLayer* layer, const EaLayerShape* shape, const void* x_in, const void* dy,
                             void* dx, const int* key_len, const void* pe, float* dpe, void* saved, long saved_bytes,
                             void* scratch, long scratch_bytes, ea_stream_t stream);
typedef struct EaXAttnParams { const float *ln_g, *ln_b; const void* wq; const float* bq; const void* wkv; const float* bkv; const void* wo; const float* bo; } EaXAttnParams;
typedef struct EaXAttnGrads { float *ln_g, *ln_b, *wq, *bq, *wkv, *bkv, *wo, *bo; } EaXAttnGrads;
typedef struct EaDecoderLayer {
  EaAttnParams self_attn; EaXAttnParams cross; EaFfnParams ffn;
  EaAttnGrads g_self; EaXAttnGrads g_cross; EaFfnGrads g_ffn;
  void* wt;
} EaDecoderLayer;
int ea_decoder_layer_workspace(const EaLayerShape* shape, long* saved_bytes, long* scratch_bytes);
int ea_decoder_layer_fwd(const EaDecoderLayer* layer, const EaLayerShape* shape, const void* x_in, const void* enc, void* x_out,
// ... 116 lines not shown
```

Before: 5.356 audio-hours/sec.

## Fuse subsample dropout/row-zero into BN epilogues and merge strided dgrad launches

Strided conv3x3 dgrad now runs one launch that covers every output phase class. Each workgroup looks up its phase class from a prefix table, and classes with more taps are ordered first. Separately, the subsampling output dropout and padded-row zeroing are folded into the BN+ReLU forward kernel and into the BN backward reduce/apply kernels. This removes separate elementwise passes and a clone over the subsample output and its gradient. The cost is recomputing the dropout mask in both backward kernels, plus extra per-block class lookup logic.

Measured after the change: 5.386 audio-hours/sec (median of 6 runs). No clear change (+0.6%).

```diff
diff --git a/espresso_amd/csrc/conv_igemm.hip b/espresso_amd/csrc/conv_igemm.hip
--- a/espresso_amd/csrc/conv_igemm.hip
+++ b/espresso_amd/csrc/conv_igemm.hip
@@ -23,9 +23,14 @@
   long ldw;
   int OT, OF, ot_mul, ot_add, of_mul, of_add;
 };
-
-template <int BN_>
-__global__ __launch_bounds__(256, 2) void conv_gather_kernel(const ConvGatherArgs a) {
+struct ConvGatherClasses {
+  int ncls;
+  int wg0[5];
+  int RT[4], RF[4], tap0[4], ntaps[4], ot_add[4], of_add[4];
+};
+
+template <int BN_, bool MULTI>
+__global__ __launch_bounds__(256, 2) void conv_gather_kernel(const ConvGatherArgs a, const ConvGatherClasses k) {
   constexpr int BM_ = 128, NST = 2;
   constexpr int NJ = BN_ / 32;
   constexpr int A_BYTES = BM_ * ROW_BYTES, STAGE = A_BYTES + BN_ * ROW_BYTES;
@@ -33,10 +38,18 @@
   extern __shared__ __attribute__((aligned(16))) char dsm[];
   const int tid = threadIdx.x, lane = tid & 63, wave = tid >> 6;
   const int wm = wave >> 1, wcol = (wave & 1) * (BN_ / 2);
-  const uint32_t M = (uint32_t)a.RB * a.RT * a.RF;
-  const uint32_t m0 = blockIdx.x * BM_;
+  int RT = a.RT, RF = a.RF, tap0 = 0, ntaps = a.ntaps, ot_add = a.ot_add, of_add = a.of_add;
+  uint32_t wg = blockIdx.x;
+  if constexpr (MULTI) {
+    int c = 0;
+    while (c + 1 < k.ncls && (int)blockIdx.x >= k.wg0[c + 1]) ++c;
+    RT = k.RT[c]; RF = k.RF[c]; tap0 = k.tap0[c]; ntaps = k.ntaps[c]; ot_add = k.ot_add[c]; of_add = k.of_add[c];
+    wg = blockIdx.x - (uint32_t)k.wg0[c];
+  }
+  const uint32_t M = (uint32_t)a.RB * RT * RF;
+  const uint32_t m0 = wg * BM_;
   const int cpt = a.SC / BK;
-  const int nk = a.ntaps * cpt;
+  const int nk = ntaps * cpt;
 
   int rowb[NA], rowt[NA], rowf[NA];
   int cs[NA];
@@ -46,8 +59,8 @@
     cs[i] = (lane & 7) ^ (r & 7) ^ ((r >> 4) & 7);
     const uint32_t p = m0 + r;
     if (p < M) {
-      const uint32_t q = p / (uint32_t)a.RF, b = q / (uint32_t)a.RT;
-      const int rf = (int)(p - q * a.RF), rt = (int)(q - b * a.RT);
+      const uint32_t q = p / (uint32_t)RF, b = q / (uint32_t)RT;
+      const int rf = (int)(p - q * RF), rt = (int)(q - b * RT);
       rowb[i] = (int)b * a.ST;
       rowt[i] = rt * a.at;
       rowf[i] = rf * a.af;
@@ -64,7 +77,8 @@
     bp[i] = a.W + (long)min(r, a.N - 1) * a.ldw + c * 8;
   }
   auto issue = [&](int stage, int kt) {
-    const int tap = kt / cpt, chunk = kt - tap * cpt;
+    const int ktap = kt / cpt, chunk = kt - ktap * cpt;
+    const int tap = tap0 + ktap;
     const int dt = a.bt[tap], df = a.bf[tap];
     const long ko = a.koff[tap] + chunk * BK;
     char* base = dsm + stage * STAGE + wave * 1024;
@@ -146,9 +160,9 @@
       const int rl = pass * RL + rlane;
       const uint32_t p = m0 + half * 64 + rl;
       if (p < M) {
-        const uint32_t q = p / (uint32_t)a.RF, b = q / (uint32_t)a.RT;
-        const int rf = (int)(p - q * a.RF), rt = (int)(q - b * a.RT);
-        const long orow = ((long)b * a.OT + (long)rt * a.ot_mul + a.ot_add) * a.OF + (long)rf * a.of_mul + a.of_add;
+        const uint32_t q = p / (uint32_t)RF, b = q / (uint32_t)RT;
+        const int rf = (int)(p - q * RF), rt = (int)(q - b * RT);
+        const long orow = ((long)b * a.OT + (long)rt * a.ot_mul + ot_add) * a.OF + (long)rf * a.of_mul + of_add;
         const float4 x0 = *reinterpret_cast<const float4*>(sC + rl * BN_ + cg * 8);
         const float4 x1 = *reinterpret_cast<const float4*>(sC + rl * BN_ + cg * 8 + 4);
         float v[8] = {x0.x, x0.y, x0.z, x0.w, x1.x, x1.y, x1.z, x1.w};
@@ -200,13 +214,34 @@
 template <int BN_>
 int launch_gather(const ConvGatherArgs& a, hipStream_t stream) {
   constexpr int bytes = 2 * (128 + BN_) * ROW_BYTES;
-  static bool attr_ok = hipFuncSetAttribute(reinterpret_cast<const void*>(&conv_gather_kernel<BN_>),
+  static bool attr_ok = hipFuncSetAttribute(reinterpret_cast<const void*>(&conv_gather_kernel<BN_, false>),
                                             hipFuncAttributeMaxDynamicSharedMemorySize, bytes) == hipSuccess;
   if (!attr_ok) return -1;
   const long M = (long)a.RB * a.RT * a.RF;
   if (M <= 0) return 0;
   if (M >= (1L << 31) - 128) return -1;
-  hipLaunchKernelGGL((conv_gather_kernel<BN_>), dim3((unsigned)((M + 127) / 128)), dim3(256), bytes, stream, a);
+  hipLaunchKernelGGL((conv_gather_kernel<BN_, false>), dim3((unsigned)((M + 127) / 128)), dim3(256), bytes, stream, a,
+                     ConvGatherClasses{});
+  return EA_CHECK_LAUNCH();
+}
+
+template <int BN_>
+int launch_gather_classes(const ConvGatherArgs& a, ConvGatherClasses k, hipStream_t stream) {
+  constexpr int bytes = 2 * (128 + BN_) * ROW_BYTES;
+  static bool attr_ok = hipFuncSetAttribute(reinterpret_cast<const void*>(&conv_gather_kernel<BN_, true>),
+                                            hipFuncAttributeMaxDynamicSharedMemorySize, bytes) == hipSuccess;
+  if (!attr_ok) return -1;
+  long wgs = 0;
+  for (int c = 0; c < k.ncls; ++c) {
+    const long M = (long)a.RB * k.RT[c] * k.RF[c];
+    if (M <= 0 || M >= (1L << 31) - 128) return -1;
+    k.wg0[c] = (int)wgs;
+    wgs += (M + 127) / 128;
+    if (wgs >= (1L << 31) - 1) return -1;
+  }
+  if (k.ncls <= 0) return 0;
+  k.wg0[k.ncls] = (int)wgs;
+  hipLaunchKernelGGL((conv_gather_kernel<BN_, true>), dim3((unsigned)wgs), dim3(256), bytes, stream, a, k);
   return EA_CHECK_LAUNCH();
 }
 
@@ -454,30 +489,50 @@
   const int To = (T - 1) / sy + 1, Fo = (F - 1) / sx + 1;
   const bf16_t* zero = zero_line(stream);
   if (!zero) return -1;
+  ConvGatherArgs a;
+  a.src = (const bf16_t*)dZ; a.W = (const bf16_t*)Wd; a.out = (bf16_t*)dX; a.bias = nullptr; a.stats = nullptr; a.zero = zero;
+  a.RB = B; a.RT = 0; a.RF = 0;
+  a.ST = To; a.SF = Fo; a.SC = Cout;
+  a.at = 1; a.af = 1;
+  a.ntaps = 0;
+  a.N = Cin; a.ldw = 9L * Cout;
+  a.OT = T; a.OF = F; a.ot_mul = sy; a.ot_add = 0; a.of_mul = sx; a.of_add = 0;
+  struct Cls { int RT, RF, tap0, ntaps, pt, pf; } cls[4];
+  int ncls = 0;
   for (int pt = 0; pt < sy; ++pt)
     for (int pf = 0; pf < sx; ++pf) {
-      ConvGatherArgs a;
-      a.src = (const bf16_t*)dZ; a.W = (const bf16_t*)Wd; a.out = (bf16_t*)dX; a.bias = nullptr; a.stats = nullptr; a.zero = zero;
-      a.RB = B; a.RT = (T - pt + sy - 1) / sy; a.RF = (F - pf + sx - 1) / sx;
-      a.ST = To; a.SF = Fo; a.SC = Cout;
-      a.at = 1; a.af = 1;
-      a.ntaps = 0;
+      Cls c;
+      c.RT = (T - pt + sy - 1) / sy; c.RF = (F - pf + sx - 1) / sx;
+      c.tap0 = a.ntaps; c.ntaps = 0; c.pt = pt; c.pf = pf;
       for (int ky = 0; ky < 3; ++ky) {
         if ((pt + 1 - ky) % sy) continue;
         for (int kx = 0; kx < 3; ++kx) {
           if ((pf + 1 - kx) % sx) continue;
           const int t = a.ntaps++;
+          ++c.ntaps;
           a.bt[t] = (pt + 1 - ky) / sy; a.bf[t] = (pf + 1 - kx) / sx; a.koff[t] = (ky * 3 + kx) * Cout;
         }
       }
-      a.N = Cin; a.ldw = 9L * Cout;
-      a.OT = T; a.OF = F; a.ot_mul = sy; a.ot_add = pt; a.of_mul = sx; a.of_add = pf;
-      if (a.RT <= 0 || a.RF <= 0) continue;
-      if (a.ntaps == 0) return -2;
-      const int rc = Cin == 128 ? launch_gather<128>(a, stream) : launch_gather<64>(a, stream);
-      if (rc) return rc;
-    }
-  return 0;
+      if (c.ntaps == 0) return -2;
+      if (c.RT <= 0 || c.RF <= 0) continue;
+      cls[ncls++] = c;
+    }
+  if (ncls == 1) {
+    a.RT = cls[0].RT; a.RF = cls[0].RF; a.ot_add = cls[0].pt; a.of_add = cls[0].pf;
+    a.ntaps = cls[0].ntaps;
+    return Cin == 128 ? launch_gather<128>(a, stream) : launch_gather<64>(a, stream);
+  }
+  ConvGatherClasses k{};
+  for (int n = 0; n < ncls; ++n) {
+    int best = -1;
+    for (int c = 0; c < ncls; ++c)
+      if (cls[c].ntaps >= 0 && (best < 0 || cls[c].ntaps > cls[best].ntaps)) best = c;
+    k.RT[n] = cls[best].RT; k.RF[n] = cls[best].RF; k.tap0[n] = cls[best].tap0; k.ntaps[n] = cls[best].ntaps;
+    k.ot_add[n] = cls[best].pt; k.of_add[n] = cls[best].pf;
+    cls[best].ntaps = -1;
+  }
+  k.ncls = ncls;
+  return Cin == 128 ? launch_gather_classes<128>(a, k, stream) : launch_gather_classes<64>(a, k, stream);
 }
 
 extern "C" long ea_conv3x3_wgrad_workspace_bytes(int B, int T, int F, int Cin, int Cout, int sy, int sx) {
diff --git a/espresso_amd/csrc/convmodule.hip b/espresso_amd/csrc/convmodule.hip
--- a/espresso_amd/csrc/convmodule.hip
+++ b/espresso_amd/csrc/convmodule.hip
@@ -212,12 +212,35 @@
   }
 }
 
+struct BnPost {
+  const uint8_t* row_zero;
+  int ppf;
+  uint64_t seed;
+  uint32_t thr;
+  float inv_keep;
+};
+__device__ __forceinline__ uint4 bn_post8(const uint4 x, long m, int C, int ch, const BnPost& p) {
+  if (p.row_zero && p.row_zero[m / p.ppf]) return make_uint4(0, 0, 0, 0);
+  if (!p.thr) return x;
+  float k8[8], o[8];
+  ea_keep8(p.seed, (uint64_t)(m * C + ch * 8), p.thr, p.inv_keep, k8);
+  const uint32_t w[4] = {x.x, x.y, x.z, x.w};
+#pragma unroll
+  for (int e = 0; e < 8; ++e) {
+    const float v = (e & 1) ? __uint_as_float(w[e >> 1] & 0xffff0000u) : __uint_as_float(w[e >> 1] << 16);
+    o[e] = v * k8[e] + 0.f;
+  }
+  uint4 r;
+  r.x = pack_bf2(o[0], o[1]); r.y = pack_bf2(o[2], o[3]); r.z = pack_bf2(o[4], o[5]); r.w = pack_bf2(o[6], o[7]);
+  return r;
+}
+template <bool POST>
 __global__ __launch_bounds__(256) void bn_act_fwd_stats_kernel(const bf16_t* __restrict__ Z, const double* __restrict__ stats,
                                                                float* __restrict__ mean_rstd, float* __restrict__ running_mean,
                                                                float* __restrict__ running_var, const float* __restrict__ gamma,
                                                                const float* __restrict__ beta, bf16_t* __restrict__ Hout, long M,
                                                                int C, int act, float n, float eps, float momentum,
-                                                               double* __restrict__ zero_next, int zero_n) {
+                                                               double* __restrict__ zero_next, int zero_n, const BnPost post) {
   extern __shared__ float s_scsh[];
   const int nch = C >> 3;
   const long total = M * nch;
@@ -264,17 +287,19 @@
     }
     uint4 r;
     r.x = pack_bf2(o[0], o[1]); r.y = pack_bf2(o[2], o[3]); r.z = pack_bf2(o[4], o[5]); r.w = pack_bf2(o[6], o[7]);
+    if constexpr (POST) r = bn_post8(r, m, C, ch, post);
     *reinterpret_cast<uint4*>(Hout + m * C + ch * 8) = r;
   }
   if (zero_next)
     for (long i = gtid; i < zero_n; i += stride) zero_next[i] = 0.0;
 }
 
+template <bool POST>
 __global__ __launch_bounds__(256) void bn_act_bwd_reduce_kernel(const bf16_t* __restrict__ Z, const bf16_t* __restrict__ dH,
                                                                 const float* __restrict__ mean_rstd,
                                                                 const float* __restrict__ gamma, const float* __restrict__ beta,
                                                                 float* __restrict__ red, long M, int C, int act,
-                                                                int rows_per_block, int TCH) {
+                                                                int rows_per_block, int TCH, const BnPost post) {
   extern __shared__ float sm[];
   const int nch = C >> 3;
   const int cx = threadIdx.x % TCH, ry = threadIdx.x / TCH, lanes = 256 / TCH;
@@ -312,13 +337,15 @@
       for (int r = 0; r < R; ++r) {
         uz[r] = *reinterpret_cast<const uint4*>(Z + (m + (long)r * lanes) * C + ch * 8);
         ud[r] = *reinterpret_cast<const uint4*>(dH + (m + (long)r * lanes) * C + ch * 8);
+        if constexpr (POST) ud[r] = bn_post8(ud[r], m + (long)r * lanes, C, ch, post);
       }
 #pragma unroll
       for (int r = 0; r < R; ++r) accum(uz[r], ud[r]);
     }
     for (; m < r1; m += lanes) {
       const uint4 uz = *reinterpret_cast<const uint4*>(Z + m * C + ch * 8);
-      const uint4 ud = *reinterpret_cast<const uint4*>(dH + m * C + ch * 8);
+      uint4 ud = *reinterpret_cast<const uint4*>(dH + m * C + ch * 8);
+      if constexpr (POST) ud = bn_post8(ud, m, C, ch, post);
       accum(uz, ud);
     }
   }
@@ -336,13 +363,14 @@
   }
 }
 
+template <bool POST>
 __global__ __launch_bounds__(256) void bn_act_bwd_apply_kernel(const bf16_t* __restrict__ Z, const bf16_t* __restrict__ dH,
                                                                const float* __restrict__ mean_rstd,
                                                                const float* __restrict__ gamma, const float* __restrict__ beta,
                                                                const float* __restrict__ red, bf16_t* __restrict__ dZ,
                                                                long M, int C, int act, float n,
-                                                               float* __restrict__ dgamma = nullptr, float* __restrict__ dbeta = nullptr,
-                                                               float* __restrict__ zero_next = nullptr, int zero_n = 0) {
+                                                               float* __restrict__ dgamma, float* __restrict__ dbeta,
+                                                               float* __restrict__ zero_next, int zero_n, const BnPost post) {
   const int nch = C >> 3;
   const long total = M * nch;
   const float invn = n > 0.f ? 1.f / n : 0.f;
@@ -367,7 +395,8 @@
   for (long i = (long)blockIdx.x * blockDim.x + threadIdx.x; i < total; i += stride) {
     const long m = i / nch;
     const uint4 uz = *reinterpret_cast<const uint4*>(Z + m * C + ch * 8);
-    const uint4 ud = *reinterpret_cast<const uint4*>(dH + m * C + ch * 8);
+    uint4 ud = *reinterpret_cast<const uint4*>(dH + m * C + ch * 8);
+    if constexpr (POST) ud = bn_post8(ud, m, C, ch, post);
     const uint32_t wz[4] = {uz.x, uz.y, uz.z, uz.w}, wd[4] = {ud.x, ud.y, ud.z, ud.w};
     float o[8];
 #pragma unroll
@@ -691,8 +720,19 @@
                                    float momentum, double* zero_next, int zero_n, hipStream_t stream) {
   if (M <= 0) return 0;
   if (C % 8) return -2;
-  hipLaunchKernelGGL(bn_act_fwd_stats_kernel, dim3(egrid_ch(M * (C / 8), C / 8)), dim3(256), (size_t)2 * C * sizeof(float), stream, (const bf16_t*)Z, stats,
-                     mean_rstd, running_mean, running_var, gamma, beta, (bf16_t*)H, M, C, act, n, eps, momentum, zero_next, zero_n);
+  hipLaunchKernelGGL(bn_act_fwd_stats_kernel<false>, dim3(egrid_ch(M * (C / 8), C / 8)), dim3(256), (size_t)2 * C * sizeof(float), stream, (const bf16_t*)Z, stats,
+                     mean_rstd, running_mean, running_var, gamma, beta, (bf16_t*)H, M, C, act, n, eps, momentum, zero_next, zero_n, BnPost{});
+  return EA_CHECK_LAUNCH();
+}
+extern "C" int ea_bn_act_fwd_train_post(const void* Z, const double* stats, float* mean_rstd, float* running_mean, float* running_var,
+                                        const float* gamma, const float* beta, void* H, long M, int C, int act, float n, float eps,
+                                        float momentum, double* zero_next, int zero_n, const uint8_t* row_zero, int rows_per_flag,
+                                        uint64_t drop_seed, uint32_t drop_thr, float drop_scale, hipStream_t stream) {
+  if (M <= 0) return 0;
+  if (C % 8 || (row_zero && (rows_per_flag < 1 || M % rows_per_flag))) return -2;
+  const BnPost post{row_zero, rows_per_flag, drop_seed, drop_thr, drop_scale};
+  hipLaunchKernelGGL(bn_act_fwd_stats_kernel<true>, dim3(egrid_ch(M * (C / 8), C / 8)), dim3(256), (size_t)2 * C * sizeof(float), stream, (const bf16_t*)Z, stats,
+                     mean_rstd, running_mean, running_var, gamma, beta, (bf16_t*)H, M, C, act, n, eps, momentum, zero_next, zero_n, post);
   return EA_CHECK_LAUNCH();
 }
 
@@ -843,7 +883,7 @@
 }
 
 static void launch_bn_bwd_reduce(const void* Z, const void* dH, const float* mean_rstd, const float* gamma, const float* beta,
-                                 float* red, long M, int C, int act, hipStream_t stream);
+                                 float* red, long M, int C, int act, hipStream_t stream, const BnPost* post = nullptr);
 
 extern "C" int ea_bn_act_bwd(const void* Z, const void* dH, const float* mean_rstd, const float* gamma,
                              const float* beta, float* red, void* dZ, float* dgamma, float* dbeta, long M, int C,
@@ -851,9 +891,9 @@
   if (M <= 0) return 0;
   if (C % 8) return -2;
   launch_bn_bwd_reduce(Z, dH, mean_rstd, gamma, beta, red, M, C, act, stream);
-  hipLaunchKernelGGL(bn_act_bwd_apply_kernel, dim3(egrid_ch(M * (C / 8), C / 8)), dim3(256), 0, stream, (const bf16_t*)Z,
+  hipLaunchKernelGGL(bn_act_bwd_apply_kernel<false>, dim3(egrid_ch(M * (C / 8), C / 8)), dim3(256), 0, stream, (const bf16_t*)Z,
                      (const bf16_t*)dH, mean_rstd, gamma, beta, red, (bf16_t*)dZ, M, C, act,
-                     training ? (float)M : 0.f);
+                     training ? (float)M : 0.f, (float*)nullptr, (float*)nullptr, (float*)nullptr, 0, BnPost{});
   if (dgamma || dbeta) hipLaunchKernelGGL(bn_param_grad_kernel, dim3((C + 255) / 256), dim3(256), 0, stream, red, dgamma, dbeta, C);
   return EA_CHECK_LAUNCH();
 }
@@ -864,9 +904,22 @@
   if (M <= 0) return 0;
   if (C % 8) return -2;
   launch_bn_bwd_reduce(Z, dH, mean_rstd, gamma, beta, red, M, C, act, stream);
-  hipLaunchKernelGGL(bn_act_bwd_apply_kernel, dim3(egrid_ch(M * (C / 8), C / 8)), dim3(256), 0, stream, (const bf16_t*)Z,
+  hipLaunchKernelGGL(bn_act_bwd_apply_kernel<false>, dim3(egrid_ch(M * (C / 8), C / 8)), dim3(256), 0, stream, (const bf16_t*)Z,
                      (const bf16_t*)dH, mean_rstd, gamma, beta, red, (bf16_t*)dZ, M, C, act, training ? (float)M : 0.f, dgamma, dbeta,
-                     zero_next, zero_n);
+                     zero_next, zero_n, BnPost{});
+  return EA_CHECK_LAUNCH();
+}
+extern "C" int ea_bn_act_bwd_fused_post(const void* Z, const void* dOut, const float* mean_rstd, const float* gamma, const float* beta,
+                                        float* red, void* dZ, float* dgamma, float* dbeta, long M, int C, int act, int training,
+                                        float* zero_next, int zero_n, const uint8_t* row_zero, int rows_per_flag, uint64_t drop_seed,
+                                        uint32_t drop_thr, float drop_scale, hipStream_t stream) {
+  if (M <= 0) return 0;
+  if (C % 8 || (row_zero && (rows_per_flag < 1 || M % rows_per_flag))) return -2;
+  const BnPost post{row_zero, rows_per_flag, drop_seed, drop_thr, drop_scale};
+  launch_bn_bwd_reduce(Z, dOut, mean_rstd, gamma, beta, red, M, C, act, stream, &post);
+  hipLaunchKernelGGL(bn_act_bwd_apply_kernel<true>, dim3(egrid_ch(M * (C / 8), C / 8)), dim3(256), 0, stream, (const bf16_t*)Z,
+                     (const bf16_t*)dOut, mean_rstd, gamma, beta, red, (bf16_t*)dZ, M, C, act, training ? (float)M : 0.f, dgamma, dbeta,
+                     zero_next, zero_n, post);
   return EA_CHECK_LAUNCH();
 }
 
@@ -888,7 +941,7 @@
 }
 
 static void launch_bn_bwd_reduce(const void* Z, const void* dH, const float* mean_rstd, const float* gamma, const float* beta,
-                                 float* red, long M, int C, int act, hipStream_t stream) {
+                                 float* red, long M, int C, int act, hipStream_t stream, const BnPost* post) {
   const int nch = C / 8;
   int TCH = 1;
   while (TCH < 256 && TCH < nch) TCH <<= 1;
@@ -899,8 +952,12 @@
   const long want = (M + (2048 / gx) - 1) / (2048 / gx > 0 ? 2048 / gx : 1);
   if (want > rpb) rpb = (int)((want + lanes - 1) / lanes * lanes);
   dim3 g1((unsigned)gx, (unsigned)((M + rpb - 1) / rpb));
-  hipLaunchKernelGGL(bn_act_bwd_reduce_kernel, g1, dim3(256), (size_t)256 * 16 * sizeof(float), stream, (const bf16_t*)Z,
-                     (const bf16_t*)dH, mean_rstd, gamma, beta, red, M, C, act, rpb, TCH);
+  if (post)
+    hipLaunchKernelGGL(bn_act_bwd_reduce_kernel<true>, g1, dim3(256), (size_t)256 * 16 * sizeof(float), stream, (const bf16_t*)Z,
+                       (const bf16_t*)dH, mean_rstd, gamma, beta, red, M, C, act, rpb, TCH, *post);
+  else
+    hipLaunchKernelGGL(bn_act_bwd_reduce_kernel<false>, g1, dim3(256), (size_t)256 * 16 * sizeof(float), stream, (const bf16_t*)Z,
+                       (const bf16_t*)dH, mean_rstd, gamma, beta, red, M, C, act, rpb, TCH, BnPost{});
 }
 extern "C" int ea_bn_param_grad(const float* red, float* dgamma, float* dbeta, int C, hipStream_t stream) {
   hipLaunchKernelGGL(bn_param_grad_kernel, dim3((C + 255) / 256), dim3(256), 0, stream, red, dgamma, dbeta, C);
diff --git a/espresso_amd/functional.py b/espresso_amd/functional.py
--- a/espresso_amd/functional.py
+++ b/espresso_amd/functional.py
@@ -697,6 +697,8 @@
         cfgs = []
         A = None
         Tc, Fc, Cc = T, F, 1
+        seed = _next_seed("subsample.out", p_drop) if (training and p_drop > 0) else 0
+        post_done = False
         for i in range(L):
             w, b, g, beta = params[4 * i: 4 * i + 4]
             rm, rv = bufs[2 * i], bufs[2 * i + 1]
@@ -720,17 +722,23 @@
                 if training:
                     K.colstats(Zi, stats)
             n = B * To * Fo
-            mr = K.bn_finalize(stats, Co, n, bn_eps, bn_momentum, rm, rv) if training else K.bn_from_running(rm, rv, bn_eps)
-            A = K.bn_act_fwd(Zi, mr, g, beta, "relu")
+            if training:
+                post = None
+                if i == L - 1 and (seed or row_zero is not None):
+                    post, post_done = (row_zero, Fo, p_drop, seed), True
+                A, mr = K.bn_act_fwd_train(Zi, stats, g, beta, "relu", n, bn_eps, bn_momentum, rm, rv, post=post)
+            else:
+                mr = K.bn_from_running(rm, rv, bn_eps)
+                A = K.bn_act_fwd(Zi, mr, g, beta, "relu")
             saved += [Zi, mr, col, w16, g, beta]
             cfgs.append((Tc, Fc, Cc, To, Fo, Co, sy, sx))
             Tc, Fc, Cc = To, Fo, Co
         out = A.view(B * Tc, Fc * Cc)
-        seed = _next_seed("subsample.out", p_drop) if (training and p_drop > 0) else 0
-        if seed:
-            out = K.scale_dropout(out, a=1.0, drop_p=p_drop, drop_seed=seed)
-        if row_zero is not None:
-            K.zero_rows(out, row_zero)
+        if not post_done:
+            if seed:
+                out = K.scale_dropout(out, a=1.0, drop_p=p_drop, drop_seed=seed)
+            if row_zero is not None:
+                K.zero_rows(out, row_zero)
         ctx.save_for_backward(X, row_zero, *[t for t in saved if t is not None])
         ctx.layout = [[t is not None for t in saved[6 * i: 6 * i + 6]] for i in range(L)]
         ctx.cfg = (B, cfgs, p_drop, seed, training, [tuple(p.shape) for p in params[0::4]])
@@ -749,14 +757,17 @@
         for i in range(L):
             per.append([next(it) if has else None for has in ctx.layout[i]])
         dout = dout.contiguous()
-        if seed:
-            dout = K.scale_dropout(dout, a=1.0, drop_p=p_drop, drop_seed=seed)
-        elif row_zero is not None:
-            dout = dout.clone()
-        if row_zero is not None:
-            K.zero_rows(dout, row_zero)
+        Tc, Fc, Cc, To, Fo, Co, sy, sx = cfgs[-1]
+        post = (row_zero, Fo, p_drop, seed) if (seed or row_zero is not None) else None
+        if post is not None and L == 1 and Co % 64 == 0 and _CONV1_FUSED_BWD:
+            post = None
+            if seed:
+                dout = K.scale_dropout(dout, a=1.0, drop_p=p_drop, drop_seed=seed)
+            elif row_zero is not None:
+                dout = dout.clone()
+            if row_zero is not None:
+                K.zero_rows(dout, row_zero)
         grads = [None] * (4 * L)
-        Tc, Fc, Cc, To, Fo, Co, sy, sx = cfgs[-1]
         dA = dout.view(B * To * Fo, Co)
         cur = torch.cuda.current_stream(X.device)
         side = _side_stream(X.device)
@@ -784,7 +795,7 @@
                 if sg is None:
                     grads[2], grads[3] = dg, dbeta
                 continue
-            dZ = K.bn_act_bwd(Zi, dA, mr, g, beta, dg, dbeta, "relu", training)
+            dZ = K.bn_act_bwd_fused(Zi, dA, mr, g, beta, dg, dbeta, "relu", training, post=post if i == L - 1 else None)
             keep.append(dZ)
             n = B * To * Fo
             db = _zeros_f32(Co, X)
diff --git a/espresso_amd/kernels.py b/espresso_amd/kernels.py
--- a/espresso_amd/kernels.py
+++ b/espresso_amd/kernels.py
@@ -308,6 +308,42 @@
     return H
 
 
+def bn_act_fwd_train(Z, stats, gamma, beta, act, n, eps, momentum, running_mean=None, running_var=None, post=None):
+    M, C = Z.shape
+    H = torch.empty_like(Z)
+    mean_rstd = torch.empty(2, C, dtype=torch.float32, device=Z.device)
+    lib = _lib.lib()
+    if post is None:
+        check(lib.ea_bn_act_fwd_train(_p(Z), _p(stats), _p(mean_rstd), _p(running_mean), _p(running_var), _p(gamma), _p(beta), _p(H), M, C,
+                                      _ACT[act], float(n), eps, momentum, None, 0, _stream()), "ea_bn_act_fwd_train")
+    else:
+        row_zero, rows_per_flag, drop_p, drop_seed = post
+        thr, scale = drop_params(drop_p if drop_seed else 0.0)
+        check(lib.ea_bn_act_fwd_train_post(_p(Z), _p(stats), _p(mean_rstd), _p(running_mean), _p(running_var), _p(gamma), _p(beta), _p(H), M,
+                                           C, _ACT[act], float(n), eps, momentum, None, 0, _p(row_zero), rows_per_flag, drop_seed, thr,
+                                           scale, _stream()), "ea_bn_act_fwd_train_post")
+    return H, mean_rstd
+
+
+def bn_act_bwd_fused(Z, dH, mean_rstd, gamma, beta, dgamma, dbeta, act, training=True, post=None):
+    M, C = Z.shape
+    from . import functional as _F
+
+    red = _F._pool_zeros((2, C), torch.float32, Z.device)
+    dZ = torch.empty_like(Z)
+    lib = _lib.lib()
+    if post is None:
+        check(lib.ea_bn_act_bwd_fused(_p(Z), _p(dH), _p(mean_rstd), _p(gamma), _p(beta), _p(red), _p(dZ), _p(dgamma), _p(dbeta), M, C,
+                                      _ACT[act], int(training), None, 0, _stream()), "ea_bn_act_bwd_fused")
+    else:
+        row_zero, rows_per_flag, drop_p, drop_seed = post
+        thr, scale = drop_params(drop_p if drop_seed else 0.0)
+        check(lib.ea_bn_act_bwd_fused_post(_p(Z), _p(dH), _p(mean_rstd), _p(gamma), _p(beta), _p(red), _p(dZ), _p(dgamma), _p(dbeta), M, C,
+                                           _ACT[act], int(training), None, 0, _p(row_zero), rows_per_flag, drop_seed, thr, scale,
+                                           _stream()), "ea_bn_act_bwd_fused_post")
+    return dZ
+
+
 def conv1_bn_bwd(X, Z, dH, mean_rstd, gamma, beta, dgamma, dbeta, dW, dbias, B, T, F, CO, sy, sx, act, training=True):
     from . import functional as _F
 
diff --git a/include/espresso_amd.h b/include/espresso_amd.h
--- a/include/espresso_amd.h
+++ b/include/espresso_amd.h
@@ -174,6 +174,14 @@
 int ea_bn_act_bwd_fused(const void* Z, const void* dH, const float* mean_rstd, const float* gamma, const float* beta,
                         float* red, void* dZ, float* dgamma, float* dbeta, long M, int C, int act, int training,
                         float* zero_next, int zero_n, ea_stream_t stream);
+int ea_bn_act_fwd_train_post(const void* Z, const double* stats, float* mean_rstd, float* running_mean, float* running_var,
+                             const float* gamma, const float* beta, void* H, long M, int C, int act, float n, float eps,
+                             float momentum, double* zero_next, int zero_n, const uint8_t* row_zero, int rows_per_flag,
+                             uint64_t drop_seed, uint32_t drop_thr, float drop_scale, ea_stream_t stream);
+int ea_bn_act_bwd_fused_post(const void* Z, const void* dOut, const float* mean_rstd, const float* gamma, const float* beta,
+                             float* red, void* dZ, float* dgamma, float* dbeta, long M, int C, int act, int training,
+                             float* zero_next, int zero_n, const uint8_t* row_zero, int rows_per_flag, uint64_t drop_seed,
+                             uint32_t drop_thr, float drop_scale, ea_stream_t stream);
 int ea_bn_param_grad(const float* red, float* dgamma, float* dbeta, int C, ea_stream_t stream);
 int ea_conv1_bn_bwd(const float* X, const void* Z, const void* dH, const float* mean_rstd, const float* gamma, const float* beta,
                     float* red, float* dgamma, float* dbeta, float* dW, float* dbias, int B, int T, int F, int CO, int sy, int sx,
```
